# cvlab-epfl/gecco

Measured on AMD Instinct MI355X. Metric: denoiser_fwd_points_per_sec, higher is better.
Workload: dtype f16/fp6/fp8 mixed (the mixed mode with the point MLP of every layer as ONE launch: fp16 main products + fp6 block-scaled second terms for AdaGN(x) and both weights, the 768-wide hidden layer kept in registers as fp16; the other sites as in the mixed mode; fp32 accumulate, residual stream and statist; 1 GPU; C2 unconditional denoiser forward: B=64/GPU, N=2048, d=384, L=6, I=64, H=8, EDMPrecond(LinearLift(SetTransformer)), mixed fp16 / fp6- and fp8-cross-term MFMA, one-launch point MLP, random-init weights; parallelism=single GPU

## Files before the change

### gecco_amd/_lib.py

```python
from __future__ import annotations

import ctypes as C
import os

_HERE = os.path.dirname(os.path.abspath(__file__))
LIB_PATH = os.environ.get("GECCO_HIP_LIB") or os.path.join(_HERE, "libgecco_hip.so")
ABI_VERSION = 14

c_f = C.c_void_p


class GeccoAdaGN(C.Structure):
    _fields_ = [("scale_w", c_f), ("scale_b", c_f), ("bias_w", c_f), ("bias_b", c_f)]


class GeccoMLP(C.Structure):
    _fields_ = [("w0", c_f), ("b0", c_f), ("alpha", c_f), ("w2", c_f), ("b2", c_f)]


class GeccoLayer(C.Structure):
    _fields_ = [("broadcast_norm", GeccoAdaGN), ("inducers", c_f), ("kv_proj_w", c_f), ("pool_out_w", c_f),
                ("norm_1", GeccoAdaGN), ("bmlp", GeccoMLP), ("norm_2", GeccoAdaGN), ("in_proj_w", c_f),
                ("in_proj_b", c_f), ("unpool_out_w", c_f), ("unpool_out_b", c_f), ("mlp_norm", GeccoAdaGN),
                ("mlp", GeccoMLP)]


class GeccoSetTransformer(C.Structure):
    _fields_ = [("n_layers", C.c_int), ("C", C.c_int), ("H", C.c_int), ("I", C.c_int), ("ctx_dim", C.c_int),
                ("G", C.c_int), ("width", C.c_int), ("act", C.c_int), ("precision", C.c_int), ("images_ready", C.c_int),
                ("opt_mask", C.c_uint), ("opt_vals", C.c_uint), ("layers", C.POINTER(GeccoLayer))]


class GeccoLinearLift(C.Structure):
    _fields_ = [("inner", GeccoSetTransformer), ("lift_w", c_f), ("lift_b", c_f), ("lower_w", c_f),
                ("lower_b", c_f), ("sigma_data", C.c_float)]


class GeccoLinearLiftG(C.Structure):
    _fields_ = [("base", GeccoLinearLift), ("geometry_dim", C.c_int), ("do_norm", C.c_int)]


class GeccoPyramid(C.Structure):
    _fields_ = [("n_levels", C.c_int), ("C", C.c_int * 4), ("H", C.c_int * 4), ("W", C.c_int * 4), ("feat", c_f * 4),
                ("texel_f16", C.c_int)]


class GeccoReparam(C.Structure):
    _fields_ = [("kind", C.c_int), ("mean", c_f), ("std", c_f), ("logit_scale", C.c_float)]


class GeccoRayNetwork(C.Structure):
    _fields_ = [("backbone", GeccoSetTransformer), ("xyz_w", c_f), ("xyz_b", c_f), ("img_w", c_f), ("img_b", c_f),
                ("out_w", c_f), ("out_b", c_f), ("reparam", GeccoReparam), ("sigma_data", C.c_float)]


class GeccoGemm(C.Structure):
    _fields_ = [("A", c_f), ("B", c_f), ("bias", c_f), ("C", c_f), ("Z", C.c_int), ("zdiv", C.c_int), ("M", C.c_int),
                ("N", C.c_int), ("K", C.c_int), ("lda", C.c_int), ("ldb", C.c_int), ("ldc", C.c_int),
                ("sA1", C.c_longlong), ("sA2", C.c_longlong), ("sB1", C.c_longlong), ("sB2", C.c_longlong),
                ("sC1", C.c_longlong), ("sC2", C.c_longlong), ("a_kmajor", C.c_int), ("b_kmajor", C.c_int),
                ("scale", C.c_float)]


class GeccoSplitJob(C.Structure):
    _fields_ = [("W", c_f), ("img", C.c_void_p), ("Nout", C.c_int), ("K", C.c_int), ("ldw", C.c_int), ("transposed", C.c_int)]


class GeccoAdamEma(C.Structure):
    _fields_ = [("p", c_f), ("g", c_f), ("m", c_f), ("v", c_f), ("ema", c_f), ("n", C.c_size_t), ("lr", C.c_double),
                ("beta1", C.c_double), ("beta2", C.c_double), ("eps", C.c_double), ("weight_decay", C.c_double),
                ("ema_decay", C.c_double), ("grad_scale", C.c_float), ("step", C.c_int), ("do_ema", C.c_int)]


i, sz, vp, fl, db, u64 = C.c_int, C.c_size_t, C.c_void_p, C.c_float, C.c_double, C.c_uint64
PP = C.POINTER(C.c_void_p)

SIGNATURES = {
    "gecco_abi_version": (i, []),
    "gecco_build_arch": (C.c_char_p, []),
    "gecco_last_error": (C.c_char_p, []),
    "gecco_linear_f32": (i, [vp] * 9 + [i, i, i, i, i, vp]),
    "gecco_linear_row_tiles": (i, [i]),
    "gecco_linear_ex_f32": (i, [vp] * 9 + [i, i, i, i, i, i, vp, vp]),
    "gecco_linear_pair_f32": (i, [vp, vp, vp, i, vp, vp, vp, i, vp, vp, vp, i, i, i, i, vp, vp]),
    "gecco_split_bf16_images_f32": (i, [C.POINTER(GeccoSplitJob), i, vp]),
    "gecco_split_bf16_image_bytes": (sz, [i, i]),
    "gecco_linear_image_ok": (i, [i, i, i, i]),
    "gecco_split_f16_images_f32": (i, [C.POINTER(GeccoSplitJob), i, vp]),
    "gecco_split_f16_image_bytes": (sz, [i, i]),
    "gecco_linear_image_ok_f16": (i, [i, i, i, i]),
    "gecco_linear_actbwd_ok": (i, [i, i, i, i]),
    "gecco_linear_actbwd_tiles": (sz, [i, i, i]),
    "gecco_linear_actbwd_f32": (i, [vp, vp, vp, vp, i, vp, vp, vp, i, i, i, i, i, vp, vp]),
    "gecco_linear_act_keep_f32": (i, [vp, vp, vp, vp, i, vp, vp, i, i, i, i, i, vp, vp]),
    "gecco_linear_act_keep_pro_f32": (i, [vp, vp, vp, vp, vp, vp, i, vp, vp, i, i, i, i, i, vp, vp]),
    "gecco_linear_f16io": (i, [vp] * 7 + [i, i, i, i, i, i, i, vp, vp]),
    "gecco_linear_pair_f16io": (i, [vp, vp, vp, i, vp, vp, vp, i, vp, i, i, i, vp, vp]),
    "gecco_mlp_fused_f16": (i, [vp, vp, vp, vp, vp, vp, vp, vp, i, vp, i, i, i, i, vp, vp]),
    "gecco_unpool_outproj_f16": (i, [vp, vp, vp, vp, vp, vp, i, i, i, i, vp, vp]),
    "gecco_unpool_outproj_h8": (i, [vp, vp, vp, vp, vp, vp, i, i, i, i, vp, vp]),
    "gecco_mlp_fused_w": (i, [vp, vp, vp, vp, vp, vp, vp, vp, vp, i, vp, i, i, i, i, vp, vp, vp]),
    "gecco_mlp_fused_w_wsplit_bytes": (sz, [i, i]),
    "gecco_unpool_outproj_h8_wsplit_bytes": (sz, [i, i, i]),
    "gecco_unpool_attn_h8img": (i, [vp, vp, vp, i, i, i, i, vp]),
    "gecco_gemm_tn_x3_f32": (i, [vp, vp, vp, i, i, i, i, i, vp]),
    "gecco_gemm_tn_x3_bias_f32": (i, [vp, vp, vp, vp, i, i, i, i, i, vp]),
    "gecco_gemm_tn_x3_pro_f32": (i, [vp, vp, vp, vp, vp, vp, i, i, i, i, i, vp]),
    "gecco_gemm_tn_f16_f32": (i, [vp, vp, vp, vp, vp, vp, i, i, i, i, i, vp]),
    "gecco_gemm_tn_f16_tiles": (i, [i, i]),
    "gecco_gemm_tn_f16_b16_f32": (i, [vp, vp, vp, vp, i, i, i, i, i, vp]),
    "gecco_gemm_tn_f16_a16_f32": (i, [vp, vp, vp, vp, vp, vp, i, i, i, i, i, vp]),
    "gecco_gemm_tn_f16_ex_f32": (i, [vp, i, vp, i, vp, vp, vp, vp, vp, vp, vp, i, i, i, i, i, vp]),
    "gecco_linear_dotstats_a16_f32": (i, [vp] * 6 + [i, i, i, i, vp, vp]),
    "gecco_linear_astat16_actbwd_h16": (i, [vp] * 4 + [i, vp, vp, i, i, i, i, vp, vp]),
    "gecco_linear_dotstats_f32": (i, [vp] * 5 + [i, i, i, i, i, vp, vp]),
    "gecco_h8_image_bytes": (sz, [i, i]),
    "gecco_linear_h8_train_ok": (i, [i, i, i]),
    "gecco_h8_images_f32": (i, [C.POINTER(GeccoSplitJob), i, vp]),
    "gecco_linear_h8_train_f32": (i, [vp] * 5 + [i, vp, vp, vp, i, vp, vp, i, vp, i, i, i, vp, vp]),
    "gecco_astat16_image_bytes": (sz, [i, i]),
    "gecco_linear_astat16_ok": (i, [i, i, i]),
    "gecco_astat16_images_f32": (i, [C.POINTER(GeccoSplitJob), i, vp]),
    "gecco_linear_astat16_f32": (i, [vp] * 5 + [i, vp, vp, vp, i, vp, vp, i, i, i, i, vp, vp]),
    "gecco_linear_astat16_keep": (i, [vp] * 6 + [i, vp, vp, i, i, i, i, vp, vp]),
    "gecco_linear_astat16_keep_y16": (i, [vp] * 6 + [i, vp, vp, vp, i, i, i, i, vp, vp]),
    "gecco_linear_astat16_actbwd": (i, [vp] * 4 + [i, vp, vp, i, i, i, i, vp, vp]),
    "gecco_linear_act_keep_h16": (i, [vp] * 6 + [i, vp, vp, i, i, i, i, vp, vp]),
    "gecco_set_option": (i, [C.c_char_p, i]),
    "gecco_option_index": (i, [C.c_char_p]),
    "gecco_cast_f16": (i, [c_f, C.c_void_p, C.c_size_t, C.c_void_p]),
    "gecco_linear_astat_f16": (i, [vp, vp, vp, vp, vp, i, vp, vp, vp, i, vp, vp, i, i, i, i, i, vp, vp]),
    "gecco_linear_kvq_f16": (i, [vp, vp, vp, vp, vp, i, vp, vp, vp, i, vp, i, i, i, i, i, i, vp, vp]),
    "gecco_linear_kvq_y16_f16": (i, [vp, vp, vp, vp, vp, i, vp, vp, vp, i, vp, vp, i, i, i, i, i, i, vp, vp]),
    "gecco_linear_h8_img_f32": (i, [vp, vp, vp, vp, vp, vp, i, vp, i, i, i, i, i, vp, vp]),
    "gecco_linear_h8_areg_f32": (i, [vp, vp, vp, vp, vp, vp, i, i, i, i, vp, vp]),
    "gecco_affine_cast_f16": (i, [vp, vp, vp, vp, i, i, i, vp]),
    "gecco_pool_attn_f16in": (i, [vp, vp, vp, i, i, i, i, i, i, vp, sz, vp]),
    "gecco_unpool_attn_f16io": (i, [vp, vp, vp, i, i, i, i, i, i, vp]),
    "gecco_lift0_fold_f32": (i, [vp] * 8 + [i, i, i, vp]),
    "gecco_lift0_rows": (i, [vp, vp, vp, vp, i, i, i, i, i, i, i, vp]),
    "gecco_lift0_pool_f32": (i, [vp] * 5 + [i, i, i, i, vp, sz, vp]),
    "gecco_col_stats_f32": (i, [vp, vp, i, i, i, vp]),
    "gecco_stats_row_tiles": (i, [i]),
    "gecco_adagn_coeffs_f32": (i, [vp, i, i, vp, i, C.POINTER(GeccoAdaGN), vp, vp, i, i, i, fl, vp]),
    "gecco_affine_apply_f32": (i, [vp, vp, vp, vp, i, i, i, vp]),
    "gecco_adagn_f32": (i, [vp, vp, i, C.POINTER(GeccoAdaGN), vp, i, i, i, i, fl, vp, sz, vp]),
    "gecco_adagn_workspace_bytes": (sz, [i, i, i]),
    "gecco_pool_attn_f32": (i, [vp, vp, vp, i, i, i, i, i, vp, sz, vp]),
    "gecco_pool_attn_ex_f32": (i, [vp, vp, vp, i, i, i, i, i, i, vp, sz, vp]),
    "gecco_pool_attn_workspace_bytes": (sz, [i, i, i, i, i]),
    "gecco_unpool_attn_f32": (i, [vp, vp, vp, i, i, i, i, i, vp]),
    "gecco_unpool_attn_ex_f32": (i, [vp, vp, vp, i, i, i, i, i, i, vp]),
    "gecco_pool_attn_lse_f32": (i, [vp, sz, vp, i, i, i, i, i, vp]),
    "gecco_pool_attn_bwd_partials": (i, [i, i, i]),
    "gecco_pool_attn_bwd_f32": (i, [vp] * 7 + [i, i, i, i, i, vp]),
    "gecco_unpool_attn_bwd_partials": (i, [i, i, i]),
    "gecco_unpool_attn_bwd_f32": (i, [vp] * 5 + [i, i, i, i, i, vp]),
    "gecco_pool_attn_bwd_ex_f32": (i, [vp] * 7 + [i, i, i, i, i, i, vp]),
    "gecco_unpool_attn_bwd_ex_f32": (i, [vp] * 5 + [i, i, i, i, i, i, vp]),
    "gecco_edm_coeffs_f32": (i, [vp, fl, vp, i, vp]),
    "gecco_lift_f32": (i, [vp, vp, vp, vp, vp, vp, i, i, i, vp]),
    "gecco_lower_edm_f32": (i, [vp] * 9 + [i, i, i, fl, vp]),
    "gecco_set_transformer_fwd_f32": (i, [C.POINTER(GeccoSetTransformer), vp, vp, vp, i, PP, PP, vp, i, i, vp, sz, vp]),
    "gecco_set_transformer_workspace_bytes": (sz, [C.POINTER(GeccoSetTransformer), i, i]),
    "gecco_linear_lift_fwd_f32": (i, [C.POINTER(GeccoLinearLift), vp, vp, vp, vp, PP, PP, i, i, vp, sz, vp]),
    "gecco_linear_lift_workspace_bytes": (sz, [C.POINTER(GeccoLinearLift), i, i]),
    "gecco_lift_g_f32": (i, [vp, vp, vp, vp, vp, vp, i, i, i, i, vp]),
    "gecco_lower_edm_g_f32": (i, [vp] * 7 + [i, i, i, i, i, fl, vp]),
    "gecco_linear_lift_g_fwd_f32": (i, [C.POINTER(GeccoLinearLiftG), vp, vp, vp, vp, PP, PP, i, i, vp, sz, vp]),
    "gecco_linear_lift_g_workspace_bytes": (sz, [C.POINTER(GeccoLinearLiftG), i, i]),
    "gecco_nchw_to_nhwc_f32": (i, [vp, vp, i, i, i, i, vp]),
    "gecco_bilinear_taps_f32": (i, [vp, i, i, vp, vp, vp, vp, sz, vp]),
    "gecco_ray_lookup_taps_f32": (i, [vp, vp, vp, vp, vp, vp, vp, vp, vp, vp, i, i, vp]),
    "gecco_ray_lookup_f32": (i, [vp, vp, vp, C.POINTER(GeccoReparam), C.POINTER(GeccoPyramid), vp, vp, i, i, vp]),
    "gecco_lookup_row_tiles": (i, [i]),
    "gecco_ray_lookup_bwd_f32": (i, [vp, vp, vp, C.POINTER(GeccoReparam), C.POINTER(GeccoPyramid), vp, PP, i, i, vp]),
    "gecco_ray_lookup_dgeom_f32": (i, [vp, vp, C.POINTER(GeccoReparam), C.POINTER(GeccoPyramid), vp, vp, vp, i, i, vp]),
    "gecco_ray_lookup_bwd_sorted_workspace_bytes": (C.c_size_t, [C.POINTER(GeccoPyramid), i, i]),
    "gecco_ray_lookup_bwd_sorted_f32": (i, [vp, vp, vp, C.POINTER(GeccoReparam), C.POINTER(GeccoPyramid), vp, PP, i, i, vp,
                                            C.c_size_t, vp]),
    "gecco_ray_network_fwd_f32": (i, [C.POINTER(GeccoRayNetwork), vp, vp, vp, C.POINTER(GeccoPyramid), vp, vp, PP, PP,
                                      i, i, vp, sz, vp]),
    "gecco_ray_network_workspace_bytes": (sz, [C.POINTER(GeccoRayNetwork), C.POINTER(GeccoPyramid), i, i]),
# ... 112 lines not shown
```

### gecco_amd/csrc/api_common.h

```cpp
#pragma once
#include "../../include/gecco_hip.h"
#include "kernels.h"

namespace gecco_api {

extern thread_local char g_err[512];
int fail(int rc, const char* fmt, ...);

inline int check(int rc, const char* what) {
    if (rc == 0) return 0;
    if (rc > 0) return fail(rc, "%s: HIP error %d (%s)", what, rc, hipGetErrorString((hipError_t)rc));
    return fail(rc, "%s: unsupported arguments (code %d)", what, rc);
}
#define TRY(expr, what)                  \
    do {                                 \
        int rc_ = check((expr), (what)); \
        if (rc_) return rc_;             \
    } while (0)

struct Carver {
    char* base;
    size_t off = 0;
    explicit Carver(void* b) : base(static_cast<char*>(b)) {}
    float* f32(size_t n) {
        off = (off + 255) & ~size_t(255);
        float* p = base ? reinterpret_cast<float*>(base + off) : nullptr;
        off += n * sizeof(float);
        return p;
    }
};

inline int row_tiles_gemm(int rows) { const int bm = gemm_row_tile(rows); return (rows + bm - 1) / bm; }
inline int row_tiles_stats(int rows) { const int bm = stats_row_tile(rows); return (rows + bm - 1) / bm; }

enum { OPT_ASTAT = 0, OPT_CHAIN = 1, OPT_HEADMAJOR = 2, OPT_MLPFUSED = 3, OPT_UNPOOLFUSED = 4, OPT_LO8 = 5, OPT_ACTIMG = 6, OPT_H8 = 7, OPT_KVQ64 = 8, OPT_H8AREG = 9, OPT_CHAIN2 = 10, OPT_UNPOOLH8 = 11, OPT_MLPW = 12, OPT_CHAINCL = 13, OPT_H6 = 14, OPT_KVFOLD = 15, OPT_MLPWSHARE = 16, OPT_KVQPERM = 17, OPT_IMGPROJ16 = 18, OPT_LIFT0 = 19, OPT_COUNT = 20 };
enum { OPT_LIFT0_HI = OPT_LIFT0 + 1 };
int option(int which);

int make_lookup_args(const GeccoReparam* rp, const GeccoPyramid* pyr, LookupArgs* a);

inline GemmArgs gemm_args(const float* A, const float* W, const float* bias, float* C, int B, int rows, int K, int Nout) {
    GemmArgs g{};
    g.A = A; g.W = W; g.bias = bias; g.C = C; g.B = B; g.rows = rows; g.K = K; g.Nout = Nout; g.lda = K; g.ldw = K; g.ldc = Nout; g.ldr = Nout;
    return g;
}
inline GemmArgs gemm_args_pair(const float* A, const float* bias1, float* C1, int Nout1, const float* bias2, float* C2, int Nout2, int B, int rows, int K) {
    GemmArgs g = gemm_args(A, nullptr, bias1, C1, B, rows, K, Nout1 + Nout2);
    g.ldc = Nout1; g.ldr = Nout1;
    if (C2) { g.C2 = C2; g.bias2 = bias2; g.n_split = Nout1; g.ldc2 = Nout2; }
    return g;
}

inline int check_pro_pair(const char* who, const float* pro_a, const float* pro_o, bool spaced = false) {
    if ((pro_a == nullptr) == (pro_o == nullptr)) return 0;
    return fail(-1, spaced ? "%s: pro_a / pro_o must both be set" : "%s: pro_a/pro_o must both be set", who);
}
inline int check_alpha(const char* who, int act, const float* alpha, int rc) {
    return ((act == 1 || act == 2) && !alpha) ? fail(rc, "%s: GaussianActivation needs alpha", who) : 0;
}
inline int check_precision(const char* who, int precision, const void* wsplit) {
    if (precision < 0 || precision > 2) return fail(-2, "%s: precision must be 0 (fp32), 1 (split-bf16) or 2 (fp16)", who);
    if (precision >= 1 && !wsplit) return fail(-1, "%s: precision 1 / 2 need the wsplit scratch", who);
    return 0;
}
inline int check_dma_linear(const char* who, bool dma_ok, const float* W, int precision, const void* wsplit) {
    if (!dma_ok) return fail(-2, "%s: shape / precision outside the LDS-DMA kernels' reach", who);
    if (precision >= 1 && !wsplit) return fail(-1, "%s: precision 1 / 2 need wsplit", who);
    if (!W && precision == 0) return fail(-2, "%s: W == NULL (image ready) needs precision 1 / 2", who);
    return 0;
}

}
```

### gecco_amd/csrc/api_linear.hip

```cpp
#include "api_linear.h"

using namespace gecco_api;

extern "C" {

int gecco_linear_row_tiles(int rows) { return row_tiles_gemm(rows); }
int gecco_stats_row_tiles(int rows) { return row_tiles_stats(rows); }

int gecco_linear_f32(const float* A, const float* W, const float* bias, const float* pro_a, const float* pro_o,
                     const float* alpha, const float* residual, float* C, float* stats, int B, int rows, int K,
                     int Nout, int act, void* stream) {
    if (!A || !W || !C) return fail(-1, "linear: null argument");
    if (int rc = check_pro_pair("linear", pro_a, pro_o)) return rc;
    TRY(linear(Lin(A, W, bias, C, B, rows, K, Nout).pro(pro_a, pro_o).activation(act, alpha).plus(residual).with_stats(stats), (hipStream_t)stream), "linear");
    return 0;
}

int gecco_linear_ex_f32(const float* A, const float* W, const float* bias, const float* pro_a, const float* pro_o,
                        const float* alpha, const float* residual, float* C, float* stats, int B, int rows, int K,
                        int Nout, int act, int precision, void* wsplit, void* stream) {
    if (!A || !C) return fail(-1, "linear: null argument");
    if (int rc = check_pro_pair("linear", pro_a, pro_o)) return rc;
    if (int rc = check_precision("linear", precision, wsplit)) return rc;
    if (!W) {
// ... 322 lines not shown
    if (W1) {
        if (Nout2 > 0 && !W2) return fail(-1, "linear_kvq: W2 missing");
        TRY(build_images(h8_image_multi_launch, wsplit, K, s, {W1, Nout1, K, kvq_format(lo_begin / 64, lo_end / 64, order)},
                         {Nout2 > 0 ? W2 : nullptr, Nout2, K, kvq_format(0, 0, order)}, kvq_image_bytes(Nout1, K, lo_end - lo_begin)), "linear_kvq(image)");
    }
    TRY(gemm_kvq_astat_launch(g, s), "linear_kvq");
    return 0;
}

int gecco_linear_h8_img_f32(const float* x, const float* pro_a, const float* pro_o, const float* W, const float* bias,
                            const float* alpha, int act, void* c_img, int image_kind, int B, int rows, int K, int Nout, void* wsplit,
                            void* stream) {
    if (!x || !c_img || !wsplit) return fail(-1, "linear_h8_img: null argument");
    if (image_kind != 1 && image_kind != 2) return fail(-2, "linear_h8_img: image_kind must be 1 (tiled split image) or 2 (h8 activation image)");
    if (int rc = check_pro_pair("linear_h8_img", pro_a, pro_o)) return rc;
    if (int rc = check_alpha("linear_h8_img", act, alpha, -6)) return rc;
    hipStream_t s = (hipStream_t)stream;
    GemmArgs g = gemm_args(x, nullptr, bias, static_cast<float*>(c_img), B, rows, K, Nout);
    g.ldr = 0;
    g.pro_a = pro_a; g.pro_o = pro_o; g.alpha = alpha; g.act = act; g.c_img = image_kind; g.w_img = wsplit;
    g.h6 = image_kind == 2 && option(OPT_H6) ? 1 : 0;
    if (!gemm_h8_astat_supported(g))
        return fail(-2, "linear_h8_img: needs rows %% 128 == 0, Nout %% 64 == 0, Nout >= 128, K in {128, 256, 384}, act in 0 .. 3");
    if (W) TRY(build_images(h8_image_multi_launch, wsplit, K, s, {W, Nout, K, g.h6 ? H8_H6 : H8_MLP0}), "linear_h8_img(image)");
    TRY(gemm_h8_astat_launch(g, s), "linear_h8_img");
    return 0;
}

int gecco_linear_h8_areg_f32(const void* a_img, const float* W, const float* bias, const float* residual, float* C, float* stats,
                             int B, int rows, int K, int Nout, void* wsplit, void* stream) {
    if (!a_img || !C || !wsplit) return fail(-1, "linear_h8_areg: null argument");
    hipStream_t s = (hipStream_t)stream;
    GemmArgs g = gemm_args(static_cast<const float*>(a_img), nullptr, bias, C, B, rows, K, Nout);
    g.residual = residual; g.stats = stats; g.a_img = 2; g.w_img = wsplit; g.precision = 1;
    if (!gemm_h8_areg_supported(g))
        return fail(-2, "linear_h8_areg: needs rows %% 128 == 0, K in {128, 256, 384, 512, 768, 1024}, Nout %% 4 == 0");
    if (W) TRY(build_images(h8_image_multi_launch, wsplit, K, s, {W, Nout, K, H8_W128}), "linear_h8_areg(image)");
    TRY(gemm_h8_areg_launch(g, s), "linear_h8_areg");
    return 0;
}

int gecco_mlp_fused_f16(float* x, const float* pro_a, const float* pro_o, const float* W0, const float* b0, const float* W2,
                        const float* b2, const float* alpha, int act, float* stats, int B, int rows, int C, int width,
                        void* wsplit, void* stream) {
    if (!x || !pro_a || !pro_o || !wsplit || ((W0 == nullptr) != (W2 == nullptr))) return fail(-1, "mlp_fused: null argument");
    if (int rc = check_alpha("mlp_fused", act, alpha, -6)) return rc;
    if (!mlp_fused_f16_supported(C, width, rows))
        return fail(-2, "mlp_fused: needs C in {128, 256, 384}, width == 2 C, rows %% 128 == 0");
    hipStream_t s = (hipStream_t)stream;
    float* img = static_cast<float*>(wsplit);
    if (W0) {
        SplitJobs jobs;
        jobs.n = 0;
        TRY(mlp_fused_f16_stream_jobs(W0, W2, C, width, img, [&jobs](const float* W, float* at, int Nout, int K, int ldw, F16Image format, const char*) {
                if (jobs.n >= (int)(sizeof jobs.job / sizeof jobs.job[0])) return -9;
                jobs.job[jobs.n++] = SplitJob{W, at, Nout, K, ldw, format};
                return 0;
            }), "mlp_fused(split)");
        TRY(split_f16_tiled_multi_launch(jobs, s), "mlp_fused(split)");
    }
    MlpArgs ma{};
    ma.x = x; ma.pro_a = pro_a; ma.pro_o = pro_o; ma.w_stream = img; ma.b0 = b0; ma.b2 = b2; ma.alpha = alpha; ma.act = act;
    ma.stats = stats; ma.B = B; ma.rows = rows;
    TRY(mlp_fused_f16_launch(ma, C, width, s), "mlp_fused");
    return 0;
}

int gecco_unpool_outproj_f16(float* x, const void* q16, const float* kvh, const float* W, const float* bias, float* stats,
                             int B, int rows, int C, int H, void* wsplit, void* stream) {
    if (!x || !q16 || !kvh || !wsplit) return fail(-1, "unpool_outproj: null argument");
    if (!unpool_outproj_f16_supported(C, H, rows))
        return fail(-2, "unpool_outproj: needs (C, head dim) in {(128, 16), (256, 32), (384, 48)}, rows %% 128 == 0");
    hipStream_t s = (hipStream_t)stream;
    if (W) TRY(split_f16_tiled_launch(W, wsplit, C, C, C, s), "unpool_outproj(split)");
    UnpoolProjArgs ua{};
    ua.x = x; ua.q16 = q16; ua.kvh = kvh; ua.w_stream = static_cast<const float*>(wsplit); ua.bias = bias; ua.stats = stats;
    ua.B = B; ua.rows = rows; ua.H = H;
    TRY(unpool_outproj_f16_launch(ua, C, s), "unpool_outproj");
    return 0;
}

int gecco_unpool_outproj_h8(float* x, const void* q16, const float* kvh, const float* W, const float* bias, float* stats,
                            int B, int rows, int C, int H, void* wsplit, void* stream) {
    if (!x || !q16 || !kvh || !wsplit) return fail(-1, "unpool_outproj_h8: null argument");
    if (!unpool_outproj_h8_supported(C, H, rows))
        return fail(-2, "unpool_outproj_h8: needs (C, head dim) in {(128, 16), (256, 32), (384, 48)}, rows %% 128 == 0");
    hipStream_t s = (hipStream_t)stream;
    if (W) TRY(build_images(h8_image_multi_launch, wsplit, C, s, {W, C, C, H8_ATTN_ORDER}), "unpool_outproj_h8(split)");
    void* kvimg = static_cast<char*>(wsplit) + h8_image_bytes(C, C);
    TRY(kvh_image_launch(kvh, kvimg, B, C, H, s), "unpool_outproj_h8(k | v image)");
    UnpoolH8Args ua{};
    ua.x = x; ua.q16 = q16; ua.kv_img = kvimg; ua.w_img = wsplit; ua.bias = bias; ua.stats = stats; ua.B = B; ua.rows = rows; ua.H = H;
    TRY(unpool_outproj_h8_launch(ua, C, s), "unpool_outproj_h8");
    return 0;
}

int gecco_mlp_fused_w(const float* x, float* out, const float* pro_a, const float* pro_o, const float* W0, const float* b0, const float* W2,
                      const float* b2, const float* alpha, int act, float* stats, int B, int rows, int C, int width, void* wsplit, float* dbg_u,
                      void* stream) {
    if (!x || !out || !pro_a || !pro_o || !wsplit) return fail(-1, "mlp_fused_w: null argument");
    if (!mlp_fused_w_supported(C, width, rows)) return fail(-2, "mlp_fused_w: needs C in {128, 256, 384, 512}, width == 2 C, rows %% 128 == 0");
    if (act < 0 || act > 3) return fail(-6, "mlp_fused_w: act must be 0 .. 3");
    if (int rc = check_alpha("mlp_fused_w", act, alpha, -6)) return rc;
    hipStream_t s = (hipStream_t)stream;
    if (W0 && W2) TRY(mlp_fused_w_image_launch(W0, b0, W2, b2, wsplit, C, width, alpha, act, s), "mlp_fused_w(image)");
    MlpWArgs ma{};
    ma.x = x; ma.out = out; ma.pro_a = pro_a; ma.pro_o = pro_o; ma.w_img = wsplit; ma.alpha = alpha; ma.act = act; ma.stats = stats;
    ma.B = B; ma.rows = rows; ma.dbg_u = dbg_u; ma.share = option(OPT_MLPWSHARE);
    TRY(mlp_fused_w_launch(ma, C, width, s), "mlp_fused_w");
    return 0;
}

size_t gecco_mlp_fused_w_wsplit_bytes(int C, int width) { return mlp_fused_w_image_bytes(C, width); }

size_t gecco_unpool_outproj_h8_wsplit_bytes(int B, int C, int H) {
    if (H <= 0 || C % H) return 0;
    return h8_image_bytes(C, C) + unpool_outproj_h8_kv_bytes(B, C, H);
}

int gecco_unpool_attn_h8img(const void* q16, const float* kvh, void* out_img, int B, int N, int C, int H, void* stream) {
    if (!q16 || !kvh || !out_img) return fail(-1, "unpool_attn_h8img: null argument");
    if (N % 128 || C % 64 || H <= 0 || C % H || !attn_x3_supported(C / H)) return fail(-2, "unpool_attn_h8img: needs N %% 128 == 0, C %% 64 == 0, head dim 16 / 32 / 48 / 64");
    TRY(unpool_attn_launch(static_cast<const float*>(q16), kvh, static_cast<float*>(out_img), B, N, C, H, 64, (hipStream_t)stream, 2, 2, 1, 2),
        "unpool_attn_h8img");
    return 0;
}

int gecco_gemm_tn_x3_f32(const float* A, const float* Bm, float* parts, int Z, int R, int N, int K, int group, void* stream) {
    return gecco_gemm_tn_x3_bias_f32(A, Bm, parts, nullptr, Z, R, N, K, group, stream);
}

int gecco_gemm_tn_x3_bias_f32(const float* A, const float* Bm, float* parts, float* colsum_parts, int Z, int R, int N, int K,
                              int group, void* stream) {
    return gecco_gemm_tn_x3_pro_f32(A, Bm, nullptr, nullptr, parts, colsum_parts, Z, R, N, K, group, stream);
}

static TnArgs tn_args(const void* A, const void* Bm, const float* pro_a, const float* pro_o, float* parts, float* colsum_parts, int Z, int R, int N, int K, int group) {
    TnArgs g{};
    g.pro_a = pro_a; g.pro_o = pro_o;
    g.A = static_cast<const float*>(A); g.Bm = static_cast<const float*>(Bm); g.C = parts; g.Z = Z; g.R = R; g.N = N; g.K = K; g.lda = N; g.ldb = K;
    g.sA = (size_t)R * N; g.sB = (size_t)R * K; g.group = group; g.colsum = colsum_parts;
    return g;
}

int gecco_gemm_tn_x3_pro_f32(const float* A, const float* Bm, const float* pro_a, const float* pro_o, float* parts,
                             float* colsum_parts, int Z, int R, int N, int K, int group, void* stream) {
    if (!A || !Bm || !parts) return fail(-1, "gemm_tn_x3: null argument");
    if (int rc = check_pro_pair("gemm_tn_x3", pro_a, pro_o, true)) return rc;
    const TnArgs g = tn_args(A, Bm, pro_a, pro_o, parts, colsum_parts, Z, R, N, K, group);
    if (!gemm_tn_x3_supported(g)) return fail(-2, "gemm_tn_x3: needs R %% 32 == 0, N %% 4 == 0, K %% 4 == 0, group > 0");
    TRY(gemm_tn_x3_launch(g, (hipStream_t)stream), "gemm_tn_x3");
    return 0;
}

static int gemm_tn_f16(const char* who, const char* needs, const void* A, int a_f16, const void* Bm, int b_f16, const float* pro_a, const float* pro_o, float* parts,
                       float* colsum_parts, float* out, float* colsum_out, unsigned* counters, int Z, int R, int N, int K, int group, void* stream) {
    if (!A || !Bm || !parts) return fail(-1, "%s: null argument", who);
    if (int rc = check_pro_pair(who, pro_a, pro_o, true)) return rc;
    TnArgs g = tn_args(A, Bm, pro_a, pro_o, parts, colsum_parts, Z, R, N, K, group);
    g.f16 = 1; g.a_f16 = a_f16; g.b_f16 = b_f16; g.counters = counters; g.out = out; g.colsum_out = colsum_out;
    if (!gemm_tn_f16_supported(g)) return fail(-2, "%s: needs %s", who, needs);
    TRY(gemm_tn_f16_launch(g, (hipStream_t)stream), who);
    return 0;
}

int gecco_gemm_tn_f16_b16_f32(const float* A, const void* B16, float* parts, float* colsum_parts, int Z, int R, int N, int K, int group,
                              void* stream) {
    return gemm_tn_f16("gemm_tn_f16_b16", "R % 32 == 0, N % 4 == 0, K % 8 == 0, group > 0", A, 0, B16, 1, nullptr, nullptr, parts, colsum_parts, nullptr, nullptr, nullptr,
                       Z, R, N, K, group, stream);
}

int gecco_gemm_tn_f16_ex_f32(const void* A, int a_f16, const void* Bm, int b_f16, const float* pro_a, const float* pro_o, float* parts,
                             float* colsum_parts, float* out, float* colsum_out, unsigned* counters, int Z, int R, int N, int K, int group,
                             void* stream) {
    if (!A || !Bm || !parts) return fail(-1, "gemm_tn_f16_ex: null argument");
    if (int rc = check_pro_pair("gemm_tn_f16_ex", pro_a, pro_o, true)) return rc;
// ... 34 lines not shown
```

### gecco_amd/csrc/api_model_ops.hip

```cpp
#include "api_common.h"

#include <math.h>

using namespace gecco_api;

int gecco_api::make_lookup_args(const GeccoReparam* rp, const GeccoPyramid* pyr, LookupArgs* a) {
    if (!pyr || pyr->n_levels < 1 || pyr->n_levels > 4) return fail(-8, "lookup: 1..4 pyramid levels required");
    a->n_levels = pyr->n_levels;
    a->c_total = 0;
    for (int l = 0; l < 4; ++l) {
        const bool on = l < pyr->n_levels;
        a->C[l] = on ? pyr->C[l] : 0;
        a->H[l] = on ? pyr->H[l] : 1;
        a->W[l] = on ? pyr->W[l] : 1;
        a->feat[l] = on ? pyr->feat[l] : nullptr;
        if (on && !pyr->feat[l]) return fail(-1, "lookup: null pyramid level %d", l);
        a->c_total += a->C[l];
    }
    a->texel_f16 = pyr->texel_f16 ? 1 : 0;
    a->out_f16 = 0;
    a->reparam_kind = rp ? rp->kind : 0;
    a->rp_mean = rp ? rp->mean : nullptr;
    a->rp_std = rp ? rp->std : nullptr;
    a->logit_scale = rp ? rp->logit_scale : 1.1f;
// ... 116 lines not shown
    c.f32((size_t)B * H * ns * 64 * 2);
    return (c.off + 255) & ~size_t(255);
}

int gecco_pool_attn_ex_f32(const float* KV, const float* inducers, float* merged, int B, int N, int C, int H, int I,
                           int precision, void* ws, size_t ws_bytes, void* stream) {
    if (precision < 0 || precision > 2) return fail(-2, "pool_attn: precision must be 0 (fp32), 1 (split-bf16) or 2 (fp16)");
    if (ws_bytes < gecco_pool_attn_workspace_bytes(B, N, C, H, I)) return fail(-7, "pool_attn: workspace too small");
    Carver c(ws);
    const int ns = pool_attn_nsplit(B, N, H);
    float* po = c.f32((size_t)B * H * ns * 64 * (C / H));
    float* pml = c.f32((size_t)B * H * ns * 64 * 2);
    TRY(pool_attn_launch(KV, inducers, po, pml, merged, B, N, C, H, I, ns, (hipStream_t)stream, precision), "pool_attn");
    return 0;
}

int gecco_pool_attn_lse_f32(const void* ws, size_t ws_bytes, float* lse, int B, int N, int C, int H, int I, void* stream) {
    if (ws_bytes < gecco_pool_attn_workspace_bytes(B, N, C, H, I)) return fail(-7, "pool_attn_lse: workspace too small");
    Carver c(const_cast<void*>(ws));
    const int ns = pool_attn_nsplit(B, N, H);
    c.f32((size_t)B * H * ns * 64 * (C / H));
    const float* pml = c.f32((size_t)B * H * ns * 64 * 2);
    TRY(pool_attn_lse_launch(pml, lse, B, H, ns, (hipStream_t)stream), "pool_attn_lse");
    return 0;
}

int gecco_pool_attn_bwd_partials(int B, int N, int H) { return pool_attn_bwd_nsplit(B, N, H); }
int gecco_unpool_attn_bwd_partials(int B, int N, int H) { return unpool_attn_bwd_chunks(B, N, H, nullptr); }

int gecco_pool_attn_bwd_f32(const float* KV, const float* inducers, const float* merged, const float* lse, const float* dO,
                            float* dKV, float* dQ_partials, int B, int N, int C, int H, int I, void* stream) {
    return gecco_pool_attn_bwd_ex_f32(KV, inducers, merged, lse, dO, dKV, dQ_partials, B, N, C, H, I, 0, stream);
}
int gecco_unpool_attn_bwd_f32(const float* q, const float* kvh, const float* dO, float* dq, float* dkv_partials, int B, int N,
                              int C, int H, int I, void* stream) {
    return gecco_unpool_attn_bwd_ex_f32(q, kvh, dO, dq, dkv_partials, B, N, C, H, I, 0, stream);
}

int gecco_pool_attn_bwd_ex_f32(const float* KV, const float* inducers, const float* merged, const float* lse, const float* dO,
                               float* dKV, float* dQ_partials, int B, int N, int C, int H, int I, int precision, void* stream) {
    if (B <= 0 || N <= 0) return fail(-2, "pool_attn_bwd: empty batch");
    if (precision < 0 || precision > 3) return fail(-2, "pool_attn_bwd: precision must be 0 (fp32), 1 (split-bf16), 2 (fp16 operands) or 3 (fp16 operands, fp16 KV / dKV tensors)");
    const int rc = pool_attn_bwd_launch(KV, inducers, merged, lse, dO, dKV, dQ_partials, B, N, C, H, I, pool_attn_bwd_nsplit(B, N, H),
                                        (hipStream_t)stream, precision);
    if (rc == -3 || rc == -4) return fail(-2, "pool_attn_bwd: needs I == 64 and a head dim that is a multiple of 8 up to 64");
    TRY(rc, "pool_attn_bwd");
    return 0;
}

int gecco_unpool_attn_bwd_ex_f32(const float* q, const float* kvh, const float* dO, float* dq, float* dkv_partials, int B, int N,
                                 int C, int H, int I, int precision, void* stream) {
    if (B <= 0 || N <= 0) return fail(-2, "unpool_attn_bwd: empty batch");
    if (precision < 0 || precision > 3) return fail(-2, "unpool_attn_bwd: precision must be 0 (fp32), 1 (split-bf16), 2 (fp16 operands) or 3 (fp16 operands, fp16 q / dO / dq tensors)");
    const int rc = unpool_attn_bwd_launch(q, kvh, dO, dq, dkv_partials, B, N, C, H, I, (hipStream_t)stream, precision);
    if (rc == -3 || rc == -4) return fail(-2, "unpool_attn_bwd: needs I == 64 and a head dim that is a multiple of 8 up to 64");
    TRY(rc, "unpool_attn_bwd");
    return 0;
}

int gecco_pool_attn_f32(const float* KV, const float* inducers, float* merged, int B, int N, int C, int H, int I,
                        void* ws, size_t ws_bytes, void* stream) {
    return gecco_pool_attn_ex_f32(KV, inducers, merged, B, N, C, H, I, 0, ws, ws_bytes, stream);
}

int gecco_unpool_attn_ex_f32(const float* q, const float* kvh, float* out, int B, int N, int C, int H, int I,
                             int precision, void* stream) {
    if (precision < 0 || precision > 2) return fail(-2, "unpool_attn: precision must be 0 (fp32), 1 (split-bf16) or 2 (fp16)");
    TRY(unpool_attn_launch(q, kvh, out, B, N, C, H, I, (hipStream_t)stream, precision), "unpool_attn");
    return 0;
}

int gecco_unpool_attn_f32(const float* q, const float* kvh, float* out, int B, int N, int C, int H, int I,
                          void* stream) {
    return gecco_unpool_attn_ex_f32(q, kvh, out, B, N, C, H, I, 0, stream);
}

int gecco_edm_coeffs_f32(const float* sigma, float sigma_data, float* coef, int B, void* stream) {
    TRY(edm_coeffs_launch(sigma, sigma_data, coef, B, (hipStream_t)stream), "edm_coeffs");
    return 0;
}

int gecco_lift_f32(const float* x, const float* coef, const float* W, const float* bias, float* out, float* stats,
                   int B, int N, int C, void* stream) {
    TRY(lift_launch(x, coef, W, bias, out, stats, B, N, C, (hipStream_t)stream), "lift");
    return 0;
}

int gecco_lower_edm_f32(const float* feat, const float* x, const float* coef, const float* W, const float* bias,
                        const float* gn_a, const float* gn_o, float* out, float* raw, int B, int N, int C, float eps,
                        void* stream) {
    if (coef && !x) return fail(-1, "lower_edm: x required with coef");
    TRY(lower_edm_launch(feat, x, coef, W, bias, gn_a, gn_o, out, raw, B, N, C, eps, (hipStream_t)stream), "lower_edm");
    return 0;
}

int gecco_lift_g_f32(const float* x, const float* coef, const float* W, const float* bias, float* out, float* stats,
                     int B, int N, int C, int G, void* stream) {
    if (G < 1 || G > GECCO_MAX_GEOMETRY_DIM) return fail(-2, "lift_g: geometry_dim %d outside 1 .. %d", G, GECCO_MAX_GEOMETRY_DIM);
    TRY(lift_g_launch(x, coef, W, bias, out, stats, B, N, C, G, (hipStream_t)stream), "lift_g");
    return 0;
}

int gecco_lower_edm_g_f32(const float* feat, const float* x, const float* coef, const float* W, const float* bias, float* out,
                          float* raw, int B, int N, int C, int G, int do_norm, float eps, void* stream) {
    if (coef && !x) return fail(-1, "lower_edm_g: x required with coef");
    if (G < 1 || G > GECCO_MAX_GEOMETRY_DIM) return fail(-2, "lower_edm_g: geometry_dim %d outside 1 .. %d", G, GECCO_MAX_GEOMETRY_DIM);
    if (C <= 0 || C % 4 || C > 512) return fail(-2, "lower_edm_g: feature_dim %d (needs C %% 4 == 0, C <= 512)", C);
    TRY(lower_g_launch(feat, x, coef, W, bias, out, raw, B, N, C, G, do_norm, eps, (hipStream_t)stream), "lower_edm_g");
    return 0;
}

int gecco_nchw_to_nhwc_f32(const float* src, float* dst, int B, int C, int H, int W, void* stream) {
    TRY(nchw_to_nhwc_launch(src, dst, B, C, H, W, (hipStream_t)stream), "nchw_to_nhwc");
    return 0;
}

int gecco_bilinear_taps_f32(const float* uv, int H, int W, int* x0, int* y0, float* wx1, float* wy1, size_t n,
                            void* stream) {
    TRY(bilinear_taps_launch(uv, H, W, x0, y0, wx1, wy1, n, (hipStream_t)stream), "bilinear_taps");
    return 0;
}

int gecco_lookup_row_tiles(int N) { return (N + lookup_row_tile() - 1) / lookup_row_tile(); }

int gecco_cast_f16(const float* src, void* dst, size_t n, void* stream) {
    if (n && (!src || !dst)) return fail(-1, "cast_f16: null argument");
    TRY(cast_f16_launch(src, dst, n, (hipStream_t)stream), "cast_f16");
    return 0;
}

int gecco_ray_lookup_f32(const float* geom, const float* coef, const float* K, const GeccoReparam* rp,
                         const GeccoPyramid* pyr, float* out, float* stats, int B, int N, void* stream) {
    if (!geom || !K || !out) return fail(-1, "ray_lookup: null argument");
    LookupArgs a;
    int rc = make_lookup_args(rp, pyr, &a);
    if (rc) return rc;
    TRY(ray_lookup_launch(geom, coef, K, a, out, stats, B, N, (hipStream_t)stream), "ray_lookup");
    return 0;
}

int gecco_ray_lookup_taps_f32(const float* geom, const float* coef, const float* K, const GeccoReparam* rp, const GeccoPyramid* pyr, float* uv,
                              int* x0, int* y0, float* wx1, float* wy1, int B, int N, void* stream) {
    if (!geom || !K || !pyr || !uv || !x0 || !y0 || !wx1 || !wy1) return fail(-1, "ray_lookup_taps: null argument");
    LookupArgs a;
    int rc = make_lookup_args(rp, pyr, &a);
    if (rc) return rc;
    TRY(ray_lookup_taps_launch(geom, coef, K, a, uv, x0, y0, wx1, wy1, B, N, (hipStream_t)stream), "ray_lookup_taps");
    return 0;
}

int gecco_ray_lookup_bwd_f32(const float* geom, const float* coef, const float* K, const GeccoReparam* rp,
                             const GeccoPyramid* pyr, const float* dout, float* const* dfeat, int B, int N,
                             void* stream) {
    if (!geom || !K || !dout || !dfeat || !pyr) return fail(-1, "ray_lookup_bwd: null argument");
    LookupArgs a;
    int rc = make_lookup_args(rp, pyr, &a);
    if (rc) return rc;
    if (a.texel_f16) return fail(-2, "ray_lookup_bwd: fp16 texel pyramids serve the forward lookup only (pass the fp32 levels)");
    for (int l = 0; l < a.n_levels; ++l)
        if (!dfeat[l]) return fail(-1, "ray_lookup_bwd: null gradient level");
    TRY(ray_lookup_bwd_launch(geom, coef, K, a, dfeat, dout, B, N, (hipStream_t)stream), "ray_lookup_bwd");
    return 0;
}

int gecco_ray_lookup_dgeom_f32(const float* geom, const float* K, const GeccoReparam* rp, const GeccoPyramid* pyr, const float* dout,
                               float* dgeom, float* dK_partials, int B, int N, void* stream) {
// ... 353 lines not shown
```

### gecco_amd/csrc/api_network.hip

```cpp
#include "api_linear.h"

#include <atomic>
#include <stdarg.h>
#include <stdlib.h>
#include <string.h>
#include <stdio.h>

using namespace gecco_api;

namespace {

std::atomic<int> g_options[OPT_COUNT] = {-1, -1, -1, -1, -1, -1, -1, -1, -1, -1, -1, -1, -1, -1, -1, -1, -1, -1, -1, -1};
const char* const g_option_names[OPT_COUNT] = {"astat", "chain", "headmajor", "mlpfused", "unpoolfused", "lo8", "actimg", "h8", "kvq64", "h8areg", "chain2", "unpoolh8", "mlpw", "chaincl", "h6", "kvfold", "mlpwshare", "kvqperm", "imgproj16", "lift0"};
const char* const g_option_env[OPT_COUNT] = {"GECCO_ASTAT", "GECCO_CHAIN", "GECCO_HEADMAJOR", "GECCO_MLPFUSED", "GECCO_UNPOOLFUSED", "GECCO_LO8",
                                             "GECCO_ACTIMG", "GECCO_H8", "GECCO_KVQ64", "GECCO_H8AREG", "GECCO_CHAIN2", "GECCO_UNPOOLH8", "GECCO_MLPW", "GECCO_CHAINCL", "GECCO_H6", "GECCO_KVFOLD", "GECCO_MLPWSHARE",
                                             "GECCO_KVQPERM", "GECCO_IMGPROJ16", "GECCO_LIFT0"};
thread_local const GeccoSetTransformer* t_plan = nullptr;
struct PlanScope {
    const GeccoSetTransformer* prev;
    explicit PlanScope(const GeccoSetTransformer* p) : prev(t_plan) { t_plan = p; }
    ~PlanScope() { t_plan = prev; }
};

}

namespace gecco_api {

thread_local char g_err[512] = "";

int fail(int rc, const char* fmt, ...) {
    va_list ap;
    va_start(ap, fmt);
    vsnprintf(g_err, sizeof g_err, fmt, ap);
    va_end(ap);
    return rc;
}

int option(int which) {
    if (t_plan && ((t_plan->opt_mask >> which) & 1u)) {
        const int v = (int)((t_plan->opt_vals >> which) & 1u);
        return which == OPT_LIFT0 && v ? v + (int)((t_plan->opt_vals >> OPT_LIFT0_HI) & 1u) : v;
    }
    int v = g_options[which].load(std::memory_order_relaxed);
    if (v < 0) {
        const char* e = getenv(g_option_env[which]);
        const int fill = which == OPT_LIFT0 ? (e ? (atoi(e) < 0 ? 0 : atoi(e) > 2 ? 2 : atoi(e)) : 3)
                         : e ? (atoi(e) != 0) : (which != OPT_MLPWSHARE && which != OPT_IMGPROJ16);
        if (g_options[which].compare_exchange_strong(v, fill, std::memory_order_relaxed)) v = fill;
    }
    return v;
}

int linear(Lin& a, hipStream_t s) {
    GemmArgs& g = a.g;
    const int precision = a.prec;
    g.precision = 0; g.w_img = nullptr;
    if (g.act < 0 || g.act > 4) return -6;
    if ((g.act == 1 || g.act == 2) && !g.alpha) return -6;
    const bool fast = precision == 1 ? gemm_f32_dma_supported(g, 1) : precision == 2 ? gemm_f16_dma_supported(g) : false;
    const bool img = a.wsplit || a.img_ready;
    if ((g.a_f16 || g.c_f16) && !(fast && precision == 2 && img)) return -9;
    if ((g.a_img || g.c_img) && !(fast && precision == 1 && img)) return -9;
    if ((g.mul_u || g.pre_out || g.dot_x) && !(precision == 0 ? gemm_f32_dma_supported(g, 0) : (fast && img))) return -9;
    if (!g.W && !(fast && a.img_ready)) return -9;
    if (fast && img) {
        if (a.img_ready) {
            g.w_img = a.img_ready;
        } else {
            int rc = precision == 1 ? split_bf16_tiled_launch(g.W, a.wsplit, g.Nout, g.K, g.ldw, s) : split_f16_tiled_launch(g.W, a.wsplit, g.Nout, g.K, g.ldw, s);
            if (rc) return rc;
            g.w_img = a.wsplit;
        }
        g.precision = precision;
    }
    return gemm_f32_launch(g, s);
}

int linear_pair(const Lin& a, const float* W2, const float* b2, int Nout2, float* C2, hipStream_t s) {
    GemmArgs g = a.g;
    const int precision = a.prec, Nout1 = a.g.Nout, K = a.g.K;
    if ((g.c_f16 || g.a_f16) && precision != 2) return -9;
    g.Nout = Nout1 + Nout2;
    g.C2 = C2; g.W2 = W2; g.bias2 = b2; g.n_split = Nout1; g.ldc2 = Nout2;
    if (precision == 2 ? !gemm_f16_dma_supported(g) : !gemm_f32_dma_supported(g)) return 1;
    if (precision == 1 || precision == 2) {
        if (a.img_ready) {
            g.w_img = a.img_ready;
        } else {
            if (!a.wsplit) return 1;
            const bool x3 = precision == 1;
            const ImageFormat plain = x3 ? ImageFormat(BF16_PLAIN) : ImageFormat(F16_PLAIN);
            const int rc = build_images(x3 ? launch_each<split_bf16_tiled_launch> : launch_each<split_f16_tiled_launch>, a.wsplit, K, s, {g.W, Nout1, K, plain}, {W2, Nout2, K, plain},
                                        x3 ? split_bf16_image_bytes(Nout1, K) : split_f16_image_bytes(Nout1, K));
            if (rc) return rc;
            g.w_img = a.wsplit;
        }
        g.precision = precision;
    }
    if (precision == 2) return gemm_f16_dma_launch(g, s);
    return gemm_f32_dma_launch(g, s);
}

}

namespace {

struct STWorkspace {
    float *big, *q, *attn;
    float *stats_x, *stats_s;
    float *a1, *o1, *a2, *o2, *as, *os;
    float *part_o, *part_ml;
    float *merged, *h0, *u, *h2, *h, *kvh;
    float* wsplit;
    float* wimg;
    size_t wimg_layer, o_q, o_out, o_w0, o_w2;
    size_t o_pout, o_b0, o_b2, o_ukv, b2_half;
    size_t o_mf;
    size_t o_q16, o_kv_lo, o_q64;
    float* mc;
    size_t bytes;
};

struct Lift0In { const float *x, *coef, *lift_w, *lift_b; };

int max_i(int a, int b) { return a > b ? a : b; }

STWorkspace carve_st(const GeccoSetTransformer* st, int B, int N, void* base) {
    Carver c(base);
// ... 38 lines not shown
        w.wimg_layer = w.o_mf + (prec == 2 ? img(W, C) + img(C, W) : 0);
        if (st->precision == 4 && mlp_fused_w_supported((int)C, (int)W, 128)) w.wimg_layer += mlp_fused_w_image_bytes((int)C, (int)W) / sizeof(float);
        w.wimg = prec >= 1 ? c.f32(w.wimg_layer * st->n_layers) : nullptr;
        w.b2_half = img(C, C);
        const size_t f16_kv = split_f16_image_bytes(2 * (int)C, (int)C) / sizeof(float), f16_q = split_f16_image_bytes((int)C, (int)C) / sizeof(float);
        w.o_q16 = f16_kv; w.o_kv_lo = f16_kv + f16_q;
        w.o_q64 = kvq_image_bytes(2 * (int)C, (int)C, (int)C) / sizeof(float);
    }
    w.mc = c.f32((size_t)B * 3 * C * 4);
    w.bytes = (c.off + 255) & ~size_t(255);
    return w;
}

bool chain_stream_fits(const GeccoSetTransformer* st, const STWorkspace& w) {
    const size_t C = st->C, W = st->width;
    const bool f16 = st->precision == 2;
    auto img = [f16](size_t n, size_t k) { return (f16 ? split_f16_image_bytes((int)n, (int)k) : 2 * split_f16_image_bytes((int)n, (int)k)) / sizeof(float); };
    if (C % 128) return false;
    return w.o_b0 - w.o_pout == img(C, C) && w.o_b2 - w.o_b0 == img(W, C) && w.o_ukv - w.o_b2 == W / C * w.b2_half && w.o_mf - w.o_ukv == img(2 * C, C);
}

int astat_linear(const float* x, const float* pa, const float* po, const float* img, const float* bias1, int Nout1,
                 float* C1, const float* bias2, int Nout2, float* C2, const float* alpha, int act, int B, int rows,
                 int K, hipStream_t s, int hm_hd = 0, const float* img_lo = nullptr, int use64 = 0, int kvq_perm = 0, int lo_fp8 = 0) {
    GemmArgs g = gemm_args_pair(x, bias1, C1, Nout1, bias2, C2, Nout2, B, rows, K);
    g.pro_a = pa; g.pro_o = po; g.precision = 2; g.w_img = img; g.c_f16 = 1; g.hm_hd = hm_hd;
    if (use64) {
        g.kvq_perm = kvq_perm; if (use64 == 2) { g.lo_begin = Nout1 / 128; g.lo_tiles = Nout1 / 64; }
        if (!img || act || !gemm_kvq_astat_supported(g)) return 1;
        return gemm_kvq_astat_launch(g, s);
    }
    g.alpha = alpha; g.act = act; g.w_img2 = img_lo;
    if (img_lo && C2) { g.lo_begin = Nout1 / 256; g.lo_tiles = Nout1 / 128; }
    g.lo_fp8 = img_lo && lo_fp8;
    if (!img || !gemm_f16_astat_supported(g)) return 1;
    return gemm_f16_astat_launch(g, s);
}

int h8_linear(const float* a_img, const float* w_img, const float* bias, const float* res, float* C, float* stats, int B, int rows,
              int K, int Nout, hipStream_t s) {
    GemmArgs g = gemm_args(a_img, nullptr, bias, C, B, rows, K, Nout);
    g.residual = res; g.stats = stats; g.a_img = 2; g.w_img = w_img; g.precision = 1;
    return gemm_h8_areg_launch(g, s);
}

int coeffs(const float* stats, int T, int rows, const float* t, int ctx, const GeccoAdaGN* p, float* a, float* o,
           int B, int C, int G, hipStream_t s) {
    return adagn_coeffs_launch(stats, T, rows, t, ctx, p ? p->scale_w : nullptr, p ? p->scale_b : nullptr,
                               p ? p->bias_w : nullptr, p ? p->bias_b : nullptr, a, o, B, C, G, 1e-5f, s);
}

struct StRoute {
    int rc;
    int pr, apr, kmod, Tn, Ti, ns;
    bool mixed;
    bool astat;
    bool imgs, build;
    bool io16;
    bool a16;
    int hd_try;
    bool mlpf_on;
    bool h8_on;
    bool kvq_on;
    bool kvq16_on;
    int use64;
    bool kvq_p48;
    bool lo8;
    bool h8x, h8o;
    bool h6_on;
    bool uo8_on;
    bool uof_on;
    int aimg;
    bool o8;
    int himg;
    bool mfw_on;
    int mfw_share;
    bool chain_on;
    bool chain2_on;
    bool chain;
    bool chain_cl;
    bool kvfold;
    int lift0;
    bool lift0_hm;
};

StRoute st_route(const GeccoSetTransformer* st, int B, int N, const float* const* h_in, bool points) {
    StRoute r{};
    const int C = st->C, I = st->I, H = st->H, G = st->G, Wd = st->width, act = st->act;
    const int prec = st->precision == 4 ? 3 : st->precision;
    const bool wimg = prec >= 1;
    const void* const some_img = st;
    r.mixed = prec == 3 && N >= 128 && N % 128 == 0 && C % 128 == 0 && C <= 512 && !(C % H) &&
              attn_x3_supported(C / H) && st->I == 64 && option(OPT_ASTAT);
    const bool mixed = r.mixed;
    const int pr = r.pr = mixed ? 1 : (prec == 3 ? 1 : prec);
    r.apr = mixed ? 2 : pr;
    r.Tn = row_tiles_gemm(N); r.Ti = row_tiles_gemm(I); r.kmod = (pr == 2 || mixed) ? 32 : 16;
    const int ns = r.ns = pool_attn_nsplit(B, N, H);
    r.mlpf_on = pr == 2 && wimg && option(OPT_MLPFUSED) && mlp_fused_f16_supported(C, Wd, N);
    if (mixed && wimg && option(OPT_H8) && option(OPT_ACTIMG) && (act == 0 || (act >= 1 && act <= 3))) {
        GemmArgs hg{};
        hg.c_img = 1; hg.w_img = some_img; hg.rows = N; hg.Nout = Wd; hg.K = C; hg.lda = C; hg.act = act;
        r.h8_on = gemm_h8_astat_supported(hg) && Wd % 16 == 0 && C % 16 == 0;
    }
    r.kvq_on = mixed && wimg && option(OPT_KVQ64) && option(OPT_HEADMAJOR) && (C == 128 || C == 256 || C == 384 || C == 512) && !((C / H) & 7);
    r.kvq16_on = !mixed && pr == 2 && wimg && option(OPT_KVQ64) && option(OPT_HEADMAJOR) && option(OPT_ASTAT) && C == 512 &&
                 !((C / H) & 7) && N >= 128 && N % 128 == 0;
    auto h8_areg_takes = [&](int K) {
        GemmArgs hg{};
        hg.a_img = 2; hg.w_img = some_img; hg.rows = N; hg.Nout = C; hg.K = K; hg.lda = K; hg.ldc = C; hg.ldr = C;
        return gemm_h8_areg_supported(hg);
    };
    r.h8x = mixed && wimg && option(OPT_H8AREG) && option(OPT_ACTIMG) && Wd % 64 == 0 && N % 128 == 0 && h8_areg_takes(Wd);
    r.h8o = mixed && wimg && option(OPT_H8AREG) && option(OPT_ACTIMG) && I == 64 && C % 64 == 0 && attn_x3_supported(C / H) && h8_areg_takes(C);
    r.h6_on = r.h8_on && r.h8x && option(OPT_H6);
    r.uo8_on = r.h8o && r.kvq_on && option(OPT_UNPOOLH8) && I == 64 && unpool_outproj_h8_supported(C, H, N) &&
               unpool_outproj_h8_kv_bytes(B, C, H) <= (size_t)B * N * C * sizeof(float);
    r.mfw_on = mixed && st->precision == 4 && option(OPT_MLPW) && wimg && mlp_fused_w_supported(C, Wd, N) &&
               (size_t)B * N * C * sizeof(float) < ((size_t)1 << 31);
    r.mfw_share = r.mfw_on ? option(OPT_MLPWSHARE) : 0;
    r.chain_on = pr == 2 && wimg && option(OPT_CHAIN) && inducer_chain_f16_supported(C, Wd, H, G, I) &&
                 (ns == 1 || ns == 2 || ns == 4 || ns == 8);
    const bool cl_ok = option(OPT_CHAINCL) && C >= 256 && (size_t)st->n_layers * 8 <= (size_t)I * C;
    r.chain2_on = mixed && wimg && option(OPT_CHAIN2) && (C <= 384 || cl_ok) && inducer_chain_f16_supported(C, Wd, H, G, I) &&
                  (ns == 1 || ns == 2 || ns == 4 || ns == 8) && (act >= 0 && act <= 3);
    r.imgs = pr >= 1 && wimg && !(C % r.kmod) && !(Wd % r.kmod);
    r.build = r.imgs && !st->images_ready;
    r.astat = option(OPT_ASTAT);
    r.hd_try = option(OPT_HEADMAJOR) ? C / H : 0;
    r.use64 = r.kvq_on ? 2 : r.kvq16_on ? 1 : 0;
    r.kvq_p48 = r.kvq_on && option(OPT_KVQPERM) && r.hd_try && kvq_perm48_ok(C / H, C, 2 * C, C);
    r.lo8 = mixed && !r.kvq_on && option(OPT_LO8) && gemm_f16_astat_lo8_supported(C);
    r.io16 = (pr == 2 || mixed) && r.imgs && N >= 128 && attn_x3_supported(C / H) && !(C % 8) && !(Wd % 8);
    if (mixed && !(r.io16 && !(N % 128) && !(C % 128))) {
        r.rc = fail(-3, "set_transformer: the mixed mode needs rows %% 128 == 0, feature_dim %% 128 == 0 and a head dim of 16 / 32 / 48 / 64");
        return r;
    }
    r.a16 = r.io16 && !mixed;
    r.uof_on = !mixed && r.imgs && I == 64 && option(OPT_UNPOOLFUSED) && unpool_outproj_f16_supported(C, H, N);
    r.aimg = pr == 1 && !r.a16 && r.imgs && option(OPT_ACTIMG) && I == 64 && attn_x3_supported(C / H) && N >= 128 && N % 128 == 0 && C % 64 == 0;
    r.o8 = r.h8o && r.aimg && N % 128 == 0;
    r.himg = pr == 1 && !r.a16 && r.imgs && option(OPT_ACTIMG) && N >= 128 && N % 128 == 0 && Wd % 16 == 0 && C % 16 == 0;
    r.chain = (r.chain_on || r.chain2_on) && r.imgs;
    r.chain_cl = r.chain && cl_ok;
    r.kvfold = r.uo8_on && r.chain && option(OPT_KVFOLD);
    for (int li = 0; r.kvfold && li < st->n_layers; ++li)
        if (h_in && h_in[li]) r.kvfold = false;
    r.lift0 = points && lift0_supported(C, H) ? option(OPT_LIFT0) : 0;
    if (r.lift0 == 3) r.lift0 = C >= 256 ? 2 : 0;
    if (r.lift0 == 2 && !lift0_pool_supported(C, H)) r.lift0 = 1;
    r.lift0_hm = r.lift0 && r.io16 && r.astat && r.hd_try && lift0_head_major_ok(C / H);
    if (r.lift0 && r.uo8_on && !r.lift0_hm) r.lift0 = 0;
    return r;
}

template <class Job, int Cap, class Launch>
int push_job(Job (&table)[Cap], int& n, const Job& job, Launch launch) {
    if (n >= Cap) { const int rc = launch(); n = 0; if (rc) return rc; }
    table[n++] = job;
    return 0;
}
struct JobQueue {
    SplitJobs jobs;
    int (*launch)(const SplitJobs&, hipStream_t);
    hipStream_t s;
    JobQueue(int (*launch_)(const SplitJobs&, hipStream_t), hipStream_t s_) : launch(launch_), s(s_) { jobs.n = 0; }
    int flush() { const int rc = launch(jobs, s); jobs.n = 0; return rc; }
    int push(const float* Wp, float* img, int Nout, int K, int ldw, ImageFormat format) {
        return push_job(jobs.job, jobs.n, SplitJob{Wp, img, Nout, K, ldw, format}, [this] { return launch(jobs, s); });
    }
};

int build_weight_images(const StRoute& r, const GeccoSetTransformer* st, const STWorkspace& w, const float* const* h_in, hipStream_t s) {
    const int C = st->C, Wd = st->width, act = st->act;
    JobQueue jobs(r.pr == 2 ? split_f16_tiled_multi_launch : split_bf16_tiled_multi_launch, s);
    const ImageFormat plain = r.pr == 2 ? ImageFormat(F16_PLAIN) : ImageFormat(BF16_PLAIN);
    JobQueue jobs16(split_f16_tiled_multi_launch, s);
    JobQueue jobs8(h8_image_multi_launch, s);
    MlpWImageJob mjobs[16];
    int nmj = 0;
    auto flush_mj = [&] { return mlp_fused_w_images_launch(mjobs, nmj, C, Wd, act, s); };
    for (int li = 0; li < st->n_layers; ++li) {
        const GeccoLayer& L = st->layers[li];
        float* base = w.wimg + (size_t)li * w.wimg_layer;
        const bool cached = h_in && h_in[li];
        const bool own_kvq = r.mixed || r.kvq16_on;
        const bool pts = li == 0 && r.lift0;
        const bool kv_img = !cached && !pts, q_img = !pts;
        if (r.kvq_on) {
            const KvqOrder order = r.kvq_p48 ? KVQ_HEAD48 : KVQ_PLAIN;
            if (kv_img) TRY(jobs8.push(L.kv_proj_w, base, 2 * C, C, C, kvq_format(C / 64, 2 * C / 64, order)), "split(kv_proj, kvq)");
            if (q_img) TRY(jobs8.push(L.in_proj_w, base + w.o_q64, C, C, C, kvq_format(0, 0, order)), "split(q_proj, kvq)");
        } else if (r.mixed) {
            if (kv_img) TRY(jobs16.push(L.kv_proj_w, base, 2 * C, C, C, F16_PLAIN), "split(weights)");
            if (q_img) TRY(jobs16.push(L.in_proj_w, base + w.o_q16, C, C, C, F16_PLAIN), "split(weights)");
            if (kv_img) TRY(jobs16.push(L.kv_proj_w, base + w.o_kv_lo, 2 * C, C, C, r.lo8 ? F16_LO_FP8 : F16_LO), "split(weights)");
        }
        const bool chain2_here = r.chain2_on && !cached;
        if (chain2_here) {
            TRY(jobs16.push(L.pool_out_w, base + w.o_pout, C, C, C, F16_HI_LO), "split(pool.out_proj, two-term)");
            TRY(jobs16.push(L.bmlp.w0, base + w.o_b0, Wd, C, C, F16_HI_LO), "split(broadcast.mlp.0, two-term)");
            for (int hf = 0; hf < Wd / C; ++hf)
                TRY(jobs16.push(L.bmlp.w2 + (size_t)hf * C, base + w.o_b2 + hf * w.b2_half, C, C, Wd, F16_HI_LO), "split(broadcast.mlp.2 K-half, two-term)");
            TRY(jobs16.push(L.in_proj_w + (size_t)C * C, base + w.o_ukv, 2 * C, C, C, F16_HI_LO), "split(unpool.in_proj kv, two-term)");
        }
        if (r.kvq16_on) {
            if (kv_img) TRY(jobs8.push(L.kv_proj_w, base, 2 * C, C, C, kvq_format(0, 0)), "split(kv_proj, kvq)");
            if (q_img) TRY(jobs8.push(L.in_proj_w, base + w.o_q, C, C, C, kvq_format(0, 0)), "split(q_proj, kvq)");
        }
        if (!cached && !chain2_here) {
            if (!own_kvq && kv_img) TRY(jobs.push(L.kv_proj_w, base, 2 * C, C, C, plain), "split(kv_proj)");
            TRY(jobs.push(L.pool_out_w, base + w.o_pout, C, C, C, plain), "split(pool.out_proj)");
            TRY(jobs.push(L.bmlp.w0, base + w.o_b0, Wd, C, C, plain), "split(broadcast.mlp.0)");
            if (r.chain_on) {
                for (int hf = 0; hf < Wd / C; ++hf)
                    TRY(jobs.push(L.bmlp.w2 + (size_t)hf * C, base + w.o_b2 + hf * w.b2_half, C, C, Wd, plain), "split(broadcast.mlp.2 K-half)");
            } else {
                TRY(jobs.push(L.bmlp.w2, base + w.o_b2, C, Wd, Wd, plain), "split(broadcast.mlp.2)");
            }
        }
        if (!chain2_here) TRY(jobs.push(L.in_proj_w + (size_t)C * C, base + w.o_ukv, 2 * C, C, C, plain), "split(unpool.in_proj kv)");
        if (!own_kvq && q_img) TRY(jobs.push(L.in_proj_w, base + w.o_q, C, C, C, plain), "split(q_proj)");
        if (r.h8o) TRY(jobs8.push(L.unpool_out_w, base + w.o_out, C, C, C, r.uo8_on ? H8_ATTN_ORDER : H8_W128), "split(out_proj, h8)");
        else TRY(jobs.push(L.unpool_out_w, base + w.o_out, C, C, C, plain), "split(out_proj)");
        if (r.mlpf_on) {
            const int rc = mlp_fused_f16_stream_jobs(L.mlp.w0, L.mlp.w2, C, Wd, base + w.o_mf, [&jobs](const float* W, float* at, int Nout, int K, int ldw, F16Image format, const char* what) {
                return check(jobs.push(W, at, Nout, K, ldw, format), what);
            });
            if (rc) return rc;
        } else if (r.mfw_on) {
            TRY(push_job(mjobs, nmj, MlpWImageJob{L.mlp.w0, L.mlp.b0, L.mlp.w2, L.mlp.b2, base + w.o_mf, L.mlp.alpha}, flush_mj), "split(mlp, w2 streams)");
        } else {
            if (r.h8_on) TRY(jobs8.push(L.mlp.w0, base + w.o_w0, Wd, C, C, r.h6_on ? H8_H6 : H8_MLP0), "split(mlp.0, h8)");
            else TRY(jobs.push(L.mlp.w0, base + w.o_w0, Wd, C, C, plain), "split(mlp.0)");
            if (r.h8x) TRY(jobs8.push(L.mlp.w2, base + w.o_w2, C, Wd, Wd, H8_W128), "split(mlp.2, h8)");
// ... 36 lines not shown
                       : fail(rc < 0 ? rc : -3, "set_transformer: q projection outside the A-stationary kernel's reach (its weight image is in that kernel's format)");
    if (rc == 0 && r.hd_try) c.hm = 1;
    if (rc < 0) return check(rc, with_kv ? "kv_proj|q_proj (A-stationary)" : "unpool.in_proj(q) (A-stationary)");
    c.q_done = rc == 0;
    if (c.q_done || !with_kv) return 0;
    if (io16) TRY(affine_cast_f16_launch(c.x, w.a1, w.o1, w.attn, B, N, C, c.s), "broadcast_norm -> fp16");
    Lin kv = Lin(io16 ? w.attn : c.x, L.kv_proj_w, nullptr, w.big, B, N, C, 2 * C).pro(io16 ? nullptr : w.a1, io16 ? nullptr : w.o1).f16(io16, io16);
    rc = linear_pair(Lin(kv).weights(r.pr, w.wsplit, (2 * C) % 128 == 0 ? c.im : nullptr), L.in_proj_w, L.in_proj_b, C, w.q, c.s);
    if (rc < 0) return check(rc, "kv_proj|q_proj");
    c.q_done = rc == 0;
    if (!c.q_done) TRY(linear(kv.weights(r.pr, w.wsplit, c.im), c.s), "kv_proj");
    return 0;
}

int project_from_points(StLayer& c, bool with_kv) {
    const StRoute& r = c.r; const STWorkspace& w = c.w; const GeccoLayer& L = c.L;
    const int C = c.st->C, H = c.st->H, B = c.B, N = c.N;
    TRY(lift0_fold_launch(L.kv_proj_w, L.in_proj_w, L.in_proj_b, c.pts->lift_w, c.pts->lift_b, w.a1, w.o1, w.mc, with_kv ? 0 : 2 * C, 3 * C, B, C, c.s), "lift0 fold");
    const int hd = r.lift0_hm ? C / H : 0;
    const Lift0Seg segs[2] = {{w.q, 2 * C, C, hd}, {w.big, 0, 2 * C, hd}};
    TRY(lift0_rows_launch(c.pts->x, c.pts->coef, w.mc, segs, with_kv && r.lift0 == 1 ? 2 : 1, r.io16, B, N, C, c.s), "lift0 rows");
    c.hm = hd != 0;
    c.q_done = true;
    return 0;
}

int inducer_stage(StLayer& c) {
    const StRoute& r = c.r; const STWorkspace& w = c.w; const GeccoLayer& L = c.L; const GeccoSetTransformer* st = c.st; hipStream_t s = c.s;
    const int C = st->C, I = st->I, H = st->H, G = st->G, Wd = st->width, ctx = st->ctx_dim, act = st->act, B = c.B, pr = r.pr;
    if (c.pts && r.lift0 == 2) {
        TRY(lift0_pool_launch(c.pts->x, c.pts->coef, w.mc, L.inducers, w.part_o, w.part_ml, B, c.N, C, H, r.ns, s), "pool_attn (points)");
        if (!r.chain) TRY(pool_merge_launch(w.part_o, w.part_ml, w.merged, B, C, H, r.ns, s), "pool_attn merge");
    } else {
        TRY(pool_attn_launch(w.big, L.inducers, w.part_o, w.part_ml, r.chain ? nullptr : w.merged, B, c.N, C, H, I, r.ns, s, r.apr, r.io16, c.hm), "pool_attn");
    }
    if (r.chain) {
        ChainArgs ca{};
        ca.part_o = w.part_o; ca.part_ml = w.part_ml; ca.nsplit = r.ns; ca.H = H;
        ca.w_stream = c.im + w.o_pout;
        ca.b0 = L.bmlp.b0; ca.b2 = L.bmlp.b2; ca.bkv = L.in_proj_b + C; ca.alpha = L.bmlp.alpha; ca.act = act; ca.two_term = r.chain2_on ? 1 : 0;
        ca.n1_scale_w = L.norm_1.scale_w; ca.n1_scale_b = L.norm_1.scale_b; ca.n1_bias_w = L.norm_1.bias_w; ca.n1_bias_b = L.norm_1.bias_b;
        ca.n2_scale_w = L.norm_2.scale_w; ca.n2_scale_b = L.norm_2.scale_b; ca.n2_bias_w = L.norm_2.bias_w; ca.n2_bias_b = L.norm_2.bias_b;
        ca.t = c.t; ca.ctx_dim = ctx; ca.G = G; ca.eps = 1e-5f; ca.h_out = c.hdst; ca.kvh = w.kvh; ca.B = B;
        if (r.chain_cl) {
            ca.cluster = 1; ca.x1 = w.h0; ca.x3 = w.h2; ca.xu = reinterpret_cast<unsigned*>(w.u);
            ca.flags = reinterpret_cast<unsigned*>(w.merged) + (size_t)c.li * B * 8;
        }
        if (r.kvfold) {
            ca.kv_img = reinterpret_cast<unsigned short*>(w.attn);
            ca.kv_img_bytes = (int)(unpool_outproj_h8_kv_bytes(1, C, H) / H);
            c.kv_img_done = true;
        }
        if ((act == 1 || act == 2) && !L.bmlp.alpha) return fail(-6, "inducer chain: GaussianActivation needs alpha");
        TRY(inducer_chain_f16_launch(ca, C, Wd, s), "inducer chain");
        c.kvh_done = true;
    } else {
        TRY(linear(Lin(w.merged, L.pool_out_w, nullptr, w.h0, B, I, C, C).with_stats(w.stats_s).weights(pr, w.wsplit, c.img(w.o_pout)), s), "pool.out_proj");
        TRY(coeffs(w.stats_s, r.Ti, I, c.t, ctx, &L.norm_1, w.as, w.os, B, C, G, s), "adagn_coeffs(norm_1)");
        TRY(linear(Lin(w.h0, L.bmlp.w0, L.bmlp.b0, w.u, B, I, C, Wd).pro(w.as, w.os).activation(act, L.bmlp.alpha).weights(pr, w.wsplit, c.img(w.o_b0)), s), "broadcast.mlp.0");
        TRY(linear(Lin(w.u, L.bmlp.w2, L.bmlp.b2, w.h2, B, I, Wd, C).with_stats(w.stats_s).weights(pr, w.wsplit, c.img(w.o_b2)), s), "broadcast.mlp.2");
        TRY(coeffs(w.stats_s, r.Ti, I, c.t, ctx, &L.norm_2, w.as, w.os, B, C, G, s), "adagn_coeffs(norm_2)");
        TRY(affine_apply_launch(w.h2, w.as, w.os, c.hdst, B, I, C, s), "norm_2 apply");
    }
    c.h = c.hdst;
    return 0;
}

int unpool_stage(StLayer& c) {
    const StRoute& r = c.r; const STWorkspace& w = c.w; const GeccoLayer& L = c.L; float* x = c.x; hipStream_t s = c.s;
    const int C = c.st->C, I = c.st->I, H = c.st->H, B = c.B, N = c.N, pr = r.pr;
    const bool io16 = r.io16;
    if (!c.kvh_done)
        TRY(linear(Lin(c.h, L.in_proj_w + (size_t)C * C, L.in_proj_b + C, w.kvh, B, I, C, 2 * C).weights(pr, w.wsplit, c.img(w.o_ukv)), s), "unpool.in_proj(kv)");
    if (!c.q_done && io16 && c.cached)
        if (const int rc = project_stage(c, false)) return rc;
    if (!c.q_done) {
        if (io16 && c.cached) TRY(affine_cast_f16_launch(x, w.a1, w.o1, w.attn, B, N, C, s), "broadcast_norm -> fp16");
        TRY(linear(Lin(io16 ? w.attn : x, L.in_proj_w, L.in_proj_b, w.q, B, N, C, C).pro(io16 ? nullptr : w.a1, io16 ? nullptr : w.o1)
                       .weights(pr, w.wsplit, c.img(w.o_q)).f16(io16, io16), s), "unpool.in_proj(q)");
    }
    if (r.uo8_on) {
        if (!c.hm || !c.im) return fail(-3, "set_transformer: unpool + out_proj (h8) needs the head-major fp16 q");
        if (!c.kv_img_done) TRY(kvh_image_launch(w.kvh, w.attn, B, C, H, s), "unpool k | v image");
        UnpoolH8Args ua{};
        ua.x = x; ua.q16 = w.q; ua.kv_img = w.attn; ua.w_img = c.im + w.o_out; ua.bias = L.unpool_out_b; ua.stats = w.stats_x; ua.B = B; ua.rows = N; ua.H = H;
        TRY(unpool_outproj_h8_launch(ua, C, s), "unpool attention + out_proj (h8)");
    } else if (r.uof_on && c.hm) {
        UnpoolProjArgs ua{};
        ua.x = x; ua.q16 = w.q; ua.kvh = w.kvh; ua.w_stream = c.im + w.o_out; ua.bias = L.unpool_out_b; ua.stats = w.stats_x; ua.B = B; ua.rows = N; ua.H = H;
        TRY(unpool_outproj_f16_launch(ua, C, s), "unpool attention + out_proj");
    } else {
        TRY(unpool_attn_launch(w.q, w.kvh, w.attn, B, N, C, H, I, s, r.apr, r.mixed ? 2 : (int)io16, c.hm, r.o8 ? 2 : r.aimg), "unpool_attn");
        if (r.o8)
            TRY(h8_linear(w.attn, c.im + w.o_out, L.unpool_out_b, x, x, w.stats_x, B, N, C, C, s), "unpool.out_proj+residual (h8)");
        else
            TRY(linear(Lin(w.attn, L.unpool_out_w, L.unpool_out_b, x, B, N, C, C).plus(x).with_stats(w.stats_x).weights(pr, w.wsplit, c.img(w.o_out))
                           .f16(r.a16, 0).image(r.aimg, 0), s), "unpool.out_proj+residual");
    }
    return 0;
}

int mlp_stage(StLayer& c) {
    const StRoute& r = c.r; const STWorkspace& w = c.w; const GeccoLayer& L = c.L; const GeccoSetTransformer* st = c.st; hipStream_t s = c.s;
    const int C = st->C, G = st->G, Wd = st->width, act = st->act, B = c.B, N = c.N, pr = r.pr, himg = r.himg;
    const bool a16 = r.a16; float *x = c.x, *so = c.so;
    TRY(coeffs(w.stats_x, r.Tn, N, c.t, st->ctx_dim, &L.mlp_norm, w.a2, w.o2, B, C, G, s), "adagn_coeffs(mlp_norm)");
    if (r.mlpf_on && c.im) {
        MlpArgs ma{};
        ma.x = x; ma.pro_a = w.a2; ma.pro_o = w.o2; ma.w_stream = c.im + w.o_mf;
        ma.b0 = L.mlp.b0; ma.b2 = L.mlp.b2; ma.alpha = L.mlp.alpha; ma.act = act; ma.stats = so; ma.B = B; ma.rows = N;
        if ((act == 1 || act == 2) && !L.mlp.alpha) return fail(-6, "mlp: GaussianActivation needs alpha");
        TRY(mlp_fused_f16_launch(ma, C, Wd, s), "mlp (fused)");
        return 0;
    }
    int m0_done = a16 && r.astat ? astat_linear(x, w.a2, w.o2, c.img(w.o_w0), L.mlp.b0, Wd, w.big, nullptr, 0, nullptr, L.mlp.alpha, act, B, N, C, s) : 1;
    if (m0_done < 0) TRY(m0_done, "mlp.0 (A-stationary)");
    if (m0_done == 1 && r.mfw_on && c.im) {
        MlpWArgs ma{};
        ma.x = x; ma.out = x; ma.pro_a = w.a2; ma.pro_o = w.o2; ma.w_img = c.im + w.o_mf; ma.alpha = L.mlp.alpha;
        ma.act = act; ma.stats = so; ma.B = B; ma.rows = N; ma.share = r.mfw_share;
        if ((act == 1 || act == 2) && !L.mlp.alpha) return fail(-6, "mlp: GaussianActivation needs alpha");
        TRY(mlp_fused_w_launch(ma, C, Wd, s), "mlp (one launch, w2)");
        return 0;
    }
    if (m0_done == 1 && r.h8_on && himg && c.im) {
        GemmArgs hg{};
        hg.A = x; hg.pro_a = w.a2; hg.pro_o = w.o2; hg.bias = L.mlp.b0; hg.alpha = L.mlp.alpha; hg.act = act; hg.C = w.big;
        hg.B = B; hg.rows = N; hg.K = C; hg.Nout = Wd; hg.lda = C; hg.ldw = C; hg.ldc = Wd; hg.c_img = r.h8x ? 2 : 1; hg.w_img = c.im + w.o_w0; hg.h6 = r.h6_on ? 1 : 0;
        if ((act == 1 || act == 2) && !L.mlp.alpha) return fail(-6, "mlp.0: GaussianActivation needs alpha");
        TRY(gemm_h8_astat_launch(hg, s), "mlp.0 (h8)");
        m0_done = 0;
    }
    if (m0_done == 1) {
        if (a16) TRY(affine_cast_f16_launch(x, w.a2, w.o2, w.attn, B, N, C, s), "mlp_norm -> fp16");
        TRY(linear(Lin(a16 ? w.attn : x, L.mlp.w0, L.mlp.b0, w.big, B, N, C, Wd).pro(a16 ? nullptr : w.a2, a16 ? nullptr : w.o2).activation(act, L.mlp.alpha)
                       .weights(pr, w.wsplit, c.img(w.o_w0)).f16(a16, a16).image(0, (himg && r.h8x) ? 2 : himg), s), "mlp.0");
    }
    if (himg && r.h8x && c.im) {
        TRY(h8_linear(w.big, c.im + w.o_w2, L.mlp.b2, x, x, so, B, N, Wd, C, s), "mlp.2+residual (h8)");
        return 0;
    }
    TRY(linear(Lin(w.big, L.mlp.w2, L.mlp.b2, x, B, N, Wd, C).plus(x).with_stats(so).weights(pr, w.wsplit, c.img(w.o_w2)).f16(a16, 0).image(himg, 0), s), "mlp.2+residual");
    return 0;
}

int st_forward(const GeccoSetTransformer* st, float* x, const float* t, const float* stats_x, int stats_T,
               const float* const* h_in, float* const* h_out, float* stats_out, int B, int N, void* ws,
               size_t ws_bytes, hipStream_t s, const Lift0In* pts = nullptr) {
    if (!st || !x || !t || !ws) return fail(-1, "set_transformer: null argument");
    if (st->I != 64) return fail(-3, "set_transformer: num_inducers must be 64 (got %d)", st->I);
    if (st->C % st->H || st->C % st->G || st->C % 4) return fail(-3, "set_transformer: bad feature_dim %d", st->C);
    if (st->act < 0 || st->act > 3) return fail(-3, "set_transformer: act must be 0 (identity), 1 / 2 (GaussianActivation normalized / raw) or 3 (ReLU)");
    PlanScope plan_scope(st);
    const STWorkspace w = carve_st(st, B, N, ws);
    if (ws_bytes < w.bytes) return fail(-7, "set_transformer: workspace too small (%zu < %zu)", ws_bytes, w.bytes);
    const StRoute r = st_route(st, B, N, h_in, pts != nullptr);
    if (r.rc) return r.rc;
    if (r.chain && !chain_stream_fits(st, w)) return fail(-3, "set_transformer: the inducer chain's weight stream does not fill its places in the workspace");
    const int C = st->C, H = st->H, G = st->G;
    const float* sx = stats_x; int sT = stats_T;
    if (!sx) {
        TRY(col_stats_launch(x, w.stats_x, B, N, C, s), "col_stats");
        sx = w.stats_x;
        sT = row_tiles_stats(N);
    }
    int rc = r.build ? build_weight_images(r, st, w, h_in, s) : 0;
    if (rc) return rc;
    if (r.chain_cl) TRY((int)hipMemsetAsync(w.merged, 0, (size_t)st->n_layers * B * 8 * sizeof(unsigned), s), "inducer chain counters");
    if (r.kvfold) TRY((int)hipMemsetAsync(w.attn, 0, unpool_outproj_h8_kv_bytes(B, C, H), s), "k | v image pads");
    for (int li = 0; li < st->n_layers; ++li) {
        const GeccoLayer& L = st->layers[li];
        const bool cached = h_in && h_in[li];
        StLayer c{st, r, w, L, li, r.imgs ? w.wimg + (size_t)li * w.wimg_layer : nullptr, x, t, B, N, s, cached ? h_in[li] : nullptr,
                  (h_out && h_out[li]) ? h_out[li] : w.h, (li + 1 < st->n_layers) ? w.stats_x : stats_out, cached};
        TRY(coeffs(sx, sT, N, t, st->ctx_dim, &L.broadcast_norm, w.a1, w.o1, B, C, G, s), "adagn_coeffs(broadcast_norm)");
        if (li == 0 && r.lift0) c.pts = pts;
        rc = c.pts ? project_from_points(c, !cached) : cached ? 0 : project_stage(c, true);
        if (!rc && !cached) rc = inducer_stage(c);
        if (!rc) rc = unpool_stage(c);
        if (!rc) rc = mlp_stage(c);
        if (rc) return rc;
        sx = w.stats_x;
        sT = r.Tn;
    }
    return 0;
}

struct LLWorkspace {
    float *feat, *coef, *stats;
    void* st_ws;
    size_t st_bytes, bytes;
};

LLWorkspace carve_ll(const GeccoLinearLift* m, int B, int N, void* base) {
    Carver c(base);
    LLWorkspace w;
    w.feat = c.f32((size_t)B * N * m->inner.C);
    w.coef = c.f32((size_t)B * 5);
    w.stats = c.f32((size_t)B * row_tiles_stats(N) * 2 * m->inner.C);
    c.off = (c.off + 255) & ~size_t(255);
    w.st_bytes = carve_st(&m->inner, B, N, nullptr).bytes;
    w.st_ws = base ? static_cast<char*>(base) + c.off : nullptr;
    w.bytes = c.off + w.st_bytes;
    return w;
}

struct RNWorkspace {
    float *feat, *raw, *coef, *stats_raw, *stats_x, *stats_out, *a_raw, *o_raw, *a_out, *o_out, *wsplit, *wfold, *bfold;
    void* st_ws;
    size_t st_bytes, bytes;
};

RNWorkspace carve_rn(const GeccoRayNetwork* m, int c_total, int B, int N, void* base) {
    Carver c(base);
    RNWorkspace w;
    const size_t C = m->backbone.C;
    w.feat = c.f32((size_t)B * N * C);
    w.raw = c.f32((size_t)B * N * c_total);
    w.coef = c.f32((size_t)B * 5);
    w.stats_raw = c.f32((size_t)B * gecco_lookup_row_tiles(N) * 2 * c_total);
    w.stats_x = c.f32((size_t)B * row_tiles_gemm(N) * 2 * C);
    w.stats_out = c.f32((size_t)B * row_tiles_gemm(N) * 2 * C);
    w.a_raw = c.f32((size_t)B * c_total);
    w.o_raw = c.f32((size_t)B * c_total);
    w.a_out = c.f32((size_t)B * C);
    w.o_out = c.f32((size_t)B * C);
    w.wsplit = c.f32(((C + 127) / 128 * 128) * (size_t)c_total);
    const bool fold = m->backbone.precision == 4;
    w.wfold = fold ? c.f32((size_t)B * ((C + 127) / 128 * 128) * c_total / 2) : nullptr;
    w.bfold = fold ? c.f32((size_t)B * C) : nullptr;
    c.off = (c.off + 255) & ~size_t(255);
    w.st_bytes = carve_st(&m->backbone, B, N, nullptr).bytes;
    w.st_ws = base ? static_cast<char*>(base) + c.off : nullptr;
    w.bytes = c.off + w.st_bytes;
    return w;
}

}

extern "C" {

int gecco_abi_version(void) { return GECCO_ABI_VERSION; }
const char* gecco_build_arch(void) { return "gfx950"; }
const char* gecco_last_error(void) { return g_err; }

int gecco_option_index(const char* name) {
    if (name)
        for (int i = 0; i < OPT_COUNT; ++i)
            if (!strcmp(name, g_option_names[i])) return i;
    return -1;
}

int gecco_set_option(const char* name, int value) {
    if (!name) return fail(-1, "set_option: null name");
    for (int i = 0; i < OPT_COUNT; ++i)
        if (!strcmp(name, g_option_names[i])) {
            g_options[i].store(value < 0 ? -1 : i == OPT_LIFT0 ? (value > 2 ? 2 : value) : (value != 0), std::memory_order_relaxed);
            return 0;
        }
    return fail(-2, "set_option: unknown option '%s' (astat, chain, headmajor, mlpfused, unpoolfused, lo8, actimg, h8, kvq64, h8areg, chain2, unpoolh8, mlpw, chaincl, h6, kvfold, mlpwshare, kvqperm, imgproj16, lift0)", name);
}

size_t gecco_set_transformer_workspace_bytes(const GeccoSetTransformer* st, int B, int N) {
    return carve_st(st, B, N, nullptr).bytes;
}

int gecco_set_transformer_fwd_f32(const GeccoSetTransformer* st, float* x, const float* t, const float* stats_x,
                                  int stats_T, const float* const* h_in, float* const* h_out, float* stats_out,
                                  int B, int N, void* ws, size_t ws_bytes, void* stream) {
    return st_forward(st, x, t, stats_x, stats_T, h_in, h_out, stats_out, B, N, ws, ws_bytes, (hipStream_t)stream);
}

size_t gecco_linear_lift_workspace_bytes(const GeccoLinearLift* m, int B, int N) {
    return carve_ll(m, B, N, nullptr).bytes;
}

int gecco_linear_lift_fwd_f32(const GeccoLinearLift* m, const float* x, const float* sigma, float* denoised,
                              float* raw, const float* const* h_in, float* const* h_out, int B, int N, void* ws,
                              size_t ws_bytes, void* stream) {
    if (!m || !x || !sigma || !(denoised || raw)) return fail(-1, "linear_lift: null argument");
    LLWorkspace w = carve_ll(m, B, N, ws);
    if (ws_bytes < w.bytes) return fail(-7, "linear_lift: workspace too small (%zu < %zu)", ws_bytes, w.bytes);
    hipStream_t s = (hipStream_t)stream;
    const int C = m->inner.C;
    TRY(edm_coeffs_launch(sigma, m->sigma_data, w.coef, B, s), "edm_coeffs");
    TRY(lift_launch(x, w.coef, m->lift_w, m->lift_b, w.feat, w.stats, B, N, C, s), "lift");
    if (m->inner.ctx_dim != 1) return fail(-3, "linear_lift: t_embed_dim must be 1 under EDMPrecond");
    const Lift0In pts{x, w.coef, m->lift_w, m->lift_b};
    int rc = st_forward(&m->inner, w.feat, w.coef + 4 * (size_t)B, w.stats, row_tiles_stats(N), h_in, h_out, nullptr, B,
                        N, w.st_ws, w.st_bytes, s, &pts);
    if (rc) return rc;
    TRY(lower_edm_launch(w.feat, x, w.coef, m->lower_w, m->lower_b, nullptr, nullptr, denoised, raw, B, N, C, 1e-5f, s),
        "lower_edm");
    return 0;
}

size_t gecco_linear_lift_g_workspace_bytes(const GeccoLinearLiftG* m, int B, int N) {
    return carve_ll(&m->base, B, N, nullptr).bytes;
}

int gecco_linear_lift_g_fwd_f32(const GeccoLinearLiftG* m, const float* x, const float* sigma, float* denoised,
                                float* raw, const float* const* h_in, float* const* h_out, int B, int N, void* ws,
                                size_t ws_bytes, void* stream) {
    if (!m || !x || !sigma || !(denoised || raw)) return fail(-1, "linear_lift_g: null argument");
    const int G = m->geometry_dim, C = m->base.inner.C;
    if (G < 1 || G > GECCO_MAX_GEOMETRY_DIM)
        return fail(-2, "linear_lift_g: geometry_dim %d outside 1 .. %d", G, GECCO_MAX_GEOMETRY_DIM);
    if (C % 4 || C > 512) return fail(-2, "linear_lift_g: feature_dim %d (needs C %% 4 == 0, C <= 512)", C);
    LLWorkspace w = carve_ll(&m->base, B, N, ws);
    if (ws_bytes < w.bytes) return fail(-7, "linear_lift_g: workspace too small (%zu < %zu)", ws_bytes, w.bytes);
    hipStream_t s = (hipStream_t)stream;
    if (m->base.inner.ctx_dim != 1) return fail(-3, "linear_lift_g: t_embed_dim must be 1 under EDMPrecond");
    TRY(edm_coeffs_launch(sigma, m->base.sigma_data, w.coef, B, s), "edm_coeffs");
    TRY(lift_g_launch(x, w.coef, m->base.lift_w, m->base.lift_b, w.feat, w.stats, B, N, C, G, s), "lift_g");
    int rc = st_forward(&m->base.inner, w.feat, w.coef + 4 * (size_t)B, w.stats, row_tiles_stats(N), h_in, h_out, nullptr, B,
                        N, w.st_ws, w.st_bytes, s);
    if (rc) return rc;
    TRY(lower_g_launch(w.feat, x, w.coef, m->base.lower_w, m->base.lower_b, denoised, raw, B, N, C, G, m->do_norm, 1e-5f, s),
        "lower_edm_g");
    return 0;
}

size_t gecco_ray_network_workspace_bytes(const GeccoRayNetwork* m, const GeccoPyramid* pyr, int B, int N) {
    int ct = 0;
    for (int l = 0; l < pyr->n_levels && l < 4; ++l) ct += pyr->C[l];
    return carve_rn(m, ct, B, N, nullptr).bytes;
}

int gecco_ray_network_fwd_f32(const GeccoRayNetwork* m, const float* x, const float* sigma, const float* K,
                              const GeccoPyramid* pyr, float* denoised, float* raw, const float* const* h_in,
                              float* const* h_out, int B, int N, void* ws, size_t ws_bytes, void* stream) {
    if (!m || !x || !sigma || !K || !(denoised || raw)) return fail(-1, "ray_network: null argument");
    if (m->backbone.ctx_dim != 1) return fail(-3, "ray_network: t_embed_dim must be 1 under EDMPrecond");
    LookupArgs a;
    int rc = make_lookup_args(&m->reparam, pyr, &a);
    if (rc) return rc;
    RNWorkspace w = carve_rn(m, a.c_total, B, N, ws);
    if (ws_bytes < w.bytes) return fail(-7, "ray_network: workspace too small (%zu < %zu)", ws_bytes, w.bytes);
    hipStream_t s = (hipStream_t)stream;
    const int C = m->backbone.C;
    TRY(edm_coeffs_launch(sigma, m->sigma_data, w.coef, B, s), "edm_coeffs");
    TRY(lift_launch(x, w.coef, m->xyz_w, m->xyz_b, w.feat, nullptr, B, N, C, s), "xyz_embed");
    PlanScope plan_scope(&m->backbone);
    const bool img16 = m->backbone.precision == 4 && option(OPT_IMGPROJ16) && a.c_total % 32 == 0 && N >= 128 && C % 4 == 0;
    a.out_f16 = img16;
    TRY(ray_lookup_launch(x, w.coef, K, a, w.raw, w.stats_raw, B, N, s), "ray_lookup");
    TRY(adagn_coeffs_launch(w.stats_raw, gecco_lookup_row_tiles(N), N, nullptr, 0, nullptr, nullptr, nullptr, nullptr,
                            w.a_raw, w.o_raw, B, a.c_total, 16, 1e-5f, s), "gn16(img)");
    if (img16) {
        TRY(fold_f16_image_launch(m->img_w, m->img_b, w.a_raw, w.o_raw, w.wfold, w.bfold, B, C, a.c_total, a.c_total, s), "img_feature_proj fold");
        GemmArgs g{};
        g.A = w.raw; g.a_f16 = 1; g.bias = w.bfold; g.bias_bstride = C; g.residual = w.feat; g.C = w.feat; g.stats = w.stats_x;
        g.B = B; g.rows = N; g.K = a.c_total; g.Nout = C; g.lda = a.c_total; g.ldw = a.c_total; g.ldc = C; g.ldr = C;
        g.precision = 2; g.w_img = w.wfold; g.w_img_bstride = (size_t)((C + 127) / 128 * 128) * a.c_total / 2;
        if (!gemm_f16_dma_supported(g)) return fail(-9, "img_feature_proj: shape outside the fp16 streaming kernel");
        TRY(gemm_f32_launch(g, s), "img_feature_proj");
    } else {
        TRY(linear(Lin(w.raw, m->img_w, m->img_b, w.feat, B, N, a.c_total, C).pro(w.a_raw, w.o_raw).plus(w.feat).with_stats(w.stats_x)
                       .weights(m->backbone.precision >= 3 ? 1 : m->backbone.precision, w.wsplit), s), "img_feature_proj");
    }
    rc = st_forward(&m->backbone, w.feat, w.coef + 4 * (size_t)B, w.stats_x, row_tiles_gemm(N), h_in, h_out,
                    w.stats_out, B, N, w.st_ws, w.st_bytes, s);
    if (rc) return rc;
    TRY(adagn_coeffs_launch(w.stats_out, row_tiles_gemm(N), N, nullptr, 0, nullptr, nullptr, nullptr, nullptr, w.a_out,
                            w.o_out, B, C, 16, 1e-5f, s), "gn16(out)");
    TRY(lower_edm_launch(w.feat, x, w.coef, m->out_w, m->out_b, w.a_out, w.o_out, denoised, raw, B, N, C, 1e-5f, s),
        "output_proj+edm");
    return 0;
}
// ... 3 lines not shown
```

### gecco_amd/csrc/kernel_prims.h

```cpp
#pragma once
#include "common.h"

#include <type_traits>
#include <utility>

typedef _Float16 f16x2 __attribute__((ext_vector_type(2)));
typedef _Float16 f16x4 __attribute__((ext_vector_type(4)));
typedef _Float16 f16x8 __attribute__((ext_vector_type(8)));
typedef _Float16 f16x32 __attribute__((ext_vector_type(32)));
typedef __bf16 bf16x2 __attribute__((ext_vector_type(2)));
typedef __bf16 bf16x4 __attribute__((ext_vector_type(4)));
typedef __bf16 bf16x8 __attribute__((ext_vector_type(8)));
typedef float f32x2 __attribute__((ext_vector_type(2)));
typedef unsigned int u32x2 __attribute__((ext_vector_type(2)));
typedef unsigned int u32x4 __attribute__((ext_vector_type(4)));
typedef unsigned int u32x6 __attribute__((ext_vector_type(6)));
typedef int i32x4 __attribute__((ext_vector_type(4)));
typedef int i32x8 __attribute__((ext_vector_type(8)));
typedef short s16x2 __attribute__((ext_vector_type(2)));
typedef short s16x4 __attribute__((ext_vector_type(4)));
typedef unsigned short u16;

template <int... I, class F>
__device__ __forceinline__ void static_for(std::integer_sequence<int, I...>, F&& f) {
    (f(std::integral_constant<int, I>{}), ...);
}
template <int N, class F>
__device__ __forceinline__ void static_for(F&& f) {
    static_for(std::make_integer_sequence<int, N>{}, f);
}
template <int TAG, int... I, class F>
__device__ __forceinline__ void static_for_tag(std::integer_sequence<int, I...>, F&& f) {
    (f(std::integral_constant<int, I>{}, std::integral_constant<int, TAG>{}), ...);
}

constexpr int waitcnt_imm(int vm, int lgkm) { return (vm & 0xF) | (0x7 << 4) | ((lgkm & 0xF) << 8) | ((vm >> 4) << 14); }
template <int N>
__device__ __forceinline__ void wait_vm() { __builtin_amdgcn_s_waitcnt(waitcnt_imm(N, 0xF)); }
template <int N>
__device__ __forceinline__ void wait_vm_lgkm0() { __builtin_amdgcn_s_waitcnt(waitcnt_imm(N, 0)); }

__device__ __forceinline__ void wave_lds_sync() { asm volatile("s_waitcnt lgkmcnt(0)" ::: "memory"); }
__device__ __forceinline__ void lds_barrier() {
    asm volatile("s_waitcnt lgkmcnt(0)" ::: "memory");
    __builtin_amdgcn_s_barrier();
    asm volatile("" ::: "memory");
}

__device__ __forceinline__ void dma16_buf(__amdgpu_buffer_rsrc_t rsrc, unsigned voff, unsigned soff, void* lds_wave_base) {
    __builtin_amdgcn_raw_ptr_buffer_load_lds(rsrc, (__attribute__((address_space(3))) void*)lds_wave_base, 16, voff, soff, 0, 0);
}
__device__ __forceinline__ u32x4 frag(const u16* p) { return *reinterpret_cast<const u32x4*>(p); }

__device__ __forceinline__ unsigned swap_pair(unsigned v) {
    return (unsigned)__builtin_amdgcn_mov_dpp((int)v, 0xB1, 0xF, 0xF, true);
}
__device__ __forceinline__ float wave_sum(float v) {
#pragma unroll
    for (int o = 32; o > 0; o >>= 1) v += __shfl_xor(v, o, 64);
    return v;
}
__device__ __forceinline__ float wave_max(float v) {
#pragma unroll
    for (int o = 32; o > 0; o >>= 1) v = fmaxf(v, __shfl_xor(v, o, 64));
    return v;
}
__device__ __forceinline__ float lanes_sum(float v, int width) {
    for (int o = 1; o < width; o <<= 1) v += __shfl_xor(v, o, 64);
    return v;
}

__device__ __forceinline__ unsigned pack2(float v0, float v1) {
    asm volatile("" : "+v"(v0), "+v"(v1));
    f16x2 p;
    p[0] = (_Float16)v0;
    p[1] = (_Float16)v1;
    return __builtin_bit_cast(unsigned, p);
}
__device__ __forceinline__ float clamp448(float v) { return __builtin_fminf(__builtin_fmaxf(v, -448.f), 448.f); }
__device__ __forceinline__ unsigned pack_fp8x4(float a, float b, float c, float d) {
    int pk = 0;
    pk = __builtin_amdgcn_cvt_pk_fp8_f32(a, b, pk, false);
    pk = __builtin_amdgcn_cvt_pk_fp8_f32(c, d, pk, true);
    return (unsigned)pk;
}

template <bool F16>
__device__ __forceinline__ void split4(const f32x4& x, u32x2& hi, u32x2& lo) {
    if (F16) {
        f16x4 v;
#pragma unroll
        for (int e = 0; e < 4; ++e) v[e] = (_Float16)x[e];
        hi = __builtin_bit_cast(u32x2, v);
        lo = hi;
        return;
    }
    bf16x4 l;
#pragma unroll
    for (int p = 0; p < 2; ++p) {
        const unsigned ua = __float_as_uint(x[2 * p]), uc = __float_as_uint(x[2 * p + 1]);
        hi[p] = __builtin_amdgcn_perm(uc, ua, 0x07060302u);
        l[2 * p] = (__bf16)(x[2 * p] - __uint_as_float(ua & 0xFFFF0000u));
        l[2 * p + 1] = (__bf16)(x[2 * p + 1] - __uint_as_float(uc & 0xFFFF0000u));
    }
    lo = __builtin_bit_cast(u32x2, l);
}
template <bool F16>
__device__ __forceinline__ void split_acc8(const f32x16& s, int e0, u32x4& hi, u32x4& lo) {
    if (F16) {
        f16x8 v;
#pragma unroll
        for (int e = 0; e < 8; ++e) v[e] = (_Float16)s[e0 + e];
        hi = __builtin_bit_cast(u32x4, v);
        lo = hi;
        return;
    }
    u32x4 hb;
    bf16x8 l;
#pragma unroll
    for (int p = 0; p < 4; ++p) {
        const float a = s[e0 + 2 * p], c = s[e0 + 2 * p + 1];
        const unsigned ua = __float_as_uint(a), uc = __float_as_uint(c);
        hb[p] = __builtin_amdgcn_perm(uc, ua, 0x07060302u);
        l[2 * p] = (__bf16)(a - __uint_as_float(ua & 0xFFFF0000u));
        l[2 * p + 1] = (__bf16)(c - __uint_as_float(uc & 0xFFFF0000u));
    }
    hi = hb;
    lo = __builtin_bit_cast(u32x4, l);
}
template <bool F16>
__device__ __forceinline__ f32x16 mfma3(const u32x4& ahi, const u32x4& alo, const u32x4& bhi, const u32x4& blo, f32x16 acc) {
    if (F16) return __builtin_amdgcn_mfma_f32_32x32x16_f16(__builtin_bit_cast(f16x8, ahi), __builtin_bit_cast(f16x8, bhi), acc, 0, 0, 0);
    const bf16x8 ah = __builtin_bit_cast(bf16x8, ahi), al = __builtin_bit_cast(bf16x8, alo);
    const bf16x8 bh = __builtin_bit_cast(bf16x8, bhi), bl = __builtin_bit_cast(bf16x8, blo);
    acc = __builtin_amdgcn_mfma_f32_32x32x16_bf16(al, bh, acc, 0, 0, 0);
    acc = __builtin_amdgcn_mfma_f32_32x32x16_bf16(ah, bl, acc, 0, 0, 0);
    return __builtin_amdgcn_mfma_f32_32x32x16_bf16(ah, bh, acc, 0, 0, 0);
}

__device__ __forceinline__ int e8m0_scale_byte(float m) {
    const int e = (int)(__float_as_uint(m * (16.0f / 15.0f)) >> 23) - 2;
    return m > 0.f ? (e < 1 ? 1 : e) : 127;
}
__device__ __forceinline__ float e8m0_scale_of(int byte) { return __uint_as_float((unsigned)byte << 23); }
__device__ __forceinline__ float absmax32(f16x8 a, f16x8 b, f16x8 c, f16x8 d) {
    auto ab = [](f16x8 v) {
        u32x4 u = __builtin_bit_cast(u32x4, v);
        u &= 0x7fff7fffu;
        return __builtin_bit_cast(f16x8, u);
    };
    f16x8 m = __builtin_elementwise_max(__builtin_elementwise_max(ab(a), ab(b)), __builtin_elementwise_max(ab(c), ab(d)));
    const f16x2 m2 = __builtin_elementwise_max(__builtin_elementwise_max(f16x2{m[0], m[1]}, f16x2{m[2], m[3]}),
// ... 13 lines not shown
```

### gecco_amd/csrc/kernels.h

```cpp
#pragma once
#include <hip/hip_runtime.h>
#include <stddef.h>
#include "weight_images.h"

struct GemmArgs {
    const float* A;
    const float* W;
    const float* bias;
    const float* pro_a;
    const float* pro_o;
    const float* alpha;
    const float* residual;
    float* C;
    float* stats;
    int B, rows, K, Nout;
    int lda, ldw, ldc, ldr;
    int act;
    int precision;
    const void* w_img;
    float* C2;
    const float* W2;
    const float* bias2;
    int n_split, ldc2;
    int a_f16, c_f16;
// ... 16 lines not shown
    int h6;
    int h8_stagger, h8_pair;
};

int gemm_row_tile(int rows);
int gemm_f32_launch(const GemmArgs& g, hipStream_t st);
bool gemm_f32_dma_supported(const GemmArgs& g, int precision = -1);
int gemm_f32_dma_launch(const GemmArgs& g, hipStream_t st);
size_t split_bf16_image_bytes(int Nout, int K);
int split_bf16_tiled_launch(const float* W, void* img, int Nout, int K, int ldw, hipStream_t st);
int split_bf16_tiled_multi_launch(const SplitJobs& jobs, hipStream_t st);

bool gemm_f16_dma_supported(const GemmArgs& g);
int gemm_f16_dma_launch(const GemmArgs& g, hipStream_t st);
size_t split_f16_image_bytes(int Nout, int K);
int fold_f16_image_launch(const float* W, const float* bias, const float* pa, const float* po, void* img, float* bias_out, int B, int Nout, int K,
                          int ldw, hipStream_t st);
int split_f16_tiled_launch(const float* W, void* img, int Nout, int K, int ldw, hipStream_t st);
int split_f16_tiled_multi_launch(const SplitJobs& jobs, hipStream_t st);

struct ChainArgs {
    const float* part_o;
    const float* part_ml;
    int nsplit, H;
    const float* w_stream;
    int two_term;
    const float *b0, *b2, *bkv, *alpha;
    int act;
    const float *n1_scale_w, *n1_scale_b, *n1_bias_w, *n1_bias_b;
    const float *n2_scale_w, *n2_scale_b, *n2_bias_w, *n2_bias_b;
    const float* t;
    int ctx_dim, G;
    float eps;
    float* h_out;
    float* kvh;
    int B;
    int cluster;
    float *x1, *x3;
    unsigned* xu;
    unsigned* flags;
    unsigned short* kv_img;
    int kv_img_bytes;
};
bool inducer_chain_f16_supported(int C, int Wd, int H, int G, int I);
int inducer_chain_f16_launch(const ChainArgs& g, int C, int Wd, hipStream_t st);

struct MlpArgs {
    float* x;
    const float *pro_a, *pro_o;
    const float* w_stream;
    const float *b0, *b2, *alpha;
    int act;
    float* stats;
    int B, rows;
    int stagger;
};
bool mlp_fused_f16_supported(int C, int Wd, int rows);
int mlp_fused_f16_launch(const MlpArgs& g, int C, int Wd, hipStream_t st);

struct UnpoolProjArgs {
    float* x;
    const void* q16;
    const float* kvh;
    const float* w_stream;
    const float* bias;
    float* stats;
    int B, rows, H;
    int stagger;
};
bool unpool_outproj_f16_supported(int C, int H, int rows);
int unpool_outproj_f16_launch(const UnpoolProjArgs& g, int C, hipStream_t st);

struct UnpoolH8Args {
    float* x;
    const void* q16;
    const void* kv_img;
    const void* w_img;
    const float* bias;
    float* stats;
    int B, rows, H;
    int rev;
    int stagger, pair;
};
bool unpool_outproj_h8_supported(int C, int H, int rows);
size_t unpool_outproj_h8_kv_bytes(int B, int C, int H);
int kvh_image_launch(const float* kvh, void* img, int B, int C, int H, hipStream_t st);
int unpool_outproj_h8_launch(const UnpoolH8Args& g, int C, hipStream_t st);

struct MlpWArgs {
    const float* x;
    float* out;
    const float *pro_a, *pro_o;
    const void* w_img;
    const float* alpha;
    int act;
    float* stats;
    int B, rows;
    float* dbg_u;
    int share;
};
bool mlp_fused_w_supported(int C, int Wd, int rows);
size_t mlp_fused_w_image_bytes(int C, int Wd);
struct MlpWImageJob { const float *W0, *b0, *W2, *b2; void* img; const float* alpha; };
int mlp_fused_w_images_launch(const MlpWImageJob* jobs, int n, int C, int Wd, int act, hipStream_t st);
int mlp_fused_w_image_launch(const float* W0, const float* b0, const float* W2, const float* b2, void* img, int C, int Wd, const float* alpha, int act,
                             hipStream_t st);
int mlp_fused_w_launch(const MlpWArgs& g, int C, int Wd, hipStream_t st);

struct TnArgs {
    const float* A;
    const float* Bm;
    float* C;
    int Z, R, N, K, lda, ldb;
    size_t sA, sB;
    int group;
    float* colsum;
    int xcd;
    const float* pro_a;
    const float* pro_o;
    int f16;
    int b_f16;
    int a_f16;
    unsigned* counters;
    float* out;
    float* colsum_out;
};
bool gemm_tn_f16_supported(const TnArgs& g);
int gemm_tn_f16_tiles(int N, int K);
int gemm_tn_f16_launch(const TnArgs& g, hipStream_t st);
bool gemm_x3_areg_supported(const GemmArgs& g);
int gemm_x3_areg_launch(const GemmArgs& g, hipStream_t st);
bool gemm_tn_x3_supported(const TnArgs& g);
int gemm_tn_x3_launch(const TnArgs& g, hipStream_t st);

bool gemm_f16_astat_lo8_supported(int K);
bool gemm_f16_astat_supported(const GemmArgs& g);
int gemm_f16_astat_launch(const GemmArgs& g, hipStream_t st);

size_t h8_image_bytes(int Nout, int K);
int h8_image_multi_launch(const SplitJobs& jobs, hipStream_t st);
bool gemm_h8_astat_supported(const GemmArgs& g);
size_t kvq_image_bytes(int Nout, int K, int lo_cols);
bool gemm_kvq_astat_supported(const GemmArgs& g);
bool kvq_perm48_ok(int hm_hd, int K, int n_first, int n_second);
int gemm_kvq_astat_launch(const GemmArgs& g, hipStream_t st);
bool gemm_h8_train_supported(const GemmArgs& g);
int gemm_h8_train_launch(const GemmArgs& g, hipStream_t st);
bool gemm_astat_train_supported(const GemmArgs& g);
int gemm_astat_train_launch(const GemmArgs& g, hipStream_t st);
int gemm_h8_astat_launch(const GemmArgs& g, hipStream_t st);

size_t h8_w128_image_bytes(int Nout, int K);
bool gemm_h8_areg_supported(const GemmArgs& g);
int gemm_h8_areg_launch(const GemmArgs& g, hipStream_t st);

struct GemmGeneralArgs {
    const float* A;
    const float* B;
    const float* bias;
    float* C;
    int Z, zdiv;
    int M, N, K;
    int lda, ldb, ldc;
    long long sA1, sA2, sB1, sB2, sC1, sC2;
    int a_kmajor, b_kmajor;
    float scale;
};
int gemm_general_launch(const GemmGeneralArgs& g, hipStream_t st);
int reduce_batch_launch(const float* parts, float* out, size_t n, int Z, size_t stride, int accumulate, hipStream_t st);

// ... 221 lines not shown
```

### gecco_amd/csrc/pointwise.hip

```cpp
#include "kernel_prims.h"
#include "kernels.h"
#include "launch_state.h"

#include <stdlib.h>

namespace {

constexpr int STATS_ROWS = 128;

__global__ __launch_bounds__(256) void col_stats_kernel(const float* __restrict__ x, float* __restrict__ stats,
                                                        int rows, int C, int T) {
    __shared__ f32x4 red[2][256];
    const int tile = blockIdx.x % T, b = blockIdx.x / T;
    const int m0 = tile * STATS_ROWS, m1 = min(rows, m0 + STATS_ROWS);
    const float* xb = x + (size_t)b * rows * C;
    if (C % 4 == 0 && C / 4 <= 256) {
        const int c4n = C / 4, RL = 256 / c4n;
        const int c4 = threadIdx.x % c4n, rl = threadIdx.x / c4n;
        f32x4 s1 = {0.f, 0.f, 0.f, 0.f}, s2 = {0.f, 0.f, 0.f, 0.f};
        if (rl < RL) {
            for (int m = m0 + rl; m < m1; m += RL) {
                const f32x4 v = *reinterpret_cast<const f32x4*>(xb + (size_t)m * C + c4 * 4);
                s1 += v;
                s2 += v * v;
// ... 99 lines not shown
        cs[cl] = s1;
        cs[Cp + cl] = s2;
    }
    __syncthreads();
    for (int g = threadIdx.x; g < Gp; g += blockDim.x) {
        double s1 = 0.0, s2 = 0.0;
        for (int cl = g * cpg; cl < (g + 1) * cpg; ++cl) {
            s1 += cs[cl];
            s2 += cs[Cp + cl];
        }
        const double n = (double)rows * cpg;
        const double mean = s1 / n;
        double var = s2 / n - mean * mean;
        var = var < 0.0 ? 0.0 : var;
        gm[g] = mean;
        gm[Gp + g] = 1.0 / sqrt(var + (double)eps);
    }
    __syncthreads();
    for (int cl = threadIdx.x; cl < Cp; cl += blockDim.x) {
        const int g = cl / cpg, c = c0 + cl;
        const float mean = (float)gm[g], rstd = (float)gm[Gp + g];
        float s = 1.f, z = 0.f;
        if (scale_w) {
            s = scale_b[c];
            z = bias_b[c];
            for (int j = 0; j < ctx_dim; ++j) {
                const float tj = t[(size_t)b * ctx_dim + j];
                s += tj * scale_w[(size_t)c * ctx_dim + j];
                z += tj * bias_w[(size_t)c * ctx_dim + j];
            }
        }
        a[(size_t)b * C + c] = s * rstd;
        o[(size_t)b * C + c] = z - s * mean * rstd;
    }
}

__global__ __launch_bounds__(256) void affine_apply_kernel(const float* __restrict__ x, const float* __restrict__ a,
                                                           const float* __restrict__ o, float* __restrict__ y,
                                                           size_t total4, int rowsC4, int C4) {
    for (size_t i = (size_t)blockIdx.x * blockDim.x + threadIdx.x; i < total4; i += (size_t)gridDim.x * blockDim.x) {
        const size_t b = i / rowsC4;
        const int c4 = (int)(i % C4);
        const f32x4 xv = reinterpret_cast<const f32x4*>(x)[i];
        const f32x4 av = reinterpret_cast<const f32x4*>(a)[b * C4 + c4];
        const f32x4 ov = reinterpret_cast<const f32x4*>(o)[b * C4 + c4];
        reinterpret_cast<f32x4*>(y)[i] = xv * av + ov;
    }
}

__global__ __launch_bounds__(256) void affine_cast_f16_kernel(const float* __restrict__ x, const float* __restrict__ a,
                                                              const float* __restrict__ o, _Float16* __restrict__ y,
                                                              size_t total8, int rowsC8, int C8) {
    for (size_t i = (size_t)blockIdx.x * blockDim.x + threadIdx.x; i < total8; i += (size_t)gridDim.x * blockDim.x) {
        const size_t b = i / rowsC8;
        const int c8 = (int)(i % C8);
        const f32x4 x0 = GECCO_NT_LOAD(reinterpret_cast<const f32x4*>(x) + 2 * i);
        const f32x4 x1 = GECCO_NT_LOAD(reinterpret_cast<const f32x4*>(x) + 2 * i + 1);
        const f32x4 a0 = reinterpret_cast<const f32x4*>(a)[(b * C8 + c8) * 2], a1 = reinterpret_cast<const f32x4*>(a)[(b * C8 + c8) * 2 + 1];
        const f32x4 o0 = reinterpret_cast<const f32x4*>(o)[(b * C8 + c8) * 2], o1 = reinterpret_cast<const f32x4*>(o)[(b * C8 + c8) * 2 + 1];
        f16x8 v;
#pragma unroll
        for (int e = 0; e < 4; ++e) {
            float f0 = __builtin_fmaf(x0[e], a0[e], o0[e]), f1 = __builtin_fmaf(x1[e], a1[e], o1[e]);
            asm volatile("" : "+v"(f0), "+v"(f1));
            v[e] = (_Float16)f0;
            v[4 + e] = (_Float16)f1;
        }
        reinterpret_cast<f16x8*>(y)[i] = v;
    }
}

__global__ void edm_coeffs_kernel(const float* __restrict__ sigma, float sd, float* __restrict__ coef, int B) {
    const int b = blockIdx.x * blockDim.x + threadIdx.x;
    if (b >= B) return;
    const float s = sigma[b];
    const float q = s * s + sd * sd;
    coef[4 * b + 0] = sd * sd / q;
    coef[4 * b + 1] = s * sd / sqrtf(q);
    coef[4 * b + 2] = 1.0f / sqrtf(sd * sd + s * s);
    coef[4 * b + 3] = logf(s) / 4.0f;
    coef[4 * B + b] = logf(s) / 4.0f;
}

__global__ __launch_bounds__(256) void lift_kernel(const float* __restrict__ x, const float* __restrict__ coef,
                                                   const float* __restrict__ W, const float* __restrict__ bias,
                                                   float* __restrict__ out, float* __restrict__ stats, int N, int C,
                                                   int T) {
    __shared__ float xs[STATS_ROWS * 3];
    const int tile = blockIdx.x % T, b = blockIdx.x / T;
    const int m0 = tile * STATS_ROWS, m1 = min(N, m0 + STATS_ROWS);
    const float cin = coef ? coef[4 * b + 2] : 1.0f;
    for (int i = threadIdx.x; i < (m1 - m0) * 3; i += blockDim.x) xs[i] = cin * x[((size_t)b * N + m0) * 3 + i];
    __syncthreads();
    for (int c = threadIdx.x; c < C; c += blockDim.x) {
        const float w0 = W[c * 3 + 0], w1 = W[c * 3 + 1], w2 = W[c * 3 + 2], bb = bias ? bias[c] : 0.f;
        float s1 = 0.f, s2 = 0.f;
        for (int m = 0; m < m1 - m0; ++m) {
            const float v = xs[m * 3 + 0] * w0 + xs[m * 3 + 1] * w1 + xs[m * 3 + 2] * w2 + bb;
            out[((size_t)b * N + m0 + m) * C + c] = v;
            s1 += v;
            s2 += v * v;
        }
        if (stats) {
            stats[(((size_t)b * T + tile) * 2 + 0) * C + c] = s1;
            stats[(((size_t)b * T + tile) * 2 + 1) * C + c] = s2;
        }
    }
}

__global__ __launch_bounds__(256) void lower_edm_kernel(const float* __restrict__ feat, const float* __restrict__ x,
                                                        const float* __restrict__ coef, const float* __restrict__ W,
                                                        const float* __restrict__ bias,
                                                        const float* __restrict__ gn_a,
                                                        const float* __restrict__ gn_o, float* __restrict__ out,
                                                        float* __restrict__ raw, int B, int N, int C, float eps) {
    const int lane = threadIdx.x & 63;
    const size_t row = (size_t)blockIdx.x * 4 + (threadIdx.x >> 6);
    if (row >= (size_t)B * N) return;
    const int b = (int)(row / N);
    const float* f = feat + row * C;
    float mean = 0.f, rstd = 1.f;
    if (!gn_a) {
        float s1 = 0.f;
        for (int c = lane; c < C; c += 64) s1 += f[c];
        mean = wave_sum(s1) / C;
        float s2 = 0.f;
        for (int c = lane; c < C; c += 64) {
            const float d = f[c] - mean;
            s2 += d * d;
        }
        rstd = rsqrtf(wave_sum(s2) / C + eps);
    }
    float a0 = 0.f, a1 = 0.f, a2 = 0.f;
    for (int c = lane; c < C; c += 64) {
        const float v = gn_a ? f[c] * gn_a[(size_t)b * C + c] + gn_o[(size_t)b * C + c] : (f[c] - mean) * rstd;
        a0 += v * W[c];
        a1 += v * W[C + c];
        a2 += v * W[2 * C + c];
    }
    a0 = wave_sum(a0);
    a1 = wave_sum(a1);
    a2 = wave_sum(a2);
    if (lane < 3) {
        const float Fv = (lane == 0 ? a0 : lane == 1 ? a1 : a2) + bias[lane];
        if (raw) raw[row * 3 + lane] = Fv;
        if (out) {
            const float cs = coef ? coef[4 * b + 0] : 0.f, co = coef ? coef[4 * b + 1] : 1.f;
            out[row * 3 + lane] = coef ? cs * x[row * 3 + lane] + co * Fv : Fv;
        }
    }
}

template <int CPL>
__global__ __launch_bounds__(256) void lower_edm_v4_kernel(const float* __restrict__ feat, const float* __restrict__ x,
                                                           const float* __restrict__ coef, const float* __restrict__ W,
                                                           const float* __restrict__ bias,
                                                           const float* __restrict__ gn_a,
                                                           const float* __restrict__ gn_o, float* __restrict__ out,
                                                           float* __restrict__ raw, int B, int N, int C, float eps) {
    const int sub = threadIdx.x & 15;
    const size_t rows = (size_t)B * N;
    const size_t row_raw = (size_t)blockIdx.x * 16 + (threadIdx.x >> 4);
    const bool live = row_raw < rows;
    const size_t row = live ? row_raw : rows - 1;
    const int b = (int)(row / N);
    const int nch = C >> 2;
    auto gsum = [](float v) {
        v += __shfl_xor(v, 8, 64);
        v += __shfl_xor(v, 4, 64);
        v += __shfl_xor(v, 2, 64);
        v += __shfl_xor(v, 1, 64);
        return v;
    };
    const f32x4 z = {0.f, 0.f, 0.f, 0.f};
    f32x4 v[CPL];
#pragma unroll
    for (int i = 0; i < CPL; ++i) {
        const int ch = sub + 16 * i;
        v[i] = ch < nch ? *(reinterpret_cast<const f32x4*>(feat + row * C) + ch) : z;
    }
    if (gn_a) {
#pragma unroll
        for (int i = 0; i < CPL; ++i) {
            const int ch = sub + 16 * i;
// ... 264 lines not shown
        for (int i = 0; i < CPL; ++i) {
            const int ch = sub + 16 * i;
            if (ch < nch) {
#pragma unroll
                for (int o = 0; o < P; ++o)
                    if (o < G) {
                        const f32x4 w = reinterpret_cast<const f32x4*>(lw)[o * nch + ch];
                        a[o] += (v[i][0] * w[0] + v[i][1] * w[1]) + (v[i][2] * w[2] + v[i][3] * w[3]);
                    }
            }
        }
        const float r = group_reduce_scatter<P>(a, sub);
        if (live && writer) {
            const int b = (int)(row / N);
            const float Fv = r + (bias ? bias[oi] : 0.f);
            if (raw) raw[row * G + oi] = Fv;
            if (out) {
                const float cs = coef ? coef[4 * b + 0] : 0.f, co = coef ? coef[4 * b + 1] : 1.f;
                out[row * G + oi] = coef ? cs * x[row * G + oi] + co * Fv : Fv;
            }
        }
#pragma unroll
        for (int i = 0; i < CPL; ++i) v[i] = vn[i];
    }
}

}

int stats_row_tile(int rows) { (void)rows; return STATS_ROWS; }

int col_stats_launch(const float* x, float* stats, int B, int rows, int C, hipStream_t st) {
    const int T = (rows + STATS_ROWS - 1) / STATS_ROWS;
    hipLaunchKernelGGL(col_stats_kernel, dim3(B * T), dim3(256), 0, st, x, stats, rows, C, T);
    return (int)hipGetLastError();
}

int adagn_coeffs_launch(const float* stats, int T, int rows, const float* t, int ctx_dim, const float* scale_w,
                        const float* scale_b, const float* bias_w, const float* bias_b, float* a, float* o, int B,
                        int C, int G, float eps, hipStream_t st) {
    if (C % G) return -5;
    int parts = 1;
    while (B * parts * 2 <= 64 && T >= 64 && G % (parts * 2) == 0) parts *= 2;
    const int Cp = C / parts;
    int nsl = 1;
    while (nsl < 8 && (nsl * 2) * Cp <= 1024 && T / (nsl * 2) >= 8) nsl *= 2;
    const int nt = nsl * Cp >= 1024 ? 1024 : (nsl * Cp <= 256 ? 256 : ((nsl * Cp + 63) / 64) * 64);
    const size_t lds = (size_t)(2 * Cp + 2 * (G / parts) + 2 * nsl * Cp) * sizeof(double);
    if (lds > 48 * 1024) {
        if (const hipError_t e = lds_opt_in<adagn_coeffs_kernel>(lds)) return (int)e;
    }
    hipLaunchKernelGGL(adagn_coeffs_kernel, dim3(B, parts), dim3(nt), lds, st, stats, T, rows, t, ctx_dim, scale_w, scale_b,
                       bias_w, bias_b, a, o, C, G, eps, nsl, Cp);
    return (int)hipGetLastError();
}

int affine_apply_launch(const float* x, const float* a, const float* o, float* y, int B, int rows, int C,
                        hipStream_t st) {
    if (C % 4) return -2;
    const size_t total4 = (size_t)B * rows * C / 4;
    const unsigned grid = (unsigned)((total4 + 255) / 256 < 4096 ? (total4 + 255) / 256 : 4096);
    hipLaunchKernelGGL(affine_apply_kernel, dim3(grid ? grid : 1), dim3(256), 0, st, x, a, o, y, total4, rows * C / 4,
                       C / 4);
    return (int)hipGetLastError();
}

int affine_cast_f16_launch(const float* x, const float* a, const float* o, void* y16, int B, int rows, int C,
                           hipStream_t st) {
    if (C % 8) return -2;
    const size_t total8 = (size_t)B * rows * C / 8;
    const unsigned grid = (unsigned)((total8 + 255) / 256 < 8192 ? (total8 + 255) / 256 : 8192);
    hipLaunchKernelGGL(affine_cast_f16_kernel, dim3(grid ? grid : 1), dim3(256), 0, st, x, a, o,
                       static_cast<_Float16*>(y16), total8, rows * C / 8, C / 8);
    return (int)hipGetLastError();
}

int edm_coeffs_launch(const float* sigma, float sigma_data, float* coef, int B, hipStream_t st) {
    hipLaunchKernelGGL(edm_coeffs_kernel, dim3((B + 63) / 64), dim3(64), 0, st, sigma, sigma_data, coef, B);
    return (int)hipGetLastError();
}

int lift_launch(const float* x, const float* coef, const float* W, const float* bias, float* out, float* stats, int B,
                int N, int C, hipStream_t st) {
    const int T = (N + STATS_ROWS - 1) / STATS_ROWS;
    hipLaunchKernelGGL(lift_kernel, dim3(B * T), dim3(256), 0, st, x, coef, W, bias, out, stats, N, C, T);
    return (int)hipGetLastError();
}

int lower_edm_launch(const float* feat, const float* x, const float* coef, const float* W, const float* bias,
                     const float* gn_a, const float* gn_o, float* out, float* raw, int B, int N, int C, float eps,
                     hipStream_t st) {
    const size_t rows = (size_t)B * N;
    const int cpl = (C / 4 + 15) / 16;
    const dim3 g16((unsigned)((rows + 15) / 16));
#define LOWER_V4(CPL)                                                                                              \
    hipLaunchKernelGGL((lower_edm_v4_kernel<CPL>), g16, dim3(256), 0, st, feat, x, coef, W, bias, gn_a, gn_o, out, raw, \
                       B, N, C, eps)
    static const int v5 = env_int("GECCO_LOWER_V5", 1);
    constexpr int RPG = 8;
    if (v5 && C % 4 == 0 && cpl <= 8 && rows >= 16 * RPG * 512) {
        const dim3 g5((unsigned)((rows + 16 * RPG - 1) / (16 * RPG)));
        const size_t lds = (size_t)5 * C * sizeof(float);
#define LOWER_V5(CPL)                                                                                              \
    hipLaunchKernelGGL((lower_edm_v5_kernel<CPL, RPG>), g5, dim3(256), lds, st, feat, x, coef, W, bias, gn_a, gn_o, out, raw, \
                       B, N, C, eps)
        switch (cpl) {
            case 1: LOWER_V5(1); break;
            case 2: LOWER_V5(2); break;
            case 3: LOWER_V5(3); break;
            case 4: LOWER_V5(4); break;
            case 5: LOWER_V5(5); break;
            case 6: LOWER_V5(6); break;
            case 7: LOWER_V5(7); break;
            default: LOWER_V5(8); break;
        }
#undef LOWER_V5
        return (int)hipGetLastError();
    }
    if (C % 4 == 0 && cpl <= 8 && rows > 0) {
        switch (cpl) {
            case 1: LOWER_V4(1); break;
            case 2: LOWER_V4(2); break;
            case 3: LOWER_V4(3); break;
            case 4: LOWER_V4(4); break;
            case 5: LOWER_V4(5); break;
            case 6: LOWER_V4(6); break;
            case 7: LOWER_V4(7); break;
            default: LOWER_V4(8); break;
        }
    } else {
        hipLaunchKernelGGL(lower_edm_kernel, dim3((unsigned)((rows + 3) / 4)), dim3(256), 0, st, feat, x, coef, W, bias,
                           gn_a, gn_o, out, raw, B, N, C, eps);
    }
#undef LOWER_V4
    return (int)hipGetLastError();
}

int geometry_pow2(int G) { return G <= 1 ? 1 : G <= 2 ? 2 : G <= 4 ? 4 : G <= 8 ? 8 : 16; }

int lift_g_launch(const float* x, const float* coef, const float* W, const float* bias, float* out, float* stats, int B,
                  int N, int C, int G, hipStream_t st) {
    if (G < 1 || G > GECCO_MAX_GEOMETRY) return -2;
    const int T = (N + STATS_ROWS - 1) / STATS_ROWS;
    if (B <= 0 || N <= 0) return 0;
    switch (G) {
#define LIFT_G(GG) case GG: hipLaunchKernelGGL((lift_g_kernel<GG>), dim3(B * T), dim3(256), 0, st, x, coef, W, bias, out, stats, N, C, T); break;
        LIFT_G(1) LIFT_G(2) LIFT_G(3) LIFT_G(4) LIFT_G(5) LIFT_G(6) LIFT_G(7) LIFT_G(8)
        LIFT_G(9) LIFT_G(10) LIFT_G(11) LIFT_G(12) LIFT_G(13) LIFT_G(14) LIFT_G(15) LIFT_G(16)
#undef LIFT_G
    }
    return (int)hipGetLastError();
}

namespace {
template <int CPL, int P>
void lower_g_dispatch(bool norm, dim3 grid, size_t lds, hipStream_t st, const float* feat, const float* x, const float* coef,
                      const float* W, const float* bias, float* out, float* raw, int B, int N, int C, int G, float eps, int rpg) {
    if (norm)
        hipLaunchKernelGGL((lower_g_kernel<CPL, P, true>), grid, dim3(256), lds, st, feat, x, coef, W, bias, out, raw, B, N, C, G, eps, rpg);
    else
        hipLaunchKernelGGL((lower_g_kernel<CPL, P, false>), grid, dim3(256), lds, st, feat, x, coef, W, bias, out, raw, B, N, C, G, eps, rpg);
}
template <int CPL>
void lower_g_dispatch_p(int P, bool norm, dim3 grid, size_t lds, hipStream_t st, const float* feat, const float* x,
                        const float* coef, const float* W, const float* bias, float* out, float* raw, int B, int N, int C,
                        int G, float eps, int rpg) {
    switch (P) {
        case 1: lower_g_dispatch<CPL, 1>(norm, grid, lds, st, feat, x, coef, W, bias, out, raw, B, N, C, G, eps, rpg); break;
// ... 25 lines not shown
```

### gecco_amd/csrc/unpool_outproj_h8.hip

```cpp
#include "gemm_dma_common.h"
#include "launch_state.h"
#include "h8_scales.h"

#include <stdlib.h>

#include <utility>

namespace {

constexpr int U_STAGE = 2048;
constexpr int U_PW = 2;
#if defined(UO8_DIAG_NORES) || defined(UO8_DIAG_NOEPI)
constexpr int U_RES = 0;
#else
constexpr int U_RES = 8;
#endif
#ifdef UO8_DIAG_NOEPI
constexpr int U_STORES = 0;
#else
constexpr int U_STORES = 32;
#endif
constexpr int U_TT = 2048;
constexpr float U_LOG2E = 1.4426950408889634f;
constexpr float U_YL_SCALE = H8_AL_SCALE;

constexpr int u_kv_bytes(int HD) { return ((64 * (HD + 8) + ((HD + 31) / 32) * 32 * 72) * 2 + 4095) / 4096 * 4096; }
constexpr int u_tts_floats(int HD) { return 2 * u_kv_bytes(HD) > 4 * U_TT * 4 ? 2 * u_kv_bytes(HD) / 4 : 4 * U_TT; }

#ifdef UO8_STAMPS
__device__ unsigned long long g_uo8_stamps[2048 * 4];
__device__ unsigned long long g_uo8_epi[2048 * 4];
#define UTICK() __builtin_amdgcn_s_memtime()
#define USTAMP(i)                                                                                                \
    do {                                                                                                         \
        if (threadIdx.x == 0 && blockIdx.x < 2048) g_uo8_stamps[blockIdx.x * 4 + (i)] = __builtin_amdgcn_s_memtime(); \
    } while (0)
#else
#define USTAMP(i)
#endif

#define U_MFMA16(a, b, c) __builtin_amdgcn_mfma_f32_32x32x16_f16(a, b, c, 0, 0, 0)
#ifdef UO8_DIAG_NOMFMA
#define UG_MFMA16(a, b, c) keep16(a, b, c)
#define UG_MFMA8(a, b, c, sa, sb) keep8(a, b, c)
#else
#define UG_MFMA16(a, b, c) __builtin_amdgcn_mfma_f32_32x32x16_f16(a, b, c, 0, 0, 0)
#define UG_MFMA8(a, b, c, sa, sb) __builtin_amdgcn_mfma_scale_f32_32x32x64_f8f6f4(a, b, c, 0, 0, 0, sa, 0, sb)
#endif

__device__ __forceinline__ float max_halves(float v) {
    const auto a = __builtin_amdgcn_permlane32_swap(__builtin_bit_cast(unsigned, v), __builtin_bit_cast(unsigned, v), false, false);
    return fmaxf(__uint_as_float(a[0]), __uint_as_float(a[1]));
}
__device__ __forceinline__ float sum_halves(float v) {
    const auto a = __builtin_amdgcn_permlane32_swap(__builtin_bit_cast(unsigned, v), __builtin_bit_cast(unsigned, v), false, false);
    return __uint_as_float(a[0]) + __uint_as_float(a[1]);
}

__global__ __launch_bounds__(256) void kvh_image_kernel(const float* __restrict__ kvh, u16* __restrict__ img, int C, int H, int HD, int kvb) {
    extern __shared__ __attribute__((aligned(16))) float smem[];
    u16* buf = reinterpret_cast<u16*>(smem);
    const int b = blockIdx.x / H, hh = blockIdx.x % H;
    const int KS = HD + 8, nk = 64 * KS, CH = HD / 4;
    for (int i = threadIdx.x; i < kvb / 16; i += 256) reinterpret_cast<u32x4*>(buf)[i] = u32x4{0u, 0u, 0u, 0u};
    __syncthreads();
    const float* src = kvh + (size_t)b * 64 * 2 * C + hh * HD;
    for (int i = threadIdx.x; i < 64 * CH; i += 256) {
        const int key = i / CH, ch = i % CH;
        const f32x4 kf = *reinterpret_cast<const f32x4*>(src + (size_t)key * 2 * C + ch * 4);
        const f32x4 vf = *reinterpret_cast<const f32x4*>(src + (size_t)key * 2 * C + C + ch * 4);
        const int pos = (key & ~15) + 8 * ((key >> 2) & 1) + 4 * ((key >> 3) & 1) + (key & 3);
#pragma unroll
        for (int e = 0; e < 4; ++e) {
            buf[key * KS + ch * 4 + e] = __builtin_bit_cast(u16, (_Float16)kf[e]);
            buf[nk + (ch * 4 + e) * 72 + pos] = __builtin_bit_cast(u16, (_Float16)vf[e]);
        }
    }
    __syncthreads();
    u32x4* dst = reinterpret_cast<u32x4*>(img + (size_t)blockIdx.x * (kvb / 2));
    for (int i = threadIdx.x; i < kvb / 16; i += 256) dst[i] = reinterpret_cast<const u32x4*>(buf)[i];
}

template <int NG, int HD, int NS>
__global__ __launch_bounds__(256, NG > 6 ? 1 : 2) void unpool_outproj_h8_kernel(UnpoolH8Args g) {
    constexpr int C = 64 * NG, H = C / HD, NKT = 2 * NG, NC = HD / 16, DT = (HD + 31) / 32;
    constexpr int KS = HD + 8, VS = 72, KVB = u_kv_bytes(HD), PK = KVB / 4096;
    static_assert(C % HD == 0 && HD % 16 == 0 && HD <= 64, "head dims 16 .. 64");
    constexpr int TTSF = u_tts_floats(HD);
    static_assert(NS >= 4 && NS <= NKT, "lookahead NS - 1 >= 3 stages; the residual pieces land inside their tile");
    extern __shared__ __attribute__((aligned(16))) float smem[];
    float* ring = smem;
    float* tts = ring + NS * U_STAGE;
    float* bias_lds = tts + TTSF;
    float* red = bias_lds + C;

    const int tilesM = g.rows / 128;
    const int bid = g.rev ? (int)gridDim.x - 1 - (int)blockIdx.x : (int)blockIdx.x;
    const int b = bid / tilesM, rt = bid % tilesM, m0 = rt * 128;
    const int tid = threadIdx.x, lane = tid & 63;
    const int wave = __builtin_amdgcn_readfirstlane(tid >> 6);
    const int r = lane & 31, h = lane >> 5;

    USTAMP(0);
    for (int n = tid; n < C; n += 256) bias_lds[n] = g.bias ? g.bias[n] : 0.f;
    if (g.stagger > 0 && (((blockIdx.x >> 3) / g.pair) & 1)) {
        const unsigned long long t0 = __builtin_amdgcn_s_memtime();
        while (__builtin_amdgcn_s_memtime() - t0 < (unsigned long long)g.stagger) __builtin_amdgcn_s_sleep(8);
    }
    __syncthreads();

    const __amdgpu_buffer_rsrc_t wrsrc = __builtin_amdgcn_make_buffer_rsrc(const_cast<void*>(g.w_img), 0, 0x7fffffff, 0x00020000);
    const unsigned wvoff = (unsigned)(wave * U_PW * 256 + lane * 4) * 4u;
    const unsigned soff_last = (unsigned)(NG * NKT - 1) * (U_STAGE * 4u);
    unsigned soff = 0;
    int islot = 0;
    auto issue = [&]() {
#pragma unroll
        for (int p = 0; p < U_PW; ++p) dma16_buf(wrsrc, wvoff + p * 1024u, soff, ring + islot * U_STAGE + (wave * U_PW + p) * 256);
        soff = soff < soff_last ? soff + U_STAGE * 4u : soff_last;
        islot = islot + 1 == NS ? 0 : islot + 1;
    };
#pragma unroll
    for (int p = 0; p < NS - 1; ++p) issue();

    f16x8 fa[2 * NG][2];
    i32x8 alo[NG];
#ifdef UO8_DIAG_NOATT
#pragma unroll
    for (int i = 0; i < 2 * NG; ++i)
#pragma unroll
        for (int c = 0; c < 2; ++c)
#pragma unroll
            for (int e = 0; e < 8; ++e) fa[i][c][e] = (_Float16)(0.01f * (float)((lane + i + c + e) & 63));
#pragma unroll
    for (int i = 0; i < NG; ++i)
#pragma unroll
        for (int e = 0; e < 8; ++e) alo[i][e] = 0x20202020 + lane + e;
#else
    {
        const __amdgpu_buffer_rsrc_t kvrsrc = __builtin_amdgcn_make_buffer_rsrc(
            const_cast<char*>(static_cast<const char*>(g.kv_img) + (size_t)b * H * KVB), 0, 0x7fffffff, 0x00020000);
        char* kvbuf = reinterpret_cast<char*>(tts);
        const unsigned kvoff = (unsigned)(wave * PK * 1024 + lane * 16);
        auto kv_issue = [&](int hh) {
#pragma unroll
            for (int p = 0; p < PK; ++p)
                dma16_buf(kvrsrc, kvoff + p * 1024u, (unsigned)hh * KVB, kvbuf + (hh & 1) * KVB + (wave * PK + p) * 1024);
        };
        const _Float16* q16 = reinterpret_cast<const _Float16*>(g.q16);
        u32x4 qf[2][NC];
        auto q_load = [&](int hh, int set) {
            const _Float16* qr = q16 + (((size_t)b * H + hh) * g.rows + m0 + wave * 32 + r) * HD + 8 * h;
#pragma unroll
            for (int c = 0; c < NC; ++c) qf[set][c] = *reinterpret_cast<const u32x4*>(qr + c * 16);
        };
        kv_issue(0);
        q_load(0, 0);
        if (H > 1) {
            kv_issue(1);
            q_load(1, 1);
        }
        const float scale = U_LOG2E * rsqrtf((float)HD);
        static_for(std::make_integer_sequence<int, H>{}, [&](auto HH) {
            constexpr int hh = decltype(HH)::value, set = hh & 1;
            if constexpr (hh == 0 && H > 1) dma::wait_vm_lgkm0<PK + NC>();
            else dma::wait_vm_lgkm0<0>();
            __builtin_amdgcn_s_barrier();
            if constexpr (hh >= 1 && hh + 1 < H) {
                kv_issue(hh + 1);
                q_load(hh + 1, set ^ 1);
            }
// ... 26 lines not shown
            const f32x2 mx2 = {mx, mx};
            float ls = 0.f;
#pragma unroll
            for (int kt = 0; kt < 2; ++kt)
#pragma unroll
                for (int e = 0; e < 16; e += 2) {
                    const f32x2 t = f32x2{sc[kt][e], sc[kt][e + 1]} - mx2;
                    sc[kt][e] = __builtin_amdgcn_exp2f(t[0]);
                    sc[kt][e + 1] = __builtin_amdgcn_exp2f(t[1]);
                    ls += sc[kt][e];
                    ls += sc[kt][e + 1];
                }
            ls = sum_halves(ls);
            const float inv = 1.0f / ls;
            f16x8 pf[4];
#pragma unroll
            for (int kt = 0; kt < 2; ++kt)
#pragma unroll
                for (int sg = 0; sg < 2; ++sg)
#pragma unroll
                    for (int e = 0; e < 8; ++e) pf[2 * kt + sg][e] = (_Float16)sc[kt][8 * sg + e];
#pragma unroll
            for (int c16 = 0; c16 < 4; ++c16) asm volatile("" : "+v"(pf[c16]));
            f32x16 O[DT];
#pragma unroll
            for (int dt = 0; dt < DT; ++dt)
#pragma unroll
                for (int e = 0; e < 16; ++e) O[dt][e] = 0.f;
#pragma unroll
            for (int c16 = 0; c16 < 4; ++c16)
#pragma unroll
                for (int dt = 0; dt < DT; ++dt) {
                    const u32x4 vf = *reinterpret_cast<const u32x4*>(Vt + (dt * 32 + r) * VS + c16 * 16 + 8 * h);
                    O[dt] = U_MFMA16(__builtin_bit_cast(f16x8, vf), pf[c16], O[dt]);
                }
            static_for(std::make_integer_sequence<int, 2 * DT>{}, [&](auto PP) {
                constexpr int pp = decltype(PP)::value, dt = pp >> 1, p = pp & 1;
                if constexpr (32 * dt + 16 * p < HD) {
                    constexpr int ks = (hh * HD + 32 * dt + 16 * p) / 16;
                    f16x8 hv;
                    float lo[8];
                    const f32x2 inv2 = {inv, inv}, ysc2 = {U_YL_SCALE, U_YL_SCALE};
#pragma unroll
                    for (int e = 0; e < 8; e += 2) {
                        f32x2 v = f32x2{O[dt][8 * p + e], O[dt][8 * p + e + 1]} * inv2;
                        v[0] = h8_clamp(v[0]);
                        v[1] = h8_clamp(v[1]);
                        asm volatile("" : "+v"(v));
                        hv[e] = (_Float16)v[0];
                        hv[e + 1] = (_Float16)v[1];
                        const f32x2 d = (v - f32x2{(float)hv[e], (float)hv[e + 1]}) * ysc2;
                        lo[e] = clamp448(d[0]);
                        lo[e + 1] = clamp448(d[1]);
                    }
                    fa[ks >> 1][ks & 1] = hv;
                    alo[ks >> 2][4 * ((ks >> 1) & 1) + 2 * (ks & 1) + 0] = (int)pack_fp8x4(lo[0], lo[1], lo[2], lo[3]);
                    alo[ks >> 2][4 * ((ks >> 1) & 1) + 2 * (ks & 1) + 1] = (int)pack_fp8x4(lo[4], lo[5], lo[6], lo[7]);
                    asm volatile("" : "+v"(fa[ks >> 1][ks & 1]));
                    asm volatile("" : "+v"(alo[ks >> 2][4 * ((ks >> 1) & 1) + 2 * (ks & 1) + 0]), "+v"(alo[ks >> 2][4 * ((ks >> 1) & 1) + 2 * (ks & 1) + 1]));
                }
            });
        });
    }
#endif
    USTAMP(1);

    int boffc[2];
#pragma unroll
    for (int c = 0; c < 2; ++c) boffc[c] = r * 16 + (((2 * h + c) ^ ((r >> 2) & 3)) << 2);
    i32x8 fbA[2], fbB[2];
    auto load_f = [&](const float* sub, i32x8(&f)[2]) {
#pragma unroll
        for (int c = 0; c < 2; ++c) {
            const float* pc = sub + boffc[c];
#pragma unroll
            for (int j = 0; j < 2; ++j) {
                const u32x4 v = *reinterpret_cast<const u32x4*>(pc + j * 512);
#pragma unroll
                for (int e = 0; e < 4; ++e) f[j][4 * c + e] = (int)v[e];
            }
        }
    };

    float* tt = tts + wave * U_TT;
    float* xw = g.x + ((size_t)b * g.rows + m0 + wave * 32) * C;
    const __amdgpu_buffer_rsrc_t xrsrc = __builtin_amdgcn_make_buffer_rsrc(xw, 0, 0x7fffffff, 0x00020000);
    auto issue_res = [&](int ct) {
        int ln = lane;
        asm volatile("" : "+v"(ln));
        const unsigned v0 = (unsigned)(((ln >> 4) * C + 4 * (ln & 15)) * 4);
#pragma unroll
        for (int it = 0; it < 8; ++it) dma16_buf(xrsrc, v0 + (unsigned)(it * 4 * C * 4), (unsigned)(ct * 64 * 4), tt + it * 256);
    };

    f32x16 acc[2];
#ifdef UO8_STAMPS
    unsigned long long t_e1 = 0, t_e2 = 0;
#endif
    auto epilogue = [&](int ct) {
        const int n0 = ct * 64;
#ifdef UO8_STAMPS
        const unsigned long long te0 = UTICK();
#endif
        int ln = lane;
        asm volatile("" : "+v"(ln));
        const int r = ln & 31, h = ln >> 5;
        const float* tl = tt + 4 * h * 64 + r;
        const unsigned vo = (unsigned)((4 * h * C + r) * 4);
#pragma unroll
        for (int j = 0; j < 2; ++j) {
            const float bc = bias_lds[n0 + 32 * j + r];
            float s1 = 0.f, s2 = 0.f;
#pragma unroll
            for (int qe = 0; qe < 16; ++qe) {
                const int row = 8 * (qe >> 2) + (qe & 3);
                const float v = (acc[j][qe] + bc) + tl[row * 64 + 32 * j];
                __builtin_amdgcn_raw_buffer_store_b32(__builtin_bit_cast(int, v), xrsrc, vo, (unsigned)((row * C + n0 + 32 * j) * 4), 0);
                s1 += v;
                s2 = __builtin_fmaf(v, v, s2);
            }
            if (g.stats) {
                const float t1 = sum_halves(s1), t2 = sum_halves(s2);
                if (ln < 32) {
                    red[(wave * 2 + 0) * 64 + 32 * j + r] = t1;
                    red[(wave * 2 + 1) * 64 + 32 * j + r] = t2;
                }
            }
        }
        asm volatile("s_waitcnt lgkmcnt(0)" ::: "memory");
#ifdef UO8_STAMPS
        t_e2 += UTICK() - te0;
#endif
    };
    auto write_stats = [&](int ct) {
        float* dst = g.stats + (((size_t)b * tilesM + rt) * 2) * C + ct * 64 + lane;
#pragma unroll
        for (int which = 0; which < 2; ++which) {
            float t = 0.f;
#pragma unroll
            for (int w = 0; w < 4; ++w) t += red[(w * 2 + which) * 64 + lane];
            dst[(size_t)which * C] = t;
        }
    };

    dma::wait_vm_lgkm0<0>();
    __builtin_amdgcn_s_barrier();
    int slot = 0;
    load_f(ring, fbA);
    float one = H8_AH_DIV;
    const f32x16 zero16 = {0.f, 0.f, 0.f, 0.f, 0.f, 0.f, 0.f, 0.f, 0.f, 0.f, 0.f, 0.f, 0.f, 0.f, 0.f, 0.f};
    auto stage = [&](auto KT, int ct) {
        constexpr int kt = decltype(KT)::value, gq = kt >> 1;
        constexpr bool lst = (kt & 1) != 0;
        constexpr int young = (NS - 3) * U_PW;
        if constexpr (kt == 0) {
            if (ct == 0) dma::wait_vm_lgkm0<young>();
            else dma::wait_vm_lgkm0<young + U_STORES>();
        } else if constexpr (kt <= NS - 3) {
            if (ct == 0) dma::wait_vm_lgkm0<young + U_RES>();
            else dma::wait_vm_lgkm0<young + U_RES + U_STORES>();
        } else if constexpr (kt == NS - 2) {
            dma::wait_vm_lgkm0<young + U_RES>();
        } else {
            dma::wait_vm_lgkm0<young>();
        }
#pragma unroll
        for (int j = 0; j < 2; ++j) asm volatile("" : "+v"(fbA[j]));
        __builtin_amdgcn_s_barrier();
        if constexpr (kt == 0) {
            if (g.stats && ct > 0 && wave == ((ct - 1) & 3)) write_stats(ct - 1);
        }
        issue();
#if !defined(UO8_DIAG_NORES) && !defined(UO8_DIAG_NOEPI)
        if constexpr (kt == 0) issue_res(ct);
#endif
        const float* cur = ring + slot * U_STAGE;
        slot = slot + 1 == NS ? 0 : slot + 1;
        const float* nxt = ring + slot * U_STAGE;
        load_f(cur + 1024, fbB);
        if constexpr (!lst) {
#pragma unroll
            for (int c = 0; c < 2; ++c)
#pragma unroll
                for (int j = 0; j < 2; ++j) {
                    const i32x4 wc = c == 0 ? __builtin_shufflevector(fbA[j], fbA[j], 0, 1, 2, 3) : __builtin_shufflevector(fbA[j], fbA[j], 4, 5, 6, 7);
                    acc[j] = UG_MFMA16(fa[2 * gq][c], __builtin_bit_cast(f16x8, wc), (kt == 0 && c == 0) ? zero16 : acc[j]);
                }
        } else {
            i32x8 a8;
#pragma unroll
            for (int t = 0; t < 2; ++t)
#pragma unroll
                for (int c = 0; c < 2; ++c) {
                    const f16x8 v = fa[2 * gq + t][c];
                    s16x2 p0 = {0, 0}, p1 = {0, 0};
                    p0 = __builtin_amdgcn_cvt_scalef32_pk_fp8_f16(p0, f16x2{v[0], v[1]}, one, false);
                    p0 = __builtin_amdgcn_cvt_scalef32_pk_fp8_f16(p0, f16x2{v[2], v[3]}, one, true);
                    p1 = __builtin_amdgcn_cvt_scalef32_pk_fp8_f16(p1, f16x2{v[4], v[5]}, one, false);
                    p1 = __builtin_amdgcn_cvt_scalef32_pk_fp8_f16(p1, f16x2{v[6], v[7]}, one, true);
                    a8[4 * t + 2 * c] = __builtin_bit_cast(int, p0);
                    a8[4 * t + 2 * c + 1] = __builtin_bit_cast(int, p1);
                }
#pragma unroll
            for (int j = 0; j < 2; ++j) acc[j] = UG_MFMA8(a8, fbA[j], acc[j], H8_SC_AH, H8_SC_WL);
        }
        load_f(nxt, fbA);
        if constexpr (!lst) {
#pragma unroll
            for (int c = 0; c < 2; ++c)
#pragma unroll
                for (int j = 0; j < 2; ++j) {
                    const i32x4 wc = c == 0 ? __builtin_shufflevector(fbB[j], fbB[j], 0, 1, 2, 3) : __builtin_shufflevector(fbB[j], fbB[j], 4, 5, 6, 7);
                    acc[j] = UG_MFMA16(fa[2 * gq + 1][c], __builtin_bit_cast(f16x8, wc), acc[j]);
                }
        } else {
#pragma unroll
            for (int j = 0; j < 2; ++j) acc[j] = UG_MFMA8(alo[gq], fbB[j], acc[j], H8_SC_AL, H8_SC_W8);
        }
    };
    for (int ct = 0; ct < NG; ++ct) {
        asm volatile("" : "+s"(one));
        static_for(std::make_integer_sequence<int, NKT>{}, [&](auto KT) { stage(KT, ct); });
#ifdef UO8_DIAG_NOEPI
        if (acc[0][0] == 123.456f) epilogue(ct);
#else
        epilogue(ct);
#endif
    }
    USTAMP(2);
#ifdef UO8_STAMPS
    if (threadIdx.x == 0 && blockIdx.x < 2048) {
        g_uo8_epi[blockIdx.x * 4 + 0] = t_e1;
        g_uo8_epi[blockIdx.x * 4 + 1] = t_e2;
    }
#endif
    if (g.stats) {
        __builtin_amdgcn_s_barrier();
        if (wave == ((NG - 1) & 3)) write_stats(NG - 1);
    }
    dma::wait_vm_lgkm0<0>();
    USTAMP(3);
}

template <int NG, int HD, int NS>
int uo8_launch_t(const UnpoolH8Args& g, hipStream_t st) {
    constexpr int C = 64 * NG;
    constexpr size_t lds = ((size_t)NS * U_STAGE + u_tts_floats(HD) + C + 4 * 2 * 64) * sizeof(float);
    static_assert(lds <= 80 * 1024 || NG > 6, "two blocks per CU");
    if (const hipError_t e = lds_opt_in<unpool_outproj_h8_kernel<NG, HD, NS>>(lds)) return (int)e;
    hipLaunchKernelGGL((unpool_outproj_h8_kernel<NG, HD, NS>), dim3(g.B * (g.rows / 128)), dim3(256), lds, st, g);
    return (int)hipGetLastError();
}

}

bool unpool_outproj_h8_supported(int C, int H, int rows) {
    if (rows < 128 || rows % 128 || H <= 0 || C % H) return false;
    const int hd = C / H;
    static const int k512 = env_int("GECCO_UO8_K512", 1);
    return (C == 128 && hd == 16) || (C == 256 && hd == 32) || (C == 384 && hd == 48) || (C == 512 && hd == 64 && k512);
}

size_t unpool_outproj_h8_kv_bytes(int B, int C, int H) { return (size_t)B * H * u_kv_bytes(C / H); }

int kvh_image_launch(const float* kvh, void* img, int B, int C, int H, hipStream_t st) {
    const int hd = C / H;
    if (hd % 16 || hd > 64) return -9;
    hipLaunchKernelGGL(kvh_image_kernel, dim3(B * H), dim3(256), (size_t)u_kv_bytes(hd), st, kvh, static_cast<u16*>(img), C, H, hd, u_kv_bytes(hd));
    return (int)hipGetLastError();
}

int unpool_outproj_h8_launch(const UnpoolH8Args& g0, int C, hipStream_t st) {
    if (!unpool_outproj_h8_supported(C, g0.H, g0.rows)) return -9;
    static const int rev = env_int("GECCO_UO8_REV", 1);
    static const int stagger = env_int("GECCO_UO8_STAGGER", 0);
    static const int pair = env_int("GECCO_UO8_PAIR", 32);
    UnpoolH8Args g = g0;
    g.rev = rev != 0;
    g.stagger = g.B * (g.rows / 128) >= 512 ? stagger : 0;
    g.pair = pair > 0 ? pair : 32;
    switch (C) {
        case 128: return uo8_launch_t<2, 16, 4>(g, st);
        case 256: return uo8_launch_t<4, 32, 5>(g, st);
        case 512: return uo8_launch_t<8, 64, 4>(g, st);
        default: return uo8_launch_t<6, 48, 5>(g, st);
    }
}
```

### gecco_amd/hip_ops.py

```python
from __future__ import annotations

import contextlib
import ctypes as C
import itertools
import os
import threading
from typing import Mapping, Sequence

import torch
from torch import Tensor

from . import _lib
from ._lib import GeccoAdaGN, GeccoLayer, GeccoLinearLift, GeccoMLP, GeccoSetTransformer, check

GN_EPS = 1e-5

PRECISIONS = {"fp32": 0, "bf16x3": 1, "fp16": 2, "mixed": 3, "w2": 4}
_default_precision = os.environ.get("GECCO_PRECISION", "fp32")


def set_default_precision(name: str) -> None:
    global _default_precision
    if name not in PRECISIONS:
        raise ValueError(f"precision must be one of {sorted(PRECISIONS)}")
# ... 263 lines not shown
    lib = _lib.load()
    B, T, G = a_img.shape[:3]
    rows, K, n = T * 128, G * 64, W.shape[0]
    if out is None:
        out = torch.empty(B, rows, n, device=a_img.device, dtype=torch.float32)
    stats = torch.empty(B, rows // 128, 2, n, device=a_img.device, dtype=torch.float32) if want_stats else None
    if wsplit is None:
        wsplit = _ws((n + 127) // 128 * 128 * K * 4, a_img.device)
    check(lib.gecco_linear_h8_areg_f32(C.c_void_p(a_img.data_ptr()), None if image_ready else _ptr(W), _ptr(b), _ptr(residual), _ptr(out),
                                       _ptr(stats), B, rows, K, n, C.c_void_p(wsplit.data_ptr()), _stream()), "gecco_linear_h8_areg_f32")
    return (out, stats) if want_stats else out


def decode_split_image(img: Tensor) -> Tensor:
    Bn, T, KT = img.shape[:3]
    f = (img.to(torch.int32) << 16).view(torch.float32)
    v = f[:, :, :, 0] + f[:, :, :, 1]
    rows = torch.arange(128, device=img.device)
    swap = ((rows >> 3) & 1).bool()
    v = torch.where(swap[None, None, None, :, None], torch.cat([v[..., 8:], v[..., :8]], dim=-1), v)
    return v.permute(0, 1, 3, 2, 4).reshape(Bn, T * 128, KT * 16)


def decode_h8_image(img: Tensor) -> Tensor:
    Bn, T, G = img.shape[:3]
    hi = img[..., :16384].contiguous().view(torch.float16).reshape(Bn, T, G, 4, 2, 2, 2, 32, 8).double()
    lo = img[..., 16384:].contiguous().view(torch.float8_e4m3fn).reshape(Bn, T, G, 4, 2, 2, 32, 16).double()
    hi = hi.permute(0, 1, 3, 7, 2, 4, 6, 5, 8)
    lo = lo.permute(0, 1, 3, 6, 2, 4, 5, 7)
    return hi.reshape(Bn, T * 128, G * 64) + lo.reshape(Bn, T * 128, G * 64) * 2.0 ** -11


def mlp_fused_f16(x: Tensor, pro: tuple[Tensor, Tensor], W0: Tensor, b0: Tensor | None, W2: Tensor, b2: Tensor | None,
                  act_alpha: Tensor | None = None, normalized: bool = True, want_stats: bool = False,
                  wsplit: Tensor | None = None, image_ready: bool = False, stats: Tensor | None = None):
    lib = _lib.load()
    B, rows, Cc = x.shape
    width = W0.shape[0]
    if stats is None and want_stats:
        stats = torch.empty(B, rows // 128, 2, Cc, device=x.device, dtype=torch.float32)
    if wsplit is None:
        wsplit = _ws(4 * Cc * width, x.device)
    act = 0 if act_alpha is None else (1 if normalized else 2)
    check(lib.gecco_mlp_fused_f16(_ptr(x), _ptr(pro[0]), _ptr(pro[1]), None if image_ready else _ptr(W0), _ptr(b0),
                                  None if image_ready else _ptr(W2), _ptr(b2), _ptr(act_alpha),
                                  act, _ptr(stats), B, rows, Cc, width, C.c_void_p(wsplit.data_ptr()), _stream()),
          "gecco_mlp_fused_f16")
    return x, stats


def unpool_outproj_f16(x: Tensor, q16: Tensor, kvh: Tensor, W: Tensor, bias: Tensor | None, H: int, want_stats: bool = False,
                       wsplit: Tensor | None = None, image_ready: bool = False, stats: Tensor | None = None):
    lib = _lib.load()
    B, rows, Cc = x.shape
    if stats is None and want_stats:
        stats = torch.empty(B, rows // 128, 2, Cc, device=x.device, dtype=torch.float32)
    if wsplit is None:
        wsplit = _ws(2 * Cc * Cc, x.device)
    check(lib.gecco_unpool_outproj_f16(_ptr(x), _ptr16(q16), _ptr(kvh), None if image_ready else _ptr(W), _ptr(bias), _ptr(stats), B, rows, Cc, H,
                                       C.c_void_p(wsplit.data_ptr()), _stream()), "gecco_unpool_outproj_f16")
    return x, stats


def mlp_fused_w(x: Tensor, pro: tuple[Tensor, Tensor], W0: Tensor, b0: Tensor | None, W2: Tensor, b2: Tensor | None,
                act_alpha: Tensor | None = None, normalized: bool = True, act: str | int | None = None, want_stats: bool = False,
                wsplit: Tensor | None = None, image_ready: bool = False, stats: Tensor | None = None, out: Tensor | None = None,
                dbg_u: Tensor | None = None):
    lib = _lib.load()
    B, rows, Cc = x.shape
    width = W0.shape[0]
    if out is None:
        out = x
    if stats is None and want_stats:
        stats = torch.empty(B, rows // 128, 2, Cc, device=x.device, dtype=torch.float32)
    if wsplit is None:
        wsplit = _ws(lib.gecco_mlp_fused_w_wsplit_bytes(Cc, width), x.device)
    check(lib.gecco_mlp_fused_w(_ptr(x), _ptr(out), _ptr(pro[0]), _ptr(pro[1]), None if image_ready else _ptr(W0), _ptr(b0),
                                None if image_ready else _ptr(W2), _ptr(b2), _ptr(act_alpha), act_code(act_alpha, normalized, act),
                                _ptr(stats), B, rows, Cc, width, C.c_void_p(wsplit.data_ptr()), _ptr(dbg_u), _stream()), "gecco_mlp_fused_w")
    return out, stats


def unpool_outproj_h8(x: Tensor, q16: Tensor, kvh: Tensor, W: Tensor, bias: Tensor | None, H: int, want_stats: bool = False,
                      wsplit: Tensor | None = None, image_ready: bool = False, stats: Tensor | None = None):
    lib = _lib.load()
    B, rows, Cc = x.shape
    if stats is None and want_stats:
        stats = torch.empty(B, rows // 128, 2, Cc, device=x.device, dtype=torch.float32)
    if wsplit is None:
        wsplit = _ws(lib.gecco_unpool_outproj_h8_wsplit_bytes(B, Cc, H), x.device)
    check(lib.gecco_unpool_outproj_h8(_ptr(x), _ptr16(q16), _ptr(kvh), None if image_ready else _ptr(W), _ptr(bias), _ptr(stats), B, rows, Cc, H,
                                      C.c_void_p(wsplit.data_ptr()), _stream()), "gecco_unpool_outproj_h8")
    return x, stats


def unpool_attn_h8img(q16: Tensor, kvh: Tensor, H: int) -> Tensor:
    lib = _lib.load()
    B, _, N, hd = q16.shape
    Cc = H * hd
    out = torch.empty(B, N // 128, Cc // 64, 24576, device=q16.device, dtype=torch.uint8)
    check(lib.gecco_unpool_attn_h8img(_ptr16(q16), _ptr(kvh), C.c_void_p(out.data_ptr()), B, N, Cc, H, _stream()), "gecco_unpool_attn_h8img")
    return out


def affine_cast_f16(x: Tensor, a: Tensor, o: Tensor, out: Tensor | None = None) -> Tensor:
    lib = _lib.load()
    B, rows, Cc = x.shape
    out = torch.empty(B, rows, Cc, device=x.device, dtype=torch.float16) if out is None else out
    check(lib.gecco_affine_cast_f16(_ptr(x), _ptr(a), _ptr(o), _ptr16(out), B, rows, Cc, _stream()), "gecco_affine_cast_f16")
    return out


def pool_attn_f16in(KV16: Tensor, inducers: Tensor, H: int, head_major: bool = False) -> Tensor:
    lib = _lib.load()
    if head_major:
        B, _, N, hd = KV16.shape
        Cc = H * hd
    else:
        B, N, C2 = KV16.shape
        Cc = C2 // 2
    I = inducers.shape[-2]
    merged = torch.empty(B, I, Cc, device=KV16.device, dtype=torch.float32)
    nb = lib.gecco_pool_attn_workspace_bytes(B, N, Cc, H, I)
    ws = _ws(nb, KV16.device)
    check(lib.gecco_pool_attn_f16in(_ptr16(KV16), _ptr(inducers), _ptr(merged), B, N, Cc, H, I, int(head_major),
                                    C.c_void_p(ws.data_ptr()), nb, _stream()), "gecco_pool_attn_f16in")
    return merged


def lift0_fold(kv_w: Tensor, in_proj_w: Tensor, in_proj_b: Tensor | None, lift_w: Tensor, lift_b: Tensor | None, a1: Tensor, o1: Tensor,
               H: int) -> Tensor:
    lib = _lib.load()
    B, Cc = a1.shape
    mc = torch.empty(B, 3 * Cc, 4, device=a1.device, dtype=torch.float32)
    check(lib.gecco_lift0_fold_f32(_ptr(kv_w), _ptr(in_proj_w), _ptr(in_proj_b), _ptr(lift_w), _ptr(lift_b), _ptr(a1), _ptr(o1), _ptr(mc),
                                   B, Cc, H, _stream()), "gecco_lift0_fold_f32")
    return mc


def lift0_rows(x: Tensor, coef: Tensor, mc: Tensor, col0: int, ncols: int, head_dim: int = 0, f16: bool = True) -> Tensor:
    lib = _lib.load()
    B, N, _ = x.shape
    Cc = mc.shape[1] // 3
    shape = (B, ncols // head_dim, N, head_dim) if head_dim else (B, N, ncols)
    out = torch.empty(*shape, device=x.device, dtype=torch.float16 if f16 else torch.float32)
    check(lib.gecco_lift0_rows(_ptr(x), _ptr(coef), _ptr(mc), C.c_void_p(out.data_ptr()), col0, ncols, head_dim, int(f16), B, N, Cc,
                               _stream()), "gecco_lift0_rows")
    return out


def lift0_pool(x: Tensor, coef: Tensor, mc: Tensor, inducers: Tensor, H: int) -> Tensor:
    lib = _lib.load()
    B, N, _ = x.shape
    Cc = mc.shape[1] // 3
    merged = torch.empty(B, 64, Cc, device=x.device, dtype=torch.float32)
    nb = lib.gecco_pool_attn_workspace_bytes(B, N, Cc, H, 64)
    ws = _ws(nb, x.device)
    check(lib.gecco_lift0_pool_f32(_ptr(x), _ptr(coef), _ptr(mc), _ptr(inducers), _ptr(merged), B, N, Cc, H, C.c_void_p(ws.data_ptr()), nb,
                                   _stream()), "gecco_lift0_pool_f32")
    return merged


def unpool_attn_f16io(q16: Tensor, kvh: Tensor, H: int, out: Tensor | None = None, head_major: bool = False) -> Tensor:
    lib = _lib.load()
    if head_major:
        B, _, N, hd = q16.shape
        Cc = H * hd
    else:
        B, N, Cc = q16.shape
    out = torch.empty(B, N, Cc, device=q16.device, dtype=torch.float16) if out is None else out
    check(lib.gecco_unpool_attn_f16io(_ptr16(q16), _ptr(kvh), _ptr16(out), B, N, Cc, H, kvh.shape[1], int(head_major),
                                      _stream()), "gecco_unpool_attn_f16io")
    return out


def linear_pair(A: Tensor, W1: Tensor, b1: Tensor | None, W2: Tensor, b2: Tensor | None,
                pro: tuple[Tensor, Tensor] | None = None, out: tuple[Tensor, Tensor] | None = None,
                precision: str = "fp32", w_image: Tensor | None = None) -> tuple[Tensor, Tensor]:
    lib = _lib.load()
    B, rows, K = A.shape
    n1, n2 = W1.shape[0], W2.shape[0]
    c1, c2 = out if out is not None else (torch.empty(B, rows, n1, device=A.device, dtype=torch.float32),
                                          torch.empty(B, rows, n2, device=A.device, dtype=torch.float32))
    if w_image is not None:
        assert precision in ("bf16x3", "fp16")
        wsplit, W1, W2 = w_image, None, None
    else:
        wsplit = _ws(((n1 + 127) // 128 + (n2 + 127) // 128) * 128 * K * 4, A.device) if precision != "fp32" else None
    check(lib.gecco_linear_pair_f32(_ptr(A), _ptr(W1), _ptr(b1), n1, _ptr(c1), _ptr(W2), _ptr(b2), n2, _ptr(c2),
                                    _ptr(pro[0]) if pro else None, _ptr(pro[1]) if pro else None, B, rows, K,
                                    PRECISIONS[precision], C.c_void_p(wsplit.data_ptr()) if wsplit is not None else None,
                                    _stream()), "gecco_linear_pair_f32")
    return c1, c2


def pool_attn(KV: Tensor, inducers: Tensor, H: int, precision: str = "fp32") -> Tensor:
    lib = _lib.load()
    pr = PRECISIONS[precision]
    B, N, C2 = KV.shape
    Cc = C2 // 2
    I = inducers.shape[-2]
    merged = torch.empty(B, I, Cc, device=KV.device, dtype=torch.float32)
    nb = lib.gecco_pool_attn_workspace_bytes(B, N, Cc, H, I)
    ws = _ws(nb, KV.device)
    check(lib.gecco_pool_attn_ex_f32(_ptr(KV), _ptr(inducers), _ptr(merged), B, N, Cc, H, I, pr,
                                     C.c_void_p(ws.data_ptr()), nb, _stream()), "gecco_pool_attn_ex_f32")
    return merged


def unpool_attn(q: Tensor, kvh: Tensor, H: int, precision: str = "fp32") -> Tensor:
    lib = _lib.load()
    pr = PRECISIONS[precision]
    B, N, Cc = q.shape
    I = kvh.shape[1]
    out = torch.empty_like(q)
    check(lib.gecco_unpool_attn_ex_f32(_ptr(q), _ptr(kvh), _ptr(out), B, N, Cc, H, I, pr, _stream()),
          "gecco_unpool_attn_ex_f32")
    return out


def edm_coeffs(sigma: Tensor, sigma_data: float = 1.0) -> Tensor:
    lib = _lib.load()
    B = sigma.numel()
    coef = torch.empty(5 * B, device=sigma.device, dtype=torch.float32)
    check(lib.gecco_edm_coeffs_f32(_ptr(sigma), sigma_data, _ptr(coef), B, _stream()), "gecco_edm_coeffs_f32")
    return coef


MAX_GEOMETRY_DIM = 16


def check_geometry_dim(G: int) -> None:
    if not 1 <= G <= MAX_GEOMETRY_DIM:
        raise ValueError(f"the HIP LinearLift supports geometry_dim 1 .. {MAX_GEOMETRY_DIM}, got {G}")


def lift(x: Tensor, coef: Tensor | None, W: Tensor, bias: Tensor | None, want_stats: bool = False):
    lib = _lib.load()
    B, N, G = x.shape
    assert W.shape[1] == G, (W.shape, x.shape)
    Cc = W.shape[0]
    out = torch.empty(B, N, Cc, device=x.device, dtype=torch.float32)
    stats = torch.empty(B, lib.gecco_stats_row_tiles(N), 2, Cc, device=x.device, dtype=torch.float32) if want_stats else None
    if G == 3:
        check(lib.gecco_lift_f32(_ptr(x), _ptr(coef), _ptr(W), _ptr(bias), _ptr(out), _ptr(stats), B, N, Cc, _stream()),
              "gecco_lift_f32")
    else:
        check_geometry_dim(G)
        check(lib.gecco_lift_g_f32(_ptr(x), _ptr(coef), _ptr(W), _ptr(bias), _ptr(out), _ptr(stats), B, N, Cc, G, _stream()),
              "gecco_lift_g_f32")
    return (out, stats) if want_stats else out


def lower_edm(feat: Tensor, x: Tensor | None, coef: Tensor | None, W: Tensor, bias: Tensor | None,
              gn: tuple[Tensor, Tensor] | None = None, want_raw: bool = False, eps: float = GN_EPS, do_norm: bool = True):
    lib = _lib.load()
    B, N, Cc = feat.shape
    G = W.shape[0]
    out = torch.empty(B, N, G, device=feat.device, dtype=torch.float32)
    raw = torch.empty_like(out) if want_raw else None
    if G == 3 and (do_norm or gn is not None):
        check(lib.gecco_lower_edm_f32(_ptr(feat), _ptr(x), _ptr(coef), _ptr(W), _ptr(bias), _ptr(gn[0]) if gn else None,
                                      _ptr(gn[1]) if gn else None, _ptr(out), _ptr(raw), B, N, Cc, eps, _stream()),
              "gecco_lower_edm_f32")
    else:
        assert gn is None, "the GroupNorm lower form is 3-wide (RayNetwork)"
        check_geometry_dim(G)
        check(lib.gecco_lower_edm_g_f32(_ptr(feat), _ptr(x), _ptr(coef), _ptr(W), _ptr(bias), _ptr(out), _ptr(raw), B, N, Cc, G,
                                        int(do_norm), eps, _stream()), "gecco_lower_edm_g_f32")
    return (out, raw) if want_raw else out


def _adagn_from(p: Mapping[str, Tensor], pre: str) -> GeccoAdaGN:
    return _adagn_struct(p[pre + "scale.weight"], p[pre + "scale.bias"], p[pre + "bias.weight"], p[pre + "bias.bias"])


def _mlp_from(p: Mapping[str, Tensor], pre: str) -> GeccoMLP:
    return GeccoMLP(_ptr(p[pre + "0.weight"]), _ptr(p[pre + "0.bias"]), _ptr(p.get(pre + "1.alpha")),
                    _ptr(p[pre + "2.weight"]), _ptr(p[pre + "2.bias"]))


def layer_table(p: Mapping[str, Tensor], pre: str) -> GeccoLayer:
    return GeccoLayer(
        _adagn_from(p, pre + "broadcast_norm."), _ptr(p[pre + "broadcast.pool.inducers"]),
        _ptr(p[pre + "broadcast.pool.kv_proj.weight"]), _ptr(p[pre + "broadcast.pool.out_proj.weight"]),
        _adagn_from(p, pre + "broadcast.norm_1."), _mlp_from(p, pre + "broadcast.mlp."),
        _adagn_from(p, pre + "broadcast.norm_2."), _ptr(p[pre + "broadcast.unpool.in_proj_weight"]),
        _ptr(p[pre + "broadcast.unpool.in_proj_bias"]), _ptr(p[pre + "broadcast.unpool.out_proj.weight"]),
        _ptr(p[pre + "broadcast.unpool.out_proj.bias"]), _adagn_from(p, pre + "mlp_norm."), _mlp_from(p, pre + "mlp."))


class SetTransformerPlan:

    def __init__(self, p: Mapping[str, Tensor], pre: str, H: int, I: int = 64, G: int = 32, normalized: bool = True,
                 precision: str | None = None, act: int | None = None, options: Mapping[str, int] | None = None):
        self.lib = _lib.load()
        self.precision = precision or _default_precision
        if self.precision not in PRECISIONS:
            raise ValueError(f"precision must be one of {sorted(PRECISIONS)}")
        self.p = p
        L = 0
        while f"{pre}layers.{L}.mlp.0.weight" in p:
            L += 1
        if L == 0:
            raise KeyError(f"no layers under prefix {pre!r}")
        w0 = p[f"{pre}layers.0.mlp.0.weight"]
        self.width, self.C = w0.shape
        self.L, self.H, self.I, self.G = L, H, I, G
        self.ctx_dim = p[f"{pre}layers.0.mlp_norm.scale.weight"].shape[1]
        self.device = w0.device
        self._layers = (GeccoLayer * L)(*[layer_table(p, f"{pre}layers.{i}.") for i in range(L)])
        if act is None:
            act = (ACT_GAUSS if normalized else ACT_GAUSS_RAW) if f"{pre}layers.0.mlp.1.alpha" in p else ACT_RELU
        self.act = act
        self.table = GeccoSetTransformer(L, self.C, H, I, self.ctx_dim, G, self.width, act,
                                         PRECISIONS[self.precision], 0, 0, 0, self._layers)
        for name, value in (options or {}).items():
            _pin_option(self.table, name, value)
        self._ws: dict[tuple[int, int], Tensor] = {}
        self.images = _ImageState()

    def set_option(self, name: str, value: int) -> None:
        _pin_option(self.table, name, value)
        self.images.changed()

# ... 438 lines not shown
```

### include/gecco_hip.h

```cpp
#ifndef GECCO_HIP_H
#define GECCO_HIP_H
#include <stddef.h>
#include <stdint.h>
#ifdef __cplusplus
extern "C" {
#endif

#define GECCO_ABI_VERSION 14

int gecco_abi_version(void);
const char* gecco_build_arch(void);
const char* gecco_last_error(void);

typedef struct GeccoAdaGN {
    const float* scale_w;
    const float* scale_b;
    const float* bias_w;
    const float* bias_b;
} GeccoAdaGN;

typedef struct GeccoMLP {
    const float* w0;
    const float* b0;
    const float* alpha;
// ... 49 lines not shown
int gecco_linear_actbwd_ok(int rows, int K, int Nout, int precision);
size_t gecco_linear_actbwd_tiles(int B, int rows, int Nout);
int gecco_linear_actbwd_f32(const float* A, const float* W, const float* u, const float* alpha, int kind, const float* residual,
                            float* C, float* agrad, int B, int rows, int K, int Nout, int precision, void* wsplit, void* stream);
int gecco_linear_dotstats_f32(const float* A, const float* W, const float* dot_x, float* C, float* stats, int B, int rows, int K, int Nout,
                              int precision, void* wsplit, void* stream);
int gecco_linear_dotstats_a16_f32(const void* A16, const float* W, const float* dot_x, const float* residual, float* C, float* stats, int B,
                                  int rows, int K, int Nout, void* wsplit, void* stream);
int gecco_linear_act_keep_f32(const float* A, const float* W, const float* bias, const float* alpha, int act, float* pre_out,
                              float* C, int B, int rows, int K, int Nout, int precision, void* wsplit, void* stream);
int gecco_linear_act_keep_pro_f32(const float* A, const float* W, const float* bias, const float* pro_a, const float* pro_o,
                                  const float* alpha, int act, float* pre_out, float* C, int B, int rows, int K, int Nout,
                                  int precision, void* wsplit, void* stream);
int gecco_linear_act_keep_h16(const float* A, const float* W, const float* bias, const float* pro_a, const float* pro_o,
                              const float* alpha, int act, float* pre_out, void* C16out, int B, int rows, int K, int Nout, void* wsplit,
                              void* stream);

size_t gecco_h8_image_bytes(int Nout, int K);
int gecco_linear_h8_train_ok(int rows, int K, int Nout);
int gecco_h8_images_f32(const GeccoSplitJob* jobs, int n, void* stream);
int gecco_linear_h8_train_f32(const float* x, const float* pro_a, const float* pro_o, const float* W1, const float* bias1, int Nout1, float* C1,
                              const float* W2, const float* bias2, int Nout2, float* C2, const float* alpha, int act, float* pre_out, int B,
                              int rows, int K, void* wsplit, void* stream);

size_t gecco_astat16_image_bytes(int Nout, int K);
int gecco_linear_astat16_ok(int rows, int K, int Nout);
int gecco_astat16_images_f32(const GeccoSplitJob* jobs, int n, void* stream);
int gecco_linear_astat16_f32(const float* x, const float* pro_a, const float* pro_o, const float* W1, const float* bias1, int Nout1, float* C1,
                             const float* W2, const float* bias2, int Nout2, float* C2, const float* residual, int transposed, int B, int rows,
                             int K, void* wsplit, void* stream);
int gecco_linear_astat16_keep(const float* x, const float* pro_a, const float* pro_o, const float* W, const float* bias, const float* alpha,
                              int act, float* pre_out, void* C16out, int B, int rows, int K, int Nout, void* wsplit, void* stream);
int gecco_linear_astat16_keep_y16(const float* x, const float* pro_a, const float* pro_o, const float* W, const float* bias, const float* alpha,
                                  int act, float* pre_out, void* C16out, void* y16, int B, int rows, int K, int Nout, void* wsplit,
                                  void* stream);
int gecco_linear_astat16_actbwd(const float* dy, const float* W, const float* u, const float* alpha, int kind, float* C, float* agrad, int B,
                                int rows, int K, int Nout, void* wsplit, void* stream);
int gecco_linear_astat16_actbwd_h16(const float* dy, const float* W, const float* u, const float* alpha, int kind, void* C16, float* agrad,
                                    int B, int rows, int K, int Nout, void* wsplit, void* stream);

int gecco_col_stats_f32(const float* x, float* stats, int B, int rows, int C, void* stream);
int gecco_stats_row_tiles(int rows);

int gecco_adagn_coeffs_f32(const float* stats, int T, int rows, const float* t, int ctx_dim, const GeccoAdaGN* p,
                           float* a, float* o, int B, int C, int G, float eps, void* stream);
int gecco_affine_apply_f32(const float* x, const float* a, const float* o, float* y, int B, int rows, int C,
                           void* stream);
int gecco_adagn_f32(const float* x, const float* t, int ctx_dim, const GeccoAdaGN* p, float* y, int B, int rows,
                    int C, int G, float eps, void* ws, size_t ws_bytes, void* stream);
size_t gecco_adagn_workspace_bytes(int B, int rows, int C);

int gecco_linear_f16io(const void* A, const float* W, const float* bias, const float* alpha, const float* residual,
                       void* C, float* stats, int B, int rows, int K, int Nout, int act, int a_f16, int c_f16,
                       void* wsplit, void* stream);
int gecco_linear_pair_f16io(const void* A, const float* W1, const float* bias1, int Nout1, void* C1, const float* W2,
                            const float* bias2, int Nout2, void* C2, int B, int rows, int K, void* wsplit,
                            void* stream);
int gecco_linear_astat_f16(const float* x, const float* pro_a, const float* pro_o, const float* W1, const float* bias1,
                           int Nout1, void* C1, const float* W2, const float* bias2, int Nout2, void* C2,
                           const float* alpha, int act, int B, int rows, int K, int head_dim, void* wsplit,
                           void* stream);
int gecco_linear_kvq_f16(const float* x, const float* pro_a, const float* pro_o, const float* W1, const float* bias1, int Nout1,
                         void* C1, const float* W2, const float* bias2, int Nout2, void* C2, int B, int rows, int K, int head_dim,
                         int lo_begin, int lo_end, void* wsplit, void* stream);
int gecco_linear_kvq_y16_f16(const float* x, const float* pro_a, const float* pro_o, const float* W1, const float* bias1, int Nout1,
                             void* C1, const float* W2, const float* bias2, int Nout2, void* C2, void* y16, int B, int rows, int K,
                             int head_dim, int lo_begin, int lo_end, void* wsplit, void* stream);
int gecco_linear_h8_img_f32(const float* x, const float* pro_a, const float* pro_o, const float* W, const float* bias,
                            const float* alpha, int act, void* c_img, int image_kind, int B, int rows, int K, int Nout,
                            void* wsplit, void* stream);
int gecco_linear_h8_areg_f32(const void* a_img, const float* W, const float* bias, const float* residual, float* C, float* stats,
                             int B, int rows, int K, int Nout, void* wsplit, void* stream);
int gecco_mlp_fused_f16(float* x, const float* pro_a, const float* pro_o, const float* W0, const float* b0, const float* W2,
                        const float* b2, const float* alpha, int act, float* stats, int B, int rows, int C, int width,
                        void* wsplit, void* stream);
int gecco_unpool_outproj_f16(float* x, const void* q16, const float* kvh, const float* W, const float* bias, float* stats,
                             int B, int rows, int C, int H, void* wsplit, void* stream);
int gecco_mlp_fused_w(const float* x, float* out, const float* pro_a, const float* pro_o, const float* W0, const float* b0, const float* W2,
                      const float* b2, const float* alpha, int act, float* stats, int B, int rows, int C, int width, void* wsplit, float* dbg_u,
                      void* stream);
size_t gecco_mlp_fused_w_wsplit_bytes(int C, int width);
int gecco_unpool_outproj_h8(float* x, const void* q16, const float* kvh, const float* W, const float* bias, float* stats,
                            int B, int rows, int C, int H, void* wsplit, void* stream);
size_t gecco_unpool_outproj_h8_wsplit_bytes(int B, int C, int H);
int gecco_unpool_attn_h8img(const void* q16, const float* kvh, void* out_img, int B, int N, int C, int H, void* stream);
int gecco_affine_cast_f16(const float* x, const float* a, const float* o, void* y16, int B, int rows, int C,
                          void* stream);
int gecco_pool_attn_f16in(const void* KV16, const float* inducers, float* merged, int B, int N, int C, int H, int I,
                          int head_major, void* ws, size_t ws_bytes, void* stream);
int gecco_unpool_attn_f16io(const void* q16, const float* kvh, void* out16, int B, int N, int C, int H, int I,
                            int head_major, void* stream);

int gecco_pool_attn_f32(const float* KV, const float* inducers, float* merged, int B, int N, int C, int H, int I,
                        void* ws, size_t ws_bytes, void* stream);
int gecco_pool_attn_ex_f32(const float* KV, const float* inducers, float* merged, int B, int N, int C, int H, int I,
                           int precision, void* ws, size_t ws_bytes, void* stream);
size_t gecco_pool_attn_workspace_bytes(int B, int N, int C, int H, int I);
int gecco_lift0_fold_f32(const float* kv_w, const float* q_w, const float* q_b, const float* lift_w, const float* lift_b, const float* a1,
                         const float* o1, float* mc, int B, int C, int H, void* stream);
int gecco_lift0_rows(const float* x, const float* coef, const float* mc, void* out, int col0, int ncols, int head_dim, int out_f16,
                     int B, int N, int C, void* stream);
int gecco_lift0_pool_f32(const float* x, const float* coef, const float* mc, const float* inducers, float* merged, int B, int N, int C,
                         int H, void* ws, size_t ws_bytes, void* stream);

int gecco_pool_attn_lse_f32(const void* ws, size_t ws_bytes, float* lse, int B, int N, int C, int H, int I, void* stream);
int gecco_pool_attn_bwd_partials(int B, int N, int H);
int gecco_pool_attn_bwd_f32(const float* KV, const float* inducers, const float* merged, const float* lse, const float* dO,
                            float* dKV, float* dQ_partials, int B, int N, int C, int H, int I, void* stream);
int gecco_unpool_attn_bwd_partials(int B, int N, int H);
int gecco_unpool_attn_bwd_f32(const float* q, const float* kvh, const float* dO, float* dq, float* dkv_partials, int B, int N,
                              int C, int H, int I, void* stream);
int gecco_pool_attn_bwd_ex_f32(const float* KV, const float* inducers, const float* merged, const float* lse, const float* dO,
                               float* dKV, float* dQ_partials, int B, int N, int C, int H, int I, int precision, void* stream);
int gecco_unpool_attn_bwd_ex_f32(const float* q, const float* kvh, const float* dO, float* dq, float* dkv_partials, int B, int N,
                                 int C, int H, int I, int precision, void* stream);

int gecco_unpool_attn_f32(const float* q, const float* kvh, float* out, int B, int N, int C, int H, int I,
                          void* stream);
int gecco_unpool_attn_ex_f32(const float* q, const float* kvh, float* out, int B, int N, int C, int H, int I,
                             int precision, void* stream);

int gecco_edm_coeffs_f32(const float* sigma, float sigma_data, float* coef, int B, void* stream);
int gecco_lift_f32(const float* x, const float* coef, const float* W, const float* bias, float* out, float* stats,
                   int B, int N, int C, void* stream);
int gecco_lower_edm_f32(const float* feat, const float* x, const float* coef, const float* W, const float* bias,
                        const float* gn_a, const float* gn_o, float* out, float* raw, int B, int N, int C, float eps,
                        void* stream);


int gecco_set_transformer_fwd_f32(const GeccoSetTransformer* st, float* x, const float* t, const float* stats_x,
                                  int stats_T, const float* const* h_in, float* const* h_out, float* stats_out,
                                  int B, int N, void* ws, size_t ws_bytes, void* stream);
size_t gecco_set_transformer_workspace_bytes(const GeccoSetTransformer* st, int B, int N);

typedef struct GeccoLinearLift {
    GeccoSetTransformer inner;
    const float* lift_w;
    const float* lift_b;
    const float* lower_w;
    const float* lower_b;
    float sigma_data;
} GeccoLinearLift;

int gecco_linear_lift_fwd_f32(const GeccoLinearLift* m, const float* x, const float* sigma, float* denoised,
                              float* raw, const float* const* h_in, float* const* h_out, int B, int N, void* ws,
                              size_t ws_bytes, void* stream);
size_t gecco_linear_lift_workspace_bytes(const GeccoLinearLift* m, int B, int N);

#define GECCO_MAX_GEOMETRY_DIM 16
int gecco_lift_g_f32(const float* x, const float* coef, const float* W, const float* bias, float* out, float* stats,
                     int B, int N, int C, int G, void* stream);
int gecco_lower_edm_g_f32(const float* feat, const float* x, const float* coef, const float* W, const float* bias, float* out,
                          float* raw, int B, int N, int C, int G, int do_norm, float eps, void* stream);

typedef struct GeccoLinearLiftG {
    GeccoLinearLift base;
    int geometry_dim;
    int do_norm;
} GeccoLinearLiftG;

int gecco_linear_lift_g_fwd_f32(const GeccoLinearLiftG* m, const float* x, const float* sigma, float* denoised,
                                float* raw, const float* const* h_in, float* const* h_out, int B, int N, void* ws,
                                size_t ws_bytes, void* stream);
size_t gecco_linear_lift_g_workspace_bytes(const GeccoLinearLiftG* m, int B, int N);


// ... 258 lines not shown
```

Before: 31.09 million points/s.

## Recompute lifted features in the unpool out-proj epilogue instead of storing them

When the lift0 route and the h8 unpool+out_proj path are both on, the lift kernel now computes only the statistics and no longer writes the B x N x C fp32 feature tensor. The first layer's unpool out-proj kernel rebuilds the residual from the 3-D points, the EDM input coefficient and the lift weights staged in LDS, instead of DMA-loading residual tiles. This removes one full activation write and read. The cost is a little extra per-element arithmetic in the epilogue and more template variants. Contraction is disabled in the lift helpers so the recomputed values match the stored ones bit for bit.

```diff
diff --git a/gecco_amd/_lib.py b/gecco_amd/_lib.py
--- a/gecco_amd/_lib.py
+++ b/gecco_amd/_lib.py
@@ -99,6 +99,7 @@
     "gecco_mlp_fused_f16": (i, [vp, vp, vp, vp, vp, vp, vp, vp, i, vp, i, i, i, i, vp, vp]),
     "gecco_unpool_outproj_f16": (i, [vp, vp, vp, vp, vp, vp, i, i, i, i, vp, vp]),
     "gecco_unpool_outproj_h8": (i, [vp, vp, vp, vp, vp, vp, i, i, i, i, vp, vp]),
+    "gecco_unpool_outproj_h8_points": (i, [vp] * 10 + [i, i, i, i, vp, vp]),
     "gecco_mlp_fused_w": (i, [vp, vp, vp, vp, vp, vp, vp, vp, vp, i, vp, i, i, i, i, vp, vp, vp]),
     "gecco_mlp_fused_w_wsplit_bytes": (sz, [i, i]),
     "gecco_unpool_outproj_h8_wsplit_bytes": (sz, [i, i, i]),
diff --git a/gecco_amd/csrc/api_common.h b/gecco_amd/csrc/api_common.h
--- a/gecco_amd/csrc/api_common.h
+++ b/gecco_amd/csrc/api_common.h
@@ -33,8 +33,7 @@
 inline int row_tiles_gemm(int rows) { const int bm = gemm_row_tile(rows); return (rows + bm - 1) / bm; }
 inline int row_tiles_stats(int rows) { const int bm = stats_row_tile(rows); return (rows + bm - 1) / bm; }
 
-enum { OPT_ASTAT = 0, OPT_CHAIN = 1, OPT_HEADMAJOR = 2, OPT_MLPFUSED = 3, OPT_UNPOOLFUSED = 4, OPT_LO8 = 5, OPT_ACTIMG = 6, OPT_H8 = 7, OPT_KVQ64 = 8, OPT_H8AREG = 9, OPT_CHAIN2 = 10, OPT_UNPOOLH8 = 11, OPT_MLPW = 12, OPT_CHAINCL = 13, OPT_H6 = 14, OPT_KVFOLD = 15, OPT_MLPWSHARE = 16, OPT_KVQPERM = 17, OPT_IMGPROJ16 = 18, OPT_LIFT0 = 19, OPT_COUNT = 20 };
-enum { OPT_LIFT0_HI = OPT_LIFT0 + 1 };
+enum { OPT_ASTAT = 0, OPT_CHAIN = 1, OPT_HEADMAJOR = 2, OPT_MLPFUSED = 3, OPT_UNPOOLFUSED = 4, OPT_LO8 = 5, OPT_ACTIMG = 6, OPT_H8 = 7, OPT_KVQ64 = 8, OPT_H8AREG = 9, OPT_CHAIN2 = 10, OPT_UNPOOLH8 = 11, OPT_MLPW = 12, OPT_CHAINCL = 13, OPT_H6 = 14, OPT_KVFOLD = 15, OPT_MLPWSHARE = 16, OPT_KVQPERM = 17, OPT_IMGPROJ16 = 18, OPT_LIFT0 = 19, OPT_LIFT0_HI = 20, OPT_LIFT0FRONT = 21, OPT_COUNT = 22 };
 int option(int which);
 
 int make_lookup_args(const GeccoReparam* rp, const GeccoPyramid* pyr, LookupArgs* a);
diff --git a/gecco_amd/csrc/api_linear.hip b/gecco_amd/csrc/api_linear.hip
--- a/gecco_amd/csrc/api_linear.hip
+++ b/gecco_amd/csrc/api_linear.hip
@@ -428,16 +428,23 @@
 
 int gecco_unpool_outproj_h8(float* x, const void* q16, const float* kvh, const float* W, const float* bias, float* stats,
                             int B, int rows, int C, int H, void* wsplit, void* stream) {
-    if (!x || !q16 || !kvh || !wsplit) return fail(-1, "unpool_outproj_h8: null argument");
+    return gecco_unpool_outproj_h8_points(x, q16, kvh, W, bias, stats, nullptr, nullptr, nullptr, nullptr, B, rows, C, H, wsplit, stream);
+}
+
+int gecco_unpool_outproj_h8_points(float* x, const void* q16, const float* kvh, const float* W, const float* bias, float* stats,
+                                   const float* pts, const float* coef, const float* lift_w, const float* lift_b, int B, int rows, int C,
+                                   int H, void* wsplit, void* stream) {
+    if (!x || !q16 || !kvh || !wsplit || (pts && !lift_w)) return fail(-1, "unpool_outproj_h8: null argument");
     if (!unpool_outproj_h8_supported(C, H, rows))
         return fail(-2, "unpool_outproj_h8: needs (C, head dim) in {(128, 16), (256, 32), (384, 48)}, rows %% 128 == 0");
     hipStream_t s = (hipStream_t)stream;
     if (W) TRY(build_images(h8_image_multi_launch, wsplit, C, s, {W, C, C, H8_ATTN_ORDER}), "unpool_outproj_h8(split)");
     void* kvimg = static_cast<char*>(wsplit) + h8_image_bytes(C, C);
     TRY(kvh_image_launch(kvh, kvimg, B, C, H, s), "unpool_outproj_h8(k | v image)");
-    UnpoolH8Args ua{};
+    UnpoolH8PtsArgs ua{};
     ua.x = x; ua.q16 = q16; ua.kv_img = kvimg; ua.w_img = wsplit; ua.bias = bias; ua.stats = stats; ua.B = B; ua.rows = rows; ua.H = H;
-    TRY(unpool_outproj_h8_launch(ua, C, s), "unpool_outproj_h8");
+    ua.pts = pts; ua.coef = coef; ua.lift_w = lift_w; ua.lift_b = lift_b;
+    TRY(pts ? unpool_outproj_h8_points_launch(ua, C, s) : unpool_outproj_h8_launch(ua, C, s), "unpool_outproj_h8");
     return 0;
 }
 
diff --git a/gecco_amd/csrc/api_model_ops.hip b/gecco_amd/csrc/api_model_ops.hip
--- a/gecco_amd/csrc/api_model_ops.hip
+++ b/gecco_amd/csrc/api_model_ops.hip
@@ -222,6 +222,7 @@
 
 int gecco_lift_f32(const float* x, const float* coef, const float* W, const float* bias, float* out, float* stats,
                    int B, int N, int C, void* stream) {
+    if (!x || !W || !(out || stats)) return fail(-1, "lift: null argument");
     TRY(lift_launch(x, coef, W, bias, out, stats, B, N, C, (hipStream_t)stream), "lift");
     return 0;
 }
diff --git a/gecco_amd/csrc/api_network.hip b/gecco_amd/csrc/api_network.hip
--- a/gecco_amd/csrc/api_network.hip
+++ b/gecco_amd/csrc/api_network.hip
@@ -10,11 +10,11 @@
 
 namespace {
 
-std::atomic<int> g_options[OPT_COUNT] = {-1, -1, -1, -1, -1, -1, -1, -1, -1, -1, -1, -1, -1, -1, -1, -1, -1, -1, -1, -1};
-const char* const g_option_names[OPT_COUNT] = {"astat", "chain", "headmajor", "mlpfused", "unpoolfused", "lo8", "actimg", "h8", "kvq64", "h8areg", "chain2", "unpoolh8", "mlpw", "chaincl", "h6", "kvfold", "mlpwshare", "kvqperm", "imgproj16", "lift0"};
+std::atomic<int> g_options[OPT_COUNT] = {-1, -1, -1, -1, -1, -1, -1, -1, -1, -1, -1, -1, -1, -1, -1, -1, -1, -1, -1, -1, -1, -1};
+const char* const g_option_names[OPT_COUNT] = {"astat", "chain", "headmajor", "mlpfused", "unpoolfused", "lo8", "actimg", "h8", "kvq64", "h8areg", "chain2", "unpoolh8", "mlpw", "chaincl", "h6", "kvfold", "mlpwshare", "kvqperm", "imgproj16", "lift0", nullptr, "lift0front"};
 const char* const g_option_env[OPT_COUNT] = {"GECCO_ASTAT", "GECCO_CHAIN", "GECCO_HEADMAJOR", "GECCO_MLPFUSED", "GECCO_UNPOOLFUSED", "GECCO_LO8",
                                              "GECCO_ACTIMG", "GECCO_H8", "GECCO_KVQ64", "GECCO_H8AREG", "GECCO_CHAIN2", "GECCO_UNPOOLH8", "GECCO_MLPW", "GECCO_CHAINCL", "GECCO_H6", "GECCO_KVFOLD", "GECCO_MLPWSHARE",
-                                             "GECCO_KVQPERM", "GECCO_IMGPROJ16", "GECCO_LIFT0"};
+                                             "GECCO_KVQPERM", "GECCO_IMGPROJ16", "GECCO_LIFT0", nullptr, "GECCO_LIFT0FRONT"};
 thread_local const GeccoSetTransformer* t_plan = nullptr;
 struct PlanScope {
     const GeccoSetTransformer* prev;
@@ -43,7 +43,7 @@
     }
     int v = g_options[which].load(std::memory_order_relaxed);
     if (v < 0) {
-        const char* e = getenv(g_option_env[which]);
+        const char* e = g_option_env[which] ? getenv(g_option_env[which]) : nullptr;
         const int fill = which == OPT_LIFT0 ? (e ? (atoi(e) < 0 ? 0 : atoi(e) > 2 ? 2 : atoi(e)) : 3)
                          : e ? (atoi(e) != 0) : (which != OPT_MLPWSHARE && which != OPT_IMGPROJ16);
         if (g_options[which].compare_exchange_strong(v, fill, std::memory_order_relaxed)) v = fill;
@@ -248,6 +248,7 @@
     bool kvfold;
     int lift0;
     bool lift0_hm;
+    bool lift0_nofeat;
 };
 
 StRoute st_route(const GeccoSetTransformer* st, int B, int N, const float* const* h_in, bool points) {
@@ -317,6 +318,7 @@
     if (r.lift0 == 2 && !lift0_pool_supported(C, H)) r.lift0 = 1;
     r.lift0_hm = r.lift0 && r.io16 && r.astat && r.hd_try && lift0_head_major_ok(C / H);
     if (r.lift0 && r.uo8_on && !r.lift0_hm) r.lift0 = 0;
+    r.lift0_nofeat = r.lift0 >= 1 && r.uo8_on && option(OPT_LIFT0FRONT);
     return r;
 }
 
@@ -519,9 +521,14 @@
     if (r.uo8_on) {
         if (!c.hm || !c.im) return fail(-3, "set_transformer: unpool + out_proj (h8) needs the head-major fp16 q");
         if (!c.kv_img_done) TRY(kvh_image_launch(w.kvh, w.attn, B, C, H, s), "unpool k | v image");
-        UnpoolH8Args ua{};
+        UnpoolH8PtsArgs ua{};
         ua.x = x; ua.q16 = w.q; ua.kv_img = w.attn; ua.w_img = c.im + w.o_out; ua.bias = L.unpool_out_b; ua.stats = w.stats_x; ua.B = B; ua.rows = N; ua.H = H;
-        TRY(unpool_outproj_h8_launch(ua, C, s), "unpool attention + out_proj (h8)");
+        if (c.pts && r.lift0_nofeat) {
+            ua.pts = c.pts->x; ua.coef = c.pts->coef; ua.lift_w = c.pts->lift_w; ua.lift_b = c.pts->lift_b;
+            TRY(unpool_outproj_h8_points_launch(ua, C, s), "unpool attention + out_proj (h8, residual from the points)");
+        } else {
+            TRY(unpool_outproj_h8_launch(ua, C, s), "unpool attention + out_proj (h8)");
+        }
     } else if (r.uof_on && c.hm) {
         UnpoolProjArgs ua{};
         ua.x = x; ua.q16 = w.q; ua.kvh = w.kvh; ua.w_stream = c.im + w.o_out; ua.bias = L.unpool_out_b; ua.stats = w.stats_x; ua.B = B; ua.rows = N; ua.H = H;
@@ -684,18 +691,18 @@
 int gecco_option_index(const char* name) {
     if (name)
         for (int i = 0; i < OPT_COUNT; ++i)
-            if (!strcmp(name, g_option_names[i])) return i;
+            if (g_option_names[i] && !strcmp(name, g_option_names[i])) return i;
     return -1;
 }
 
 int gecco_set_option(const char* name, int value) {
     if (!name) return fail(-1, "set_option: null name");
     for (int i = 0; i < OPT_COUNT; ++i)
-        if (!strcmp(name, g_option_names[i])) {
+        if (g_option_names[i] && !strcmp(name, g_option_names[i])) {
             g_options[i].store(value < 0 ? -1 : i == OPT_LIFT0 ? (value > 2 ? 2 : value) : (value != 0), std::memory_order_relaxed);
             return 0;
         }
-    return fail(-2, "set_option: unknown option '%s' (astat, chain, headmajor, mlpfused, unpoolfused, lo8, actimg, h8, kvq64, h8areg, chain2, unpoolh8, mlpw, chaincl, h6, kvfold, mlpwshare, kvqperm, imgproj16, lift0)", name);
+    return fail(-2, "set_option: unknown option '%s' (astat, chain, headmajor, mlpfused, unpoolfused, lo8, actimg, h8, kvq64, h8areg, chain2, unpoolh8, mlpw, chaincl, h6, kvfold, mlpwshare, kvqperm, imgproj16, lift0, lift0front)", name);
 }
 
 size_t gecco_set_transformer_workspace_bytes(const GeccoSetTransformer* st, int B, int N) {
@@ -721,7 +728,12 @@
     hipStream_t s = (hipStream_t)stream;
     const int C = m->inner.C;
     TRY(edm_coeffs_launch(sigma, m->sigma_data, w.coef, B, s), "edm_coeffs");
-    TRY(lift_launch(x, w.coef, m->lift_w, m->lift_b, w.feat, w.stats, B, N, C, s), "lift");
+    bool nofeat;
+    {
+        PlanScope plan_scope(&m->inner);
+        nofeat = st_route(&m->inner, B, N, h_in, true).lift0_nofeat;
+    }
+    TRY(lift_launch(x, w.coef, m->lift_w, m->lift_b, nofeat ? nullptr : w.feat, w.stats, B, N, C, s), "lift");
     if (m->inner.ctx_dim != 1) return fail(-3, "linear_lift: t_embed_dim must be 1 under EDMPrecond");
     const Lift0In pts{x, w.coef, m->lift_w, m->lift_b};
     int rc = st_forward(&m->inner, w.feat, w.coef + 4 * (size_t)B, w.stats, row_tiles_stats(N), h_in, h_out, nullptr, B,
diff --git a/gecco_amd/csrc/kernel_prims.h b/gecco_amd/csrc/kernel_prims.h
--- a/gecco_amd/csrc/kernel_prims.h
+++ b/gecco_amd/csrc/kernel_prims.h
@@ -68,6 +68,19 @@
 __device__ __forceinline__ float lanes_sum(float v, int width) {
     for (int o = 1; o < width; o <<= 1) v += __shfl_xor(v, o, 64);
     return v;
+}
+
+__device__ __forceinline__ float lift_value(float x0, float x1, float x2, float w0, float w1, float w2, float b) {
+#pragma clang fp contract(off)
+    const float t1 = x1 * w1, t2 = x2 * w2;
+    const float s01 = __builtin_fmaf(x0, w0, t1);
+    const float s012 = s01 + t2;
+    return s012 + b;
+}
+__device__ __forceinline__ float add_square(float s, float v) {
+#pragma clang fp contract(off)
+    const float vv = v * v;
+    return s + vv;
 }
 
 __device__ __forceinline__ unsigned pack2(float v0, float v1) {
diff --git a/gecco_amd/csrc/kernels.h b/gecco_amd/csrc/kernels.h
--- a/gecco_amd/csrc/kernels.h
+++ b/gecco_amd/csrc/kernels.h
@@ -122,10 +122,16 @@
     int rev;
     int stagger, pair;
 };
+struct UnpoolH8PtsArgs : UnpoolH8Args {
+    const float* pts;
+    const float* coef;
+    const float *lift_w, *lift_b;
+};
 bool unpool_outproj_h8_supported(int C, int H, int rows);
 size_t unpool_outproj_h8_kv_bytes(int B, int C, int H);
 int kvh_image_launch(const float* kvh, void* img, int B, int C, int H, hipStream_t st);
 int unpool_outproj_h8_launch(const UnpoolH8Args& g, int C, hipStream_t st);
+int unpool_outproj_h8_points_launch(const UnpoolH8PtsArgs& g, int C, hipStream_t st);
 
 struct MlpWArgs {
     const float* x;
diff --git a/gecco_amd/csrc/pointwise.hip b/gecco_amd/csrc/pointwise.hip
--- a/gecco_amd/csrc/pointwise.hip
+++ b/gecco_amd/csrc/pointwise.hip
@@ -205,6 +205,7 @@
     coef[4 * B + b] = logf(s) / 4.0f;
 }
 
+template <bool STORE>
 __global__ __launch_bounds__(256) void lift_kernel(const float* __restrict__ x, const float* __restrict__ coef,
                                                    const float* __restrict__ W, const float* __restrict__ bias,
                                                    float* __restrict__ out, float* __restrict__ stats, int N, int C,
@@ -219,10 +220,10 @@
         const float w0 = W[c * 3 + 0], w1 = W[c * 3 + 1], w2 = W[c * 3 + 2], bb = bias ? bias[c] : 0.f;
         float s1 = 0.f, s2 = 0.f;
         for (int m = 0; m < m1 - m0; ++m) {
-            const float v = xs[m * 3 + 0] * w0 + xs[m * 3 + 1] * w1 + xs[m * 3 + 2] * w2 + bb;
-            out[((size_t)b * N + m0 + m) * C + c] = v;
+            const float v = lift_value(xs[m * 3 + 0], xs[m * 3 + 1], xs[m * 3 + 2], w0, w1, w2, bb);
+            if (STORE) out[((size_t)b * N + m0 + m) * C + c] = v;
             s1 += v;
-            s2 += v * v;
+            s2 = add_square(s2, v);
         }
         if (stats) {
             stats[(((size_t)b * T + tile) * 2 + 0) * C + c] = s1;
@@ -653,7 +654,9 @@
 int lift_launch(const float* x, const float* coef, const float* W, const float* bias, float* out, float* stats, int B,
                 int N, int C, hipStream_t st) {
     const int T = (N + STATS_ROWS - 1) / STATS_ROWS;
-    hipLaunchKernelGGL(lift_kernel, dim3(B * T), dim3(256), 0, st, x, coef, W, bias, out, stats, N, C, T);
+    if (!out && !stats) return -3;
+    if (out) hipLaunchKernelGGL(lift_kernel<true>, dim3(B * T), dim3(256), 0, st, x, coef, W, bias, out, stats, N, C, T);
+    else hipLaunchKernelGGL(lift_kernel<false>, dim3(B * T), dim3(256), 0, st, x, coef, W, bias, out, stats, N, C, T);
     return (int)hipGetLastError();
 }
 
diff --git a/gecco_amd/csrc/unpool_outproj_h8.hip b/gecco_amd/csrc/unpool_outproj_h8.hip
--- a/gecco_amd/csrc/unpool_outproj_h8.hip
+++ b/gecco_amd/csrc/unpool_outproj_h8.hip
@@ -81,12 +81,14 @@
     for (int i = threadIdx.x; i < kvb / 16; i += 256) dst[i] = reinterpret_cast<const u32x4*>(buf)[i];
 }
 
-template <int NG, int HD, int NS>
-__global__ __launch_bounds__(256, NG > 6 ? 1 : 2) void unpool_outproj_h8_kernel(UnpoolH8Args g) {
+template <int NG, int HD, int NS, bool PTS>
+__global__ __launch_bounds__(256, NG > 6 ? 1 : 2) void unpool_outproj_h8_kernel(std::conditional_t<PTS, UnpoolH8PtsArgs, UnpoolH8Args> g) {
     constexpr int C = 64 * NG, H = C / HD, NKT = 2 * NG, NC = HD / 16, DT = (HD + 31) / 32;
     constexpr int KS = HD + 8, VS = 72, KVB = u_kv_bytes(HD), PK = KVB / 4096;
     static_assert(C % HD == 0 && HD % 16 == 0 && HD <= 64, "head dims 16 .. 64");
     constexpr int TTSF = u_tts_floats(HD);
+    constexpr int RES = PTS ? 0 : U_RES;
+    static_assert((128 + C) * 4 <= TTSF, "the points form's tables fit the residual tiles' region");
     static_assert(NS >= 4 && NS <= NKT, "lookahead NS - 1 >= 3 stages; the residual pieces land inside their tile");
     extern __shared__ __attribute__((aligned(16))) float smem[];
     float* ring = smem;
@@ -279,7 +281,7 @@
         }
     };
 
-    float* tt = tts + wave * U_TT;
+    [[maybe_unused]] float* tt = tts + wave * U_TT;
     float* xw = g.x + ((size_t)b * g.rows + m0 + wave * 32) * C;
     const __amdgpu_buffer_rsrc_t xrsrc = __builtin_amdgcn_make_buffer_rsrc(xw, 0, 0x7fffffff, 0x00020000);
     auto issue_res = [&](int ct) {
@@ -302,25 +304,55 @@
         int ln = lane;
         asm volatile("" : "+v"(ln));
         const int r = ln & 31, h = ln >> 5;
-        const float* tl = tt + 4 * h * 64 + r;
         const unsigned vo = (unsigned)((4 * h * C + r) * 4);
-#pragma unroll
-        for (int j = 0; j < 2; ++j) {
-            const float bc = bias_lds[n0 + 32 * j + r];
-            float s1 = 0.f, s2 = 0.f;
+        if constexpr (PTS) {
+            const float4* pl = reinterpret_cast<const float4*>(tts) + wave * 32 + 4 * h;
+            const float4* ll = reinterpret_cast<const float4*>(tts) + 128 + n0 + r;
+            const float4 lw[2] = {ll[0], ll[32]};
+            const float bc[2] = {bias_lds[n0 + r], bias_lds[n0 + 32 + r]};
+            float s1[2] = {0.f, 0.f}, s2[2] = {0.f, 0.f};
 #pragma unroll
             for (int qe = 0; qe < 16; ++qe) {
                 const int row = 8 * (qe >> 2) + (qe & 3);
-                const float v = (acc[j][qe] + bc) + tl[row * 64 + 32 * j];
-                __builtin_amdgcn_raw_buffer_store_b32(__builtin_bit_cast(int, v), xrsrc, vo, (unsigned)((row * C + n0 + 32 * j) * 4), 0);
-                s1 += v;
-                s2 = __builtin_fmaf(v, v, s2);
+                const float4 p = pl[row];
+#pragma unroll
+                for (int j = 0; j < 2; ++j) {
+                    const float v = (acc[j][qe] + bc[j]) + lift_value(p.x, p.y, p.z, lw[j].x, lw[j].y, lw[j].z, lw[j].w);
+                    __builtin_amdgcn_raw_buffer_store_b32(__builtin_bit_cast(int, v), xrsrc, vo, (unsigned)((row * C + n0 + 32 * j) * 4), 0);
+                    s1[j] += v;
+                    s2[j] = __builtin_fmaf(v, v, s2[j]);
+                }
             }
             if (g.stats) {
-                const float t1 = sum_halves(s1), t2 = sum_halves(s2);
-                if (ln < 32) {
-                    red[(wave * 2 + 0) * 64 + 32 * j + r] = t1;
-                    red[(wave * 2 + 1) * 64 + 32 * j + r] = t2;
+#pragma unroll
+                for (int j = 0; j < 2; ++j) {
+                    const float t1 = sum_halves(s1[j]), t2 = sum_halves(s2[j]);
+                    if (ln < 32) {
+                        red[(wave * 2 + 0) * 64 + 32 * j + r] = t1;
+                        red[(wave * 2 + 1) * 64 + 32 * j + r] = t2;
+                    }
+                }
+            }
+        } else {
+            const float* tl = tt + 4 * h * 64 + r;
+#pragma unroll
+            for (int j = 0; j < 2; ++j) {
+                const float bc = bias_lds[n0 + 32 * j + r];
+                float s1 = 0.f, s2 = 0.f;
+#pragma unroll
+                for (int qe = 0; qe < 16; ++qe) {
+                    const int row = 8 * (qe >> 2) + (qe & 3);
+                    const float v = (acc[j][qe] + bc) + tl[row * 64 + 32 * j];
+                    __builtin_amdgcn_raw_buffer_store_b32(__builtin_bit_cast(int, v), xrsrc, vo, (unsigned)((row * C + n0 + 32 * j) * 4), 0);
+                    s1 += v;
+                    s2 = __builtin_fmaf(v, v, s2);
+                }
+                if (g.stats) {
+                    const float t1 = sum_halves(s1), t2 = sum_halves(s2);
+                    if (ln < 32) {
+                        red[(wave * 2 + 0) * 64 + 32 * j + r] = t1;
+                        red[(wave * 2 + 1) * 64 + 32 * j + r] = t2;
+                    }
                 }
             }
         }
@@ -342,6 +374,16 @@
 
     dma::wait_vm_lgkm0<0>();
     __builtin_amdgcn_s_barrier();
+    if constexpr (PTS) {
+        float4* pl = reinterpret_cast<float4*>(tts);
+        const float cin = g.coef ? g.coef[4 * b + 2] : 1.0f;
+        if (tid < 128) {
+            const float* p = g.pts + ((size_t)b * g.rows + m0 + tid) * 3;
+            pl[tid] = make_float4(cin * p[0], cin * p[1], cin * p[2], 0.f);
+        }
+        for (int n = tid; n < C; n += 256)
+            pl[128 + n] = make_float4(g.lift_w[n * 3 + 0], g.lift_w[n * 3 + 1], g.lift_w[n * 3 + 2], g.lift_b ? g.lift_b[n] : 0.f);
+    }
     int slot = 0;
     load_f(ring, fbA);
     float one = H8_AH_DIV;
@@ -354,10 +396,10 @@
             if (ct == 0) dma::wait_vm_lgkm0<young>();
             else dma::wait_vm_lgkm0<young + U_STORES>();
         } else if constexpr (kt <= NS - 3) {
-            if (ct == 0) dma::wait_vm_lgkm0<young + U_RES>();
-            else dma::wait_vm_lgkm0<young + U_RES + U_STORES>();
+            if (ct == 0) dma::wait_vm_lgkm0<young + RES>();
+            else dma::wait_vm_lgkm0<young + RES + U_STORES>();
         } else if constexpr (kt == NS - 2) {
-            dma::wait_vm_lgkm0<young + U_RES>();
+            dma::wait_vm_lgkm0<young + RES>();
         } else {
             dma::wait_vm_lgkm0<young>();
         }
@@ -369,7 +411,7 @@
         }
         issue();
 #if !defined(UO8_DIAG_NORES) && !defined(UO8_DIAG_NOEPI)
-        if constexpr (kt == 0) issue_res(ct);
+        if constexpr (kt == 0 && !PTS) issue_res(ct);
 #endif
         const float* cur = ring + slot * U_STAGE;
         slot = slot + 1 == NS ? 0 : slot + 1;
@@ -439,13 +481,13 @@
     USTAMP(3);
 }
 
-template <int NG, int HD, int NS>
-int uo8_launch_t(const UnpoolH8Args& g, hipStream_t st) {
+template <int NG, int HD, int NS, bool PTS>
+int uo8_launch_t(const std::conditional_t<PTS, UnpoolH8PtsArgs, UnpoolH8Args>& g, hipStream_t st) {
     constexpr int C = 64 * NG;
     constexpr size_t lds = ((size_t)NS * U_STAGE + u_tts_floats(HD) + C + 4 * 2 * 64) * sizeof(float);
     static_assert(lds <= 80 * 1024 || NG > 6, "two blocks per CU");
-    if (const hipError_t e = lds_opt_in<unpool_outproj_h8_kernel<NG, HD, NS>>(lds)) return (int)e;
-    hipLaunchKernelGGL((unpool_outproj_h8_kernel<NG, HD, NS>), dim3(g.B * (g.rows / 128)), dim3(256), lds, st, g);
+    if (const hipError_t e = lds_opt_in<unpool_outproj_h8_kernel<NG, HD, NS, PTS>>(lds)) return (int)e;
+    hipLaunchKernelGGL((unpool_outproj_h8_kernel<NG, HD, NS, PTS>), dim3(g.B * (g.rows / 128)), dim3(256), lds, st, g);
     return (int)hipGetLastError();
 }
 
@@ -467,19 +509,31 @@
     return (int)hipGetLastError();
 }
 
-int unpool_outproj_h8_launch(const UnpoolH8Args& g0, int C, hipStream_t st) {
+namespace {
+
+template <bool PTS, class Args>
+int uo8_launch(const Args& g0, int C, hipStream_t st) {
     if (!unpool_outproj_h8_supported(C, g0.H, g0.rows)) return -9;
     static const int rev = env_int("GECCO_UO8_REV", 1);
     static const int stagger = env_int("GECCO_UO8_STAGGER", 0);
     static const int pair = env_int("GECCO_UO8_PAIR", 32);
-    UnpoolH8Args g = g0;
+    Args g = g0;
     g.rev = rev != 0;
     g.stagger = g.B * (g.rows / 128) >= 512 ? stagger : 0;
     g.pair = pair > 0 ? pair : 32;
     switch (C) {
-        case 128: return uo8_launch_t<2, 16, 4>(g, st);
-        case 256: return uo8_launch_t<4, 32, 5>(g, st);
-        case 512: return uo8_launch_t<8, 64, 4>(g, st);
-        default: return uo8_launch_t<6, 48, 5>(g, st);
-    }
-}
+        case 128: return uo8_launch_t<2, 16, 4, PTS>(g, st);
+        case 256: return uo8_launch_t<4, 32, 5, PTS>(g, st);
+        case 512: return uo8_launch_t<8, 64, 4, PTS>(g, st);
+        default: return uo8_launch_t<6, 48, 5, PTS>(g, st);
+    }
+}
+
+}
+
+int unpool_outproj_h8_launch(const UnpoolH8Args& g, int C, hipStream_t st) { return uo8_launch<false>(g, C, st); }
+
+int unpool_outproj_h8_points_launch(const UnpoolH8PtsArgs& g, int C, hipStream_t st) {
+    if (!g.pts || !g.lift_w) return -3;
+    return uo8_launch<true>(g, C, st);
+}
diff --git a/gecco_amd/hip_ops.py b/gecco_amd/hip_ops.py
--- a/gecco_amd/hip_ops.py
+++ b/gecco_amd/hip_ops.py
@@ -369,15 +369,20 @@
 
 
 def unpool_outproj_h8(x: Tensor, q16: Tensor, kvh: Tensor, W: Tensor, bias: Tensor | None, H: int, want_stats: bool = False,
-                      wsplit: Tensor | None = None, image_ready: bool = False, stats: Tensor | None = None):
+                      wsplit: Tensor | None = None, image_ready: bool = False, stats: Tensor | None = None,
+                      points: tuple[Tensor, Tensor | None, Tensor, Tensor | None] | None = None):
     lib = _lib.load()
     B, rows, Cc = x.shape
     if stats is None and want_stats:
         stats = torch.empty(B, rows // 128, 2, Cc, device=x.device, dtype=torch.float32)
     if wsplit is None:
         wsplit = _ws(lib.gecco_unpool_outproj_h8_wsplit_bytes(B, Cc, H), x.device)
-    check(lib.gecco_unpool_outproj_h8(_ptr(x), _ptr16(q16), _ptr(kvh), None if image_ready else _ptr(W), _ptr(bias), _ptr(stats), B, rows, Cc, H,
-                                      C.c_void_p(wsplit.data_ptr()), _stream()), "gecco_unpool_outproj_h8")
+    pts, coef, lift_w, lift_b = points if points is not None else (None, None, None, None)
+    if points is not None:
+        assert pts.shape == (B, rows, 3) and lift_w.shape == (Cc, 3), (pts.shape, lift_w.shape, x.shape)
+    check(lib.gecco_unpool_outproj_h8_points(_ptr(x), _ptr16(q16), _ptr(kvh), None if image_ready else _ptr(W), _ptr(bias), _ptr(stats),
+                                             _ptr(pts), _ptr(coef), _ptr(lift_w), _ptr(lift_b), B, rows, Cc, H,
+                                             C.c_void_p(wsplit.data_ptr()), _stream()), "gecco_unpool_outproj_h8")
     return x, stats
 
 
@@ -522,12 +527,14 @@
         raise ValueError(f"the HIP LinearLift supports geometry_dim 1 .. {MAX_GEOMETRY_DIM}, got {G}")
 
 
-def lift(x: Tensor, coef: Tensor | None, W: Tensor, bias: Tensor | None, want_stats: bool = False):
+def lift(x: Tensor, coef: Tensor | None, W: Tensor, bias: Tensor | None, want_stats: bool = False, stats_only: bool = False):
     lib = _lib.load()
     B, N, G = x.shape
     assert W.shape[1] == G, (W.shape, x.shape)
+    assert not stats_only or G == 3, "the statistics-only lift is the 3-D kernel's"
+    want_stats = want_stats or stats_only
     Cc = W.shape[0]
-    out = torch.empty(B, N, Cc, device=x.device, dtype=torch.float32)
+    out = None if stats_only else torch.empty(B, N, Cc, device=x.device, dtype=torch.float32)
     stats = torch.empty(B, lib.gecco_stats_row_tiles(N), 2, Cc, device=x.device, dtype=torch.float32) if want_stats else None
     if G == 3:
         check(lib.gecco_lift_f32(_ptr(x), _ptr(coef), _ptr(W), _ptr(bias), _ptr(out), _ptr(stats), B, N, Cc, _stream()),
diff --git a/include/gecco_hip.h b/include/gecco_hip.h
--- a/include/gecco_hip.h
+++ b/include/gecco_hip.h
@@ -155,6 +155,9 @@
 size_t gecco_mlp_fused_w_wsplit_bytes(int C, int width);
 int gecco_unpool_outproj_h8(float* x, const void* q16, const float* kvh, const float* W, const float* bias, float* stats,
                             int B, int rows, int C, int H, void* wsplit, void* stream);
+int gecco_unpool_outproj_h8_points(float* x, const void* q16, const float* kvh, const float* W, const float* bias, float* stats,
+                                   const float* pts, const float* coef, const float* lift_w, const float* lift_b, int B, int rows, int C,
+                                   int H, void* wsplit, void* stream);
 size_t gecco_unpool_outproj_h8_wsplit_bytes(int B, int C, int H);
 int gecco_unpool_attn_h8img(const void* q16, const float* kvh, void* out_img, int B, int N, int C, int H, void* stream);
 int gecco_affine_cast_f16(const float* x, const float* a, const float* o, void* y16, int B, int rows, int C,
```

Result: no change. 30.96 million points/s (-0.4%).
